# MingXiangL/SPE

Hardware: AMD Instinct MI355X
Metric: images/sec (whole node) at 3x800x1333 bs=2/GPU (higher is better)
Workload: dtype bf16/fp16 operands, fp32 accumulate; 1 GPU; TSCAM_cait_S24 (C=384, depth 24, 8 heads) + 0-layer encoder + 6-layer conditional-DETR decoder x2 stages, 100 queries, COCO heads (91), 2x3x800x1333 per GPU (N=4150 tokens), fwd + SetCriterion + SetCriterionRefine + bwd + grad all-reduce + clip + AdamW; global_batch=2, parallelism=dp1

## Files before the change

### include/spe_hip.h

```cpp
#ifndef SPE_HIP_H
#define SPE_HIP_H
#include <stddef.h>
#include <stdint.h>

#ifdef __cplusplus
extern "C" {
#endif

typedef struct ihipStream_t* spe_stream_t;

int spe_abi_version(void);

int spe_set_reduce_workspace(void* ws, size_t bytes, spe_stream_t stream);
int spe_reduce_defer_ranges(const void* const* ptrs, const size_t* bytes, int n);
int spe_reduce_defer_arena(void* arena, size_t bytes);
int spe_reduce_flush(spe_stream_t stream);
int spe_reduce_pending(void);

int spe_gemm_f32(const float* A, const float* B, float* C, const float* bias, float* C2,
                 int M, int N, int K, long lda, long ldb, long ldc, int transA, int transB,
                 int batch0, int batch1, long sA0, long sA1, long sB0, long sB1, long sC0, long sC1,
                 float alpha, int act, int splitk, int precision, spe_stream_t stream);

int spe_gemm_ex(const void* A, int a_bf16, const float* B, float* C, const float* bias, float* C2,
                int M, int N, int K, long lda, long ldb, long ldc, int transA, int transB,
                int batch0, int batch1, long sA0, long sA1, long sB0, long sB1, long sC0, long sC1,
                float alpha, int act, int splitk, int precision, spe_stream_t stream);

int spe_gemm_tile(int M, int N, int nbatch);
int spe_gemm_f32_plan(int M, int N, int K, long lda, long ldb, long ldc, int transA, int transB, int batch0, int batch1,
                      long sA0, long sA1, long sB0, long sB1, long sC0, long sC1, int splitk, int precision, int a_bf16,
                      int epilogue, int a_mod16, int b_mod16, long* v);

int spe_layernorm_fwd(const float* x, const float* gamma, const float* beta, float* y, float* mean,
                      float* rstd, long R, int C, float eps, void* y16, void* y16lo, spe_stream_t stream);
int spe_layernorm_fwd_h(const float* x, const float* gamma, const float* beta, float* y, float* mean,
                        float* rstd, long R, int C, float eps, void* y16, void* yh16, spe_stream_t stream);
int spe_layernorm_bwd(const float* dy, const float* x, const float* gamma, const float* mean,
                      const float* rstd, float* dx, float* dgamma, float* dbeta, long R, int C,
                      const float* add, spe_stream_t stream);
int spe_layernorm_bwd_ls(const float* dy, const float* x, const float* gamma, const float* mean, const float* rstd, float* dx,
                         float* dgamma, float* dbeta, long R, int C, const float* add, const float* ls_y, const float* ls_gamma,
                         void* ls_dy16, float* ls_db, float* ls_dg, spe_stream_t stream);

int spe_cvt_f16(const float* x, long ldx, int R, int C, void* out, long ldo, spe_stream_t stream);
int spe_gemm_bf16nt(const void* A16, const void* B16, const void* A16lo, const void* B16lo, float* C, const float* bias,
                    float* C2, int M, int N, int K, long lda, long ldb, long ldc, float alpha, int act, int splitk,
                    spe_stream_t stream);
int spe_linear_small_fwd(const float* x, long ldx, const void* W16, const void* W16lo, const float* bias, float* y, float* pre,
                         void* x16_out, int R, int N, int K, long ldc, int act, spe_stream_t stream);
int spe_linear_small_bwd(const float* dy, const float* aux, int act, const void* x16, const void* WT16, float* dx, float* dW,
                         float* db, int R, int N, int K, spe_stream_t stream);
int spe_linear_small_group_fwd(const float* x, long ldx, const void* const* W16, const void* const* W16lo, const float* const* bias,
                               const float* const* add, float* const* y, void* x16_out, int R, int nblk, int N, int K, spe_stream_t stream);
int spe_linear_small_group_bwd(const float* const* dy, const void* x16, const void* const* WT16, float* dx, float* const* dW,
                               float* const* db, int R, int nblk, int N, int K, spe_stream_t stream);
int spe_linear_small_plan(int entry, int R, int N, int K, int nblk, long ldx, int split, int want_dx, int want_dw, int want_db,
                          int any_dw, long* v);
int spe_gemm_bf16tn(const void* A16, const void* B16, float* C, int M, int N, int R, long lda, long ldb, long ldc,
                    float alpha, int splitk, spe_stream_t stream);
int spe_gemm_bf16tn_plan(int M, int N, int R, long lda, long ldb, int splitk, int* v);
int spe_gemm_bf16nt_ex(const void* A16, const void* B16, const void* A16lo, const void* B16lo, float* C, const float* bias,
                       float* C2, void* out16, void* out16lo, long ld16, void* out16T, long ld16t, float* colsum, const float* aux,
                       const float* res, const float* rgamma, int M, int N, int K, long lda, long ldb, long ldc, float alpha, int act,
                       int half_flags, spe_stream_t stream);
int spe_gemm_bf16nt_exd(const void* A16, const void* B16, const void* A16lo, const void* B16lo, float* C, const float* bias,
                        float* C2, void* out16, void* out16lo, long ld16, void* out16T, long ld16t, float* colsum, const float* aux,
                        const float* res, const float* rgamma, int M, int N, int K, long lda, long ldb, long ldc, float alpha, int act,
                        int half_flags, float p_drop, uint64_t seed, uint64_t offset, const float* sample_scale, long rows_per_sample,
                        spe_stream_t stream);
int spe_gemm_bf16nt_plan(int M, int N, int K, int split, int ex, int f16_operands, int f16_second, int splitk, int has_out16t,
                         long ld16t, int* plan);
int spe_cvt_bf16(const float* x, long ldx, int R, int C, void* out, void* out_lo, long ldo, void* outT, long ldt, float* colsum,
                 const float* aux, int act, spe_stream_t stream);
int spe_cvt_bf16_h(const float* x, long ldx, int R, int C, void* out, void* out_h, long ldo, void* outT, long ldt, spe_stream_t stream);
int spe_cvt_bf16_multi(const void* jobs_dev, int njobs, int total_tiles, spe_stream_t stream);

int spe_softmax_fwd(const float* S, const unsigned char* mask, float* P, float* Pd, int B, int H, int Nq,
                    int Nk, long ld, float p_drop, uint64_t seed, uint64_t offset, spe_stream_t stream);
int spe_softmax_bwd(const float* dPd, const float* P, float* dS, int B, int H, int Nq, int Nk, long ld,
                    float p_drop, uint64_t seed, uint64_t offset, spe_stream_t stream);

int spe_talking_softmax_fwd(const float* S, const float* Wl, const float* bl, const float* Ww, const float* bw,
                            float* P, float* Pd, int B, int H, int Nq, int Nk, long ld, float p_drop,
                            uint64_t seed, uint64_t offset, spe_stream_t stream);
int spe_talking_softmax_bwd(const float* dPd, const float* P, const float* S, const float* Wl, const float* Ww,
                            float* dS, float* ws, int nblocks, int B, int H, int Nq, int Nk, long ld,
                            float p_drop, uint64_t seed, uint64_t offset, spe_stream_t stream);

int spe_talking_fused_supported(int H, int dh);
int spe_attn_pack(const float* x, long sb, long sn, long sh, int B, int N, int H, int dh, float scale,
                  void* out, spe_stream_t stream);
int spe_talking_stats_plan(int B, int N, int nwg, int* steps_per_wg, int* nwg_used);
int spe_talking_stats(const void* Qf, const void* Kf, const float* Wl, const float* bl, float* ws_stats,
                      int B, int H, int N, int dh, int nwg, spe_stream_t stream);
int spe_attn_merge_rows(const float* ws, float* M, float* IL, const float* bl, float* rows, int Np, int B, int H, int N,
                        int steps_per_wg, spe_stream_t stream);
int spe_talking_wgrad_reduce(const float* ws_w, int nwg, int H, float* dWl, float* dbl, float* dWw, float* dbw,
                             spe_stream_t stream);

int spe_talking_flash_plan(int B, int N, int nwg, int* steps_per_wg, int* nwg_used, int* nmajor, int* rows_padded);
int spe_talking_flash_fwd(const void* Qf, const void* Kf, const void* V16, const float* Wl, const float* Ww, const float* bw,
                          const float* c0, int Np, float* ws, float* O, void* O16, void* O16lo, void* keepbits, int B, int H, int N, int dh,
                          int nwg, float p_drop, uint64_t seed, uint64_t offset, spe_stream_t stream);

int spe_talking_bwdk_pass1(const void* Qf, const void* dOf, const void* dO16, const void* Kf, const void* Vf, const float* Wl, const float* Ww,
                           const float* bw, const float* c0, int Np, float* ws_d, float* ws_v, float* ws_w, float* Drows, float* dv, void* dv16,
                           long ob, long on, long oh, const void* keepbits, int B, int H, int N, int dh, int nwg, float p_drop, spe_stream_t stream);
int spe_talking_bwdq_plan(int B, int N, int nwg, int* steps_per_wg, int* nwg_used, int* nmajor);
int spe_talking_bwdq_pass2(const void* Qf, const void* dOf, const void* Kf, const void* Vf, const void* K16, const float* Wl, const float* Ww,
                           const float* c0, const float* Drows, int Np, float* ws_q, float* ws_w, void* dS, float* dq, void* dq16,
                           long ob, long on, long oh, float scale, const void* keepbits, int B, int H, int N, int dh, int nwg, float p_drop,
                           spe_stream_t stream);

int spe_attn_pmean(const void* Qf, const void* Kf, const float* Wl, const float* c0, int Np, float* M, float alpha, int B, int H, int N, int dh,
                   spe_stream_t stream);
int spe_attn_pmean_dense(const float* P, float* M, float alpha, int B, int H, int N, long ld, spe_stream_t stream);

int spe_conv_head_fwd(const float* x, const float* W, const float* bias, float* map, float* logits, int B, int h, int w, int C, int K,
                      spe_stream_t stream);
int spe_conv_head_plan(int B, int h, int w, int C, int K, long* ws_floats);
int spe_conv_head_bwd(const float* x, const float* W, const float* dmap, const float* dlogits, float* dx, float* dW, float* db, float* ws,
                      long ws_floats, int B, int h, int w, int C, int K, spe_stream_t stream);

int spe_attn_pack16(const float* x, long sb, long sn, long sh, int B, int N, int H, int dh, void* out, spe_stream_t stream);
int spe_attn_pack_multi(int njobs, const float* const* xs, const long* strides, const float* scales, const int* kinds,
                        void* const* outs, const int* Ns, const int* dhs, int B, int H, spe_stream_t stream);
int spe_attn_contract(const void* T, const void* X16, float* out, long ob, long on, long oh, int B, int H, int N, int dh,
                      int trans, int fmt, float alpha, float* ws, unsigned int* counters, long ws_floats, void* out16,
                      void* out16lo, spe_stream_t stream);

int spe_colsum(const float* in, float* out, long R, int C, long ld, int accumulate, spe_stream_t stream);

int spe_layerscale_residual_fwd(const float* x, const float* y, const float* gamma, const float* sample_scale,
                                float* out, long R, int C, long rows_per_sample, spe_stream_t stream);
int spe_layerscale_residual_bwd(const float* dout, const float* y, const float* gamma, const float* sample_scale,
                                float* dy, float* dgamma, long R, int C, long rows_per_sample, spe_stream_t stream);
int spe_layerscale_residual_bwd16(const float* dout, const void* y, int y_f16, const float* gamma, void* dy16, void* dy16T, long ldt,
                                  float* db, float* dgamma, long R, int C, spe_stream_t stream);
int spe_layerscale_residual_bwd16d(const float* dout, const void* y, int y_f16, const float* gamma, void* dy16, void* dy16T, long ldt,
                                   float* db, float* dgamma, long R, int C, float p_drop, uint64_t seed, uint64_t offset,
                                   const float* sample_scale, long rows_per_sample, spe_stream_t stream);

int spe_act_bwd(const float* dy, const float* aux, float* dx, long n, int mode, spe_stream_t stream);

int spe_layernorm_res_fwd(const float* x, const float* z, const float* gamma, const float* beta, float* sum, float* y,
                          float* mean, float* rstd, long R, int C, float eps, float p, uint64_t seed, uint64_t offset,
                          spe_stream_t stream);
int spe_layernorm_res_bwd(const float* dy, const float* dy2, const float* sum, const float* gamma, const float* mean, const float* rstd,
                          float* ds, float* dz, float* dgamma, float* dbeta, long R, int C, float p, uint64_t seed,
                          uint64_t offset, spe_stream_t stream);

int spe_dropout(const float* x, float* y, long n, float p, uint64_t seed, uint64_t offset, spe_stream_t stream);

int spe_patchify(const float* img, float* cols, int B, int Cin, int Hi, int Wi, int P, spe_stream_t stream);

int spe_rowdot(const float* x, const float* y, float* D, int B, int L, int H, int dh, spe_stream_t stream);

int spe_add_rows(const float* a, const float* b, float* out, long n, long period, spe_stream_t stream);

int spe_bicubic(const float* src, float* dst, int gh, int gw, int h, int w, int C, int backward, spe_stream_t stream);

int spe_matcher_cost(const float* logits, const float* boxes, const int* tgt_ids, const float* tgt_boxes,
                     const int* toff, int total_targets, float* cost, int* err, int L, int B, int Q, int Kc,
                     float w_class, float w_bbox, float w_giou, spe_stream_t stream);

int spe_hungarian(const float* cost, const int* toff, long* srow, long* gidx, int* lidx, int* err, int L, int B, int Q,
                  spe_stream_t stream);
int spe_jitter_pick(const float* box, const float* scale, float* out, int M, int ncand, int ratio, spe_stream_t stream);

int spe_focal_loss(const float* logits, const int* tclass, const float* roww, float* grad, float* loss,
                   int* argmax, int L, long rows_per_l, int Kc, float alpha, float gamma, spe_stream_t stream);

int spe_box_loss(const float* pred_boxes, const long* srow, const float* tbox, const float* w, const int* lidx,
                 float* sums, float* g_l1, float* g_giou, long n, int L, spe_stream_t stream);
int spe_box_loss_bwd(const long* srow, const int* lidx, const float* g_l1, const float* g_giou, const float* c1,
                     const float* c2, float* dpred, long n, spe_stream_t stream);

int spe_kv_frags(const void* ym16, long ldm, const void* yp16, long ldp, void* Kf, void* V16, void* K16, void* Vf,
                 int L, int B, int S, int H, int dh, spe_stream_t stream);
int spe_kv_grad_scatter(const float* dk, const float* dv, void* dYm, long ldm, void* dYp, long ldp, int layer, int B, int S,
                        int H, int dh, spe_stream_t stream);
int spe_colsum_bf16_blocks(const void* x, long ld, long R, int nblk, int blkC, float* const* outs, int accumulate, spe_stream_t stream);

int spe_mha_plan(int B, int H, int Lq, int Lk, int* nch);
int spe_mha_fwd(const void* Qf, const void* Kf, const void* V16, const void* mask, float* Opart, float* ML, float* O,
                float* LSE, void* keepbits, int B, int H, int Lq, int Lk, int dk, int dv, int nch, float p_drop,
                uint64_t seed, uint64_t offset, spe_stream_t stream);
int spe_mha_bwd(const void* Qf, const void* Kf, const void* Vf, const void* dOf, const void* K16, const void* Q16,
                const void* dO16, const void* mask, const float* LSE, const float* D, const void* keepbits, float* dq,
                float* dq_ws, float* dk, float* dv, int B, int H, int Lq, int Lk, int dk_dim, int dv_dim, int nch, float scale,
                float p_drop, spe_stream_t stream);

int spe_pos_sine(const void* mask_u8, const float* dim_t, float* out, int B, int h, int w, int npf, float scale,
                 float eps, int normalize, spe_stream_t stream);

int spe_pos_learned_fwd(const float* col, const float* row, float* out, int B, int h, int w, int npf, spe_stream_t stream);
int spe_pos_learned_bwd(const float* g, float* d_col, float* d_row, int B, int h, int w, int npf, spe_stream_t stream);

int spe_nms_sorted(const float* boxes, const long* labels, const int* counts, unsigned char* keep, int nimg, int nmax,
                   float iou_threshold, spe_stream_t stream);

int spe_detect(const float* logits, const float* boxes, const float* sizes, int B, int Q, int Kc, int k, float iou_threshold,
               int do_nms, float* out_logit, long* out_label, float* out_box, int* out_query, int* out_count, spe_stream_t stream);

int spe_cam_prepare(const float* cams, int M, int h, int w, int rows, int cols, float cam_thr, float* minmax,
                    void* out, spe_stream_t stream);
int spe_cam_contour_boxes(const void* img, int rows, int cols, float area_ratio, int* boxes, int max_boxes, int* nboxes);
int spe_cam_boxes_device_workspace(int M, int rows, int cols, size_t* bytes);
int spe_cam_boxes_device(const void* img, int M, int rows, int cols, float area_ratio, void* workspace, size_t workspace_bytes,
                         int* boxes, int* nboxes, int max_boxes, spe_stream_t stream);

int spe_cam_targets(const int* packed, const int* cls0, int M, int max_boxes, int single, int W, int H, int cap, float* boxes,
                    long* labels, int* off, spe_stream_t stream);
int spe_refine_pick(const float* prob, const float* pred_boxes, const int* cls, const int* cls_off, const int* cls_host,
                    const int* cls_off_host, int B, int Q, int Kc, int U, float* scores, int* queries, float* boxes, spe_stream_t stream);

int spe_pseudo_quality(const float* boxes, const long* labels, const float* scores, const int* off, const float* gboxes,
                       const long* glabels, const int* goff, const int* off_host, const int* goff_host, int B, int T, int G, int C,
                       float iou_thresh, long* counters, spe_stream_t stream);

int spe_proposal_recall(const float* prob, const float* boxes, const float* gboxes, const long* glabels, const int* goff,
                        const int* goff_host, int B, int Q, int Kc, int G, int C, const float* thr, int T, const int* ks, int K,
                        long* counters, spe_stream_t stream);

int spe_voc_match(const float* det_boxes, const float* det_scores, const long* det_labels, const int* det_off,
                  const double* gt_boxes, const long* gt_labels, const unsigned char* gt_difficult, const int* gt_off,
                  int nimg, int num_classes, int max_det, int max_gt, double ovthresh, double score_scale, double coord_scale,
                  unsigned char* flags, double* scores_out, int* npos, int* nimgs, int* hits, spe_stream_t stream);
int spe_voc_ap(const unsigned char* flags, const int* seg_off, const int* npos, int num_classes, double* ap07, double* ap_area,
               double* rec, double* prec, spe_stream_t stream);

int spe_coco_match(const float* det_boxes, const long* det_cats, const int* det_off, const double* gt_boxes, const long* gt_cats,
                   const unsigned char* gt_iscrowd, const double* gt_area, const int* gt_off, const double* iou_thrs,
                   const double* area_rng, int nimg, int num_cats, int max_det, int max_gt, int top, int* rank, unsigned* words,
                   int* npig, spe_stream_t stream);
int spe_coco_accumulate(const unsigned* words, const int* rank, const float* det_scores, const int* seg_off, const int* npig,
                        const int* max_dets, const double* rec_thrs, int num_cats, int num_rec, int num_max_dets, double* precision,
                        double* recall, double* scores, spe_stream_t stream);

int spe_cls_ap_workspace(int n, int C, size_t* bytes);
int spe_cls_ap(const float* scores, const signed char* targets, int n, int C, long ld, int difficult, double* workspace, double* ap,
               int* npos, int* ncounted, spe_stream_t stream);

int spe_resample_plan(long* desc_host, int n, long* totals);
int spe_resample_tables(const long* desc_host, const long* desc_dev, int n, int* tables, spe_stream_t stream);
int spe_resample_h(const long* desc_host, const long* desc_dev, int n, const int* tables, unsigned char* tmp, spe_stream_t stream);
int spe_resample_v(const long* desc_host, const long* desc_dev, int n, const int* tables, const unsigned char* tmp, const float* lut,
                   float* out, unsigned char* mask, int Hmax, int Wmax, spe_stream_t stream);

#define SPE_JPEG_UNSUPPORTED (-7)
#define SPE_JPEG_CORRUPT (-8)
#define SPE_JPEG_INFO_INTS 224
int spe_jpeg_probe(const unsigned char* data, long n, int* info);
int spe_jpeg_entropy(const unsigned char* data, long n, short* coef, long coef_elems, int* reason);
int spe_jpeg_reconstruct(const long* desc_host, const long* desc_dev, int n, const short* coef, long coef_elems,
                         unsigned char* planes, long planes_bytes, spe_stream_t stream);

int spe_ledger_state_bytes(int K, int E, size_t* bytes);
int spe_ledger_record(const float* vals, const float* weights, const unsigned char* mask, const double* extras_host, int K, int E,
                      void* state, size_t state_bytes, float* total, spe_stream_t stream);
int spe_ledger_total_bwd(const float* g, const float* weights, const unsigned char* mask, int K, float* dvals, spe_stream_t stream);
int spe_ledger_summary(void* state, size_t state_bytes, int K, int E, const int* windows_host, const int* windows_dev,
                       const float* ring_override, const int* order, double* out, spe_stream_t stream);

int spe_sqnorm_partials(const float* g, long n, float* partials, int nblocks, spe_stream_t stream);
int spe_adamw_flat(float* p, float* g, float* m, float* v, long n, const long* seg_end, const float* seg_lr,
                   const float* seg_wd, int nseg, float beta1, float beta2, float eps, float bias_c1, float bias_c2,
                   const float* partials, int npartials, float max_norm, int write_grad, float grad_scale,
                   spe_stream_t stream);

#define SPE_ADAMW_GUARD_WORDS 16
int spe_adamw_gate(void* guard, const float* partials, int npartials, float max_norm, float grad_scale, double beta1,
                   double beta2, spe_stream_t stream);
int spe_adamw_flat_guarded(float* p, float* g, float* m, float* v, long n, const long* seg_end, const float* seg_lr,
                           const float* seg_wd, int nseg, float beta1, float beta2, float eps, const void* guard,
                           int write_grad, spe_stream_t stream);

int spe_accum_flat(float* dst, const float* a, const float* b, long n, spe_stream_t stream);

int spe_adamw_flat_ema(float* p, float* g, float* m, float* v, float* e, long n, const long* seg_end, const float* seg_lr,
                       const float* seg_wd, int nseg, float beta1, float beta2, float eps, float bias_c1, float bias_c2,
                       const float* partials, int npartials, float max_norm, int write_grad, float grad_scale,
                       const void* guard, double decay, int warmup, long t, spe_stream_t stream);
int spe_swap_flat(float* a, float* b, long n, spe_stream_t stream);

#define SPE_GRAD_REPORT_WORDS 8
int spe_grad_report(const float* g, const float* p, long n, const long* par_beg, const long* par_len, int npar,
                    float grad_scale, const void* guard, int when, void* out, spe_stream_t stream);

int spe_occupy(int nwg, long micros, float* buf, long buf_floats, spe_stream_t stream);

#ifdef __cplusplus
}
#endif
#endif
```

### spe_amd/csrc/attn_flash.hip

```cpp
#include "attn_flash_common.h"

struct FlashFwdArgs {
    const unsigned char* Qf; const unsigned char* Kf; const unsigned char* V16;
    const float* Wl; const float* Ww; const float* bw;
    const float* c0;
    int Np;
    float* ws_o;
    int B, N, nt, nmaj, spw; long total;
    float p_drop; uint64_t seed, offset;
    unsigned* keepbits;
};

#define FLF_NW 8
#define FLF_HB 4
#define FLF_QS (FLF_MAJ / FLF_NW)

template <int H, int DSTEPS, bool TAIL16, bool DROP>
__global__ __launch_bounds__(64 * FLF_NW, FLF_NW / 4) void talking_flash_fwd_kernel(FlashFwdArgs a) {
    constexpr int FULL = FragDims<DSTEPS, TAIL16>::FULL, DT = FragDims<DSTEPS, TAIL16>::DT, REC = FragDims<DSTEPS, TAIL16>::REC;
    constexpr int NW = FLF_NW, QS = FLF_QS;
    constexpr int TILEB = H * REC;
    extern __shared__ __attribute__((aligned(16))) unsigned char smem[];
    const int lane = threadIdx.x & 63, wave = __builtin_amdgcn_readfirstlane(threadIdx.x >> 6);
    const unsigned lds0 = __builtin_amdgcn_readfirstlane((unsigned)(uintptr_t)(__attribute__((address_space(3))) unsigned char*)smem);
    const unsigned char* sQ = smem + 5 * TILEB + wave * (QS * TILEB);
    const unsigned ldsQ = lds0 + 5 * TILEB + wave * (QS * TILEB);
    const int grp = wave >> 2;
    const int nt = a.nt, N = a.N;

    float Al4[H / 4][H];
    fl_mixA_f32<H, false>(a.Wl, lane, Al4);
    fls16x4_t Aw[H / 4][H / 4];
    fl_mixA_16<H, false, true>(a.Ww, lane, 1.0f, Aw);
    f32x4_t vbws[H / 4];
#pragma unroll
    for (int gh = 0; gh < H / 4; ++gh)
#pragma unroll
        for (int i = 0; i < 4; ++i) vbws[gh][i] = a.bw[4 * gh + i] * FL_PD_SCALE;
    constexpr int NP = TILEB / 1024, NPW = (NP + NW - 1) / NW;
    unsigned voff[NPW];
#pragma unroll
    for (int i = 0; i < NPW; ++i) {
        const int o = (i * NW + wave) * 1024 + lane * 16;
        voff[i] = (unsigned)((o / REC) * nt * REC + o % REC);
    }

    const long s_begin = (long)blockIdx.x * a.spw;
    long s_end = s_begin + a.spw; if (s_end > a.total) s_end = a.total;
    long s = s_begin;
    while (s < s_end) {
        const int bm = (int)(s / nt), kt0 = (int)(s % nt);
        int seg = nt - kt0; if (seg > s_end - s) seg = (int)(s_end - s);
        const int b = bm / a.nmaj, mj = bm % a.nmaj;
        const int qt0 = (mj * NW + wave) * QS;
        const bool wvalid = qt0 < nt;

#pragma unroll
        for (int u = 0; u < QS; ++u) {
            constexpr int NPQ = TILEB / 1024;
            const unsigned char* qbase = a.Qf + ((long)b * H * nt + min(qt0 + u, nt - 1)) * REC;
#pragma unroll
            for (int p = 0; p < NPQ; ++p) {
                const int o = p * 1024 + lane * 16;
                fl_glds16_s(qbase, (unsigned)((o / REC) * nt * REC + o % REC), ldsQ + u * TILEB + p * 1024);
            }
        }
        auto issue_tile = [&](const unsigned char* base, int kt, unsigned dst) {
            const unsigned char* tb = base + ((long)b * H * nt + kt) * REC;
            if constexpr (NP % NW == 0 && NPW <= 4) fl_glds16_run<NPW, NW * 1024>(tb, voff, dst + wave * 1024);
            else {
#pragma unroll
                for (int i = 0; i < NPW; ++i) {
                    const int p = i * NW + wave;
                    if (NP % NW != 0 && p >= NP) break;
                    fl_glds16_s(tb, voff[i], dst + p * 1024);
                }
            }
        };
        issue_tile(a.Kf, kt0, lds0);

        f32x4_t c0v[QS][H / 4];
        int qrow[QS];
#pragma unroll
        for (int u = 0; u < QS; ++u) {
            qrow[u] = (qt0 + u) * 16 + (lane & 15);
            const float* cp = a.c0 + ((long)b * a.Np + (wvalid ? min(qrow[u], N - 1) : 0)) * H;
#pragma unroll
            for (int gh = 0; gh < H / 4; ++gh) {
                c0v[u][gh] = *reinterpret_cast<const f32x4_t*>(cp + 4 * gh);
#pragma unroll
                for (int i = 0; i < 4; ++i) c0v[u][gh][i] += 8.0f;
            }
        }
        f32x4_t O[QS][H][DT];
#pragma unroll
        for (int u = 0; u < QS; ++u)
#pragma unroll
            for (int g = 0; g < H; ++g)
#pragma unroll
                for (int dt = 0; dt < DT; ++dt) O[u][g][dt] = (f32x4_t){0.f, 0.f, 0.f, 0.f};

        auto step_barrier = [&](int j) {
            asm volatile("s_waitcnt vmcnt(0)" ::: "memory");
            __builtin_amdgcn_s_barrier();
            asm volatile("" ::: "memory");
            if (j + 1 < seg) issue_tile(a.Kf, kt0 + j + 1, lds0 + ((j + 1) % 3) * TILEB);
            if (j < seg) issue_tile(a.V16, kt0 + j, lds0 + (3 + (j & 1)) * TILEB);
        };
        step_barrier(0);
        for (int i = 0; i < seg; ++i) {
            if (grp == 0) step_barrier(i + 1);
            if (!wvalid) { if (grp != 0) step_barrier(i + 1); continue; }
            const unsigned char* sK = smem + (i % 3) * TILEB;
            const unsigned char* sV = smem + (3 + (i & 1)) * TILEB;
            fls16x4_t bv[QS][4][H / 4];
#pragma unroll
            for (int u = 0; u < QS; ++u) {
                f32x4_t sp[4][H / 4];
#pragma unroll
                for (int r = 0; r < 4; ++r)
#pragma unroll
                    for (int gh = 0; gh < H / 4; ++gh) sp[r][gh] = c0v[u][gh];
#pragma unroll
                for (int h0 = 0; h0 < H; h0 += FLF_HB) {
                    flu32x4_t kf[FLF_HB][FULL ? FULL : 1], qf[FLF_HB][FULL ? FULL : 1];
                    fls16x4_t kt16[FLF_HB], qt16[FLF_HB];
#pragma unroll
                    for (int hb = 0; hb < FLF_HB; ++hb) {
                        const unsigned char* kr = sK + (h0 + hb) * REC;
                        const unsigned char* qr = sQ + (u * H + h0 + hb) * REC;
#pragma unroll
                        for (int st = 0; st < FULL; ++st) {
                            kf[hb][st] = *reinterpret_cast<const flu32x4_t*>(kr + st * 1024 + lane * 16);
                            qf[hb][st] = *reinterpret_cast<const flu32x4_t*>(qr + st * 1024 + lane * 16);
                        }
                        if constexpr (TAIL16) {
                            kt16[hb] = *reinterpret_cast<const fls16x4_t*>(kr + FULL * 1024 + lane * 8);
                            qt16[hb] = *reinterpret_cast<const fls16x4_t*>(qr + FULL * 1024 + lane * 8);
                        }
                    }
#pragma unroll
                    for (int hb = 0; hb < FLF_HB; ++hb) {
                        f32x4_t c = {0.f, 0.f, 0.f, 0.f};
#pragma unroll
                        for (int st = 0; st < FULL; ++st) c = fl_mfma32<true>(kf[hb][st], qf[hb][st], c);
                        if constexpr (TAIL16) {
                            const f32x4_t t = fl_mfma16<true>(kt16[hb], qt16[hb], (f32x4_t){0.f, 0.f, 0.f, 0.f});
                            c = (FULL > 0) ? c + t : t;
                        }
#pragma unroll
                        for (int r = 0; r < 4; ++r)
#pragma unroll
                            for (int gh = 0; gh < H / 4; ++gh) sp[r][gh] = __builtin_amdgcn_mfma_f32_4x4x1f32(Al4[gh][h0 + hb], c[r], sp[r][gh], 0, 0, 0);
                    }
                }
#pragma unroll
                for (int r = 0; r < 4; ++r)
#pragma unroll
                    for (int hh = 0; hh < H / 4; ++hh)
                        bv[u][r][hh] = fl_pack4_f16(fl_exp2(sp[r][hh][0]), fl_exp2(sp[r][hh][1]), fl_exp2(sp[r][hh][2]), fl_exp2(sp[r][hh][3]));
                __builtin_amdgcn_sched_barrier(0);
            }
            if (grp != 0) step_barrier(i + 1);
#pragma unroll
            for (int u = 0; u < QS; ++u) {
                f32x4_t pr[4][H / 4];
#pragma unroll
                for (int r = 0; r < 4; ++r)
#pragma unroll
                    for (int gh = 0; gh < H / 4; ++gh) {
                        f32x4_t d = vbws[gh];
#pragma unroll
                        for (int hh = 0; hh < H / 4; ++hh)
                            d = __builtin_amdgcn_mfma_f32_4x4x4f16(__builtin_bit_cast(flf16x4_t, Aw[gh][hh]), __builtin_bit_cast(flf16x4_t, bv[u][r][hh]), d, 0, 0, 0);
                        pr[r][gh] = d;
                    }
                if constexpr (DROP) {
                    const uint32_t thr = (uint32_t)(a.p_drop * 65536.0f);
                    const float inv = 1.0f / (1.0f - a.p_drop);
                    uint32_t kbw = 0u;
#pragma unroll
                    for (int hp = 0; hp < H / 2; ++hp) {
                        const int g0 = 2 * hp, g1 = 2 * hp + 1;
                        uint32_t o[4];
                        fl_keep_lots<H>(a.seed, a.offset, b, hp, qrow[u], (kt0 + i) * 16 + 4 * (lane >> 4), N, o);
#pragma unroll
                        for (int r = 0; r < 4; ++r) {
                            const bool e0 = fl_lot(o, 0, r) >= thr, e1 = fl_lot(o, 1, r) >= thr;
                            pr[r][g0 >> 2][g0 & 3] *= e0 ? inv : 0.f;
                            pr[r][g1 >> 2][g1 & 3] *= e1 ? inv : 0.f;
                            kbw |= ((e0 ? 1u : 0u) | (e1 ? 2u : 0u)) << (hp * 8 + 2 * r);
                        }
                    }
                    if (a.keepbits && wvalid && qt0 + u < nt) a.keepbits[(((long)b * nt + (qt0 + u)) * nt + (kt0 + i)) * 64 + lane] = kbw;
                }
#pragma unroll
                for (int g = 0; g < H; ++g) {
                    const fls16x4_t pk = fl_pack4<true>(pr[0][g >> 2][g & 3], pr[1][g >> 2][g & 3], pr[2][g >> 2][g & 3], pr[3][g >> 2][g & 3]);
#pragma unroll
                    for (int dt = 0; dt < DT; ++dt)
                        O[u][g][dt] = fl_mfma16<true>(*reinterpret_cast<const fls16x4_t*>(sV + g * REC + dt * 512 + lane * 8), pk, O[u][g][dt]);
                }
                __builtin_amdgcn_sched_barrier(0);
            }
        }
        __builtin_amdgcn_s_barrier();

        if (wvalid) {
            const int first_wg = (int)(((long)bm * nt) / a.spw);
            const int slot = (int)blockIdx.x - first_wg;
#pragma unroll
            for (int u = 0; u < QS; ++u) {
                if (qt0 + u >= nt) continue;
                float* dst = a.ws_o + ((((long)bm * FL_MAXSLOT + slot) * NW + wave) * QS + u) * (long)(H * DT * 256);
#pragma unroll
                for (int g = 0; g < H; ++g)
#pragma unroll
                    for (int dt = 0; dt < DT; ++dt) *reinterpret_cast<f32x4_t*>(dst + (g * DT + dt) * 256 + lane * 4) = O[u][g][dt];
            }
        }
        s += seg;
    }
}

__global__ __launch_bounds__(256) void flash_merge_kernel(const float* __restrict__ ws, float* __restrict__ O, long ob, long on, long oh,
                                                          unsigned short* __restrict__ O16, unsigned short* __restrict__ O16lo,
                                                          int B, int H, int N, int nt, int dh, int DT, int nmaj, int spw, long nvec) {
    const long i = (long)blockIdx.x * 256 + threadIdx.x;
    if (i >= nvec) return;
    constexpr int QS = FLF_QS;
    const int lane = (int)(i & 63);
    long r = i >> 6;
    const int dt = (int)(r % DT); r /= DT;
    const int g = (int)(r % H); r /= H;
    const int u = (int)(r % QS); r /= QS;
    const int wave = (int)(r % FLF_NW); r /= FLF_NW;
    const int bm = (int)r;
    const int b = bm / nmaj, mj = bm % nmaj;
    const int qt = (mj * FLF_NW + wave) * QS + u;
    const int q = qt * 16 + (lane & 15), d = dt * 16 + 4 * (lane >> 4);
    if (qt >= nt || q >= N || d >= dh) return;
    const int first_wg = (int)(((long)bm * nt) / spw), last_wg = (int)(((long)(bm + 1) * nt - 1) / spw);
    const long slot_stride = (long)FLF_MAJ * H * DT * 256;
    const float* src = ws + (long)bm * FL_MAXSLOT * slot_stride + (((long)wave * QS + u) * H + g) * (long)(DT * 256) + dt * 256 + lane * 4;
    f32x4_t acc = {0.f, 0.f, 0.f, 0.f};
    for (int sl = 0; sl <= last_wg - first_wg; ++sl) acc += *reinterpret_cast<const f32x4_t*>(src + sl * slot_stride);
    acc *= (1.0f / FL_PD_SCALE);
    const long oi = (long)b * ob + (long)q * on + (long)g * oh + d;
    if (d + 3 < dh && ((ob | on | oh) & 3) == 0) {
        if (O && ((reinterpret_cast<uintptr_t>(O) & 15) == 0)) *reinterpret_cast<f32x4_t*>(O + oi) = acc;
        else if (O) { O[oi] = acc[0]; O[oi + 1] = acc[1]; O[oi + 2] = acc[2]; O[oi + 3] = acc[3]; }
        if (O16) {
            unsigned short hi[4], lo[4];
#pragma unroll
            for (int k = 0; k < 4; ++k) { hi[k] = spe_f2bf(acc[k]); lo[k] = spe_f2bf(acc[k] - spe_bf2f(hi[k])); }
            const uint2 h2 = make_uint2((unsigned)hi[0] | ((unsigned)hi[1] << 16), (unsigned)hi[2] | ((unsigned)hi[3] << 16));
            if ((reinterpret_cast<uintptr_t>(O16) & 7) == 0) *reinterpret_cast<uint2*>(O16 + oi) = h2;
            else { O16[oi] = hi[0]; O16[oi + 1] = hi[1]; O16[oi + 2] = hi[2]; O16[oi + 3] = hi[3]; }
            if (O16lo) {
                const uint2 l2 = make_uint2((unsigned)lo[0] | ((unsigned)lo[1] << 16), (unsigned)lo[2] | ((unsigned)lo[3] << 16));
                if ((reinterpret_cast<uintptr_t>(O16lo) & 7) == 0) *reinterpret_cast<uint2*>(O16lo + oi) = l2;
                else { O16lo[oi] = lo[0]; O16lo[oi + 1] = lo[1]; O16lo[oi + 2] = lo[2]; O16lo[oi + 3] = lo[3]; }
            }
        }
        return;
    }
#pragma unroll
    for (int k = 0; k < 4; ++k) {
        if (d + k >= dh) break;
        if (O) O[oi + k] = acc[k];
        if (O16) {
            const unsigned short hi = spe_f2bf(acc[k]);
            O16[oi + k] = hi;
            if (O16lo) O16lo[oi + k] = spe_f2bf(acc[k] - spe_bf2f(hi));
        }
    }
}

template <int H, int DSTEPS, bool TAIL16>
static int launch_flash_fwd(const FlashFwdArgs& a, int nwg, bool drop, hipStream_t st) {
    constexpr int DT = FragDims<DSTEPS, TAIL16>::DT;
    if constexpr (flf_lds_bytes(H, DT, true) > FL_LDS_MAX) return -2;
    else return fl_launch<FlashFwdArgs, talking_flash_fwd_kernel<H, DSTEPS, TAIL16, true>, talking_flash_fwd_kernel<H, DSTEPS, TAIL16, false>>(
        a, nwg, 64 * FLF_NW, flf_lds_bytes(H, DT, false), flf_lds_bytes(H, DT, true), drop, st);
}

extern "C" int spe_talking_flash_plan(int B, int N, int nwg, int* steps_per_wg, int* nwg_used, int* nmajor, int* rows_padded) {
    const int nt = (N + 15) / 16;
    if ((long)B * nt <= 0 || nwg <= 0) { *steps_per_wg = 0; *nwg_used = 0; *nmajor = 0; *rows_padded = 0; return 0; }
    const FlashPlan p = fl_plan(B, nt, FLF_MAJ, nt, nwg);
    *steps_per_wg = p.spw; *nwg_used = p.nwg; *nmajor = p.nmaj; *rows_padded = nt * 16 + 64;
    return 0;
}

extern "C" int spe_talking_flash_fwd(const void* Qf, const void* Kf, const void* V16, const float* Wl, const float* Ww, const float* bw,
                                     const float* c0, int Np, float* ws, float* O, void* O16, void* O16lo, void* keepbits, int B, int H, int N,
                                     int dh, int nwg, float p_drop, uint64_t seed, uint64_t offset, hipStream_t st) {
    const int nt = (N + 15) / 16;
    if ((long)B * nt <= 0) return 0;
    if (dh < 1 || dh > 64 || nwg <= 0 || (O16lo && !O16) || Np < nt * 16 + 64) return -2;
    const FlashPlan p = fl_plan(B, nt, FLF_MAJ, nt, nwg);
    FlashFwdArgs a;
    a.Qf = (const unsigned char*)Qf; a.Kf = (const unsigned char*)Kf; a.V16 = (const unsigned char*)V16;
    a.Wl = Wl; a.Ww = Ww; a.bw = bw; a.c0 = c0; a.Np = Np; a.ws_o = ws;
    a.B = B; a.N = N; a.nt = nt; a.nmaj = p.nmaj; a.spw = p.spw; a.total = p.total;
    a.p_drop = p_drop; a.seed = seed; a.offset = offset; a.keepbits = reinterpret_cast<unsigned*>(p_drop > 0.f ? keepbits : nullptr);
    const bool drop = p_drop > 0.f;
    const int rc = attn_dispatch(H, dh, [&](auto h, auto ds, auto tl) {
        return launch_flash_fwd<decltype(h)::value, decltype(ds)::value, decltype(tl)::value>(a, p.nwg, drop, st); });
    if (rc != 0) return rc;
    const int DT = frag_geom(dh).dt;
    const long nvec = (long)B * p.nmaj * FLF_MAJ * H * DT * 64;
    hipLaunchKernelGGL(flash_merge_kernel, dim3((unsigned)((nvec + 255) / 256)), dim3(256), 0, st, ws, O, (long)N * H * dh, (long)H * dh, (long)dh,
                       reinterpret_cast<unsigned short*>(O16), reinterpret_cast<unsigned short*>(O16lo), B, H, N, nt, dh, DT, p.nmaj, p.spw, nvec);
    SPE_CHECK_LAUNCH();
    return 0;
}
```

### spe_amd/csrc/attn_flash_bwd.hip

```cpp
#include "attn_flash_common.h"

#define FLB_NW 4
#define FLB_HB 4
#define FLB_GWR 144
#define FLB_NK16 3
#define FLB_RSFUSE 1
#define FLB_DQAHEAD 2
#define FLB_SB_NOMEM 0x00F
#define FLB_PHASE() __builtin_amdgcn_sched_barrier(0)
#ifndef SPE_ABLATE
#undef FLB_DBG_SAMETILE
#undef FLB_DBG_NOST
#undef FLB_DBG_STAMP
#endif
#ifdef FLB_DBG_STAMP
#define FLB_STAMP(k) asm volatile("s_memtime %0\n\ts_waitcnt lgkmcnt(0)" : "=s"(stamp[k]))
#else
#define FLB_STAMP(k)
#endif
#ifndef FLB_STAGGER
#define FLB_STAGGER 1
#endif

struct FlashBwdArgs {
// ... 209 lines not shown
                    }
            }
            f32x4_t c[HB];
            static_assert(HB == 4, "chunk of 4 heads");
            flb_score_f16<FULL, TAIL16>(kfr.f, kfr.t, &qa[h0], &qta[h0], c);
            flb_fence4(c[0], c[1], c[2], c[3]);
#pragma unroll
            for (int hb = 0; hb < HB; ++hb) {
                const f32x4_t cs = c[hb];
                *reinterpret_cast<fls16x4_t*>(gwf + (h0 + hb) * GWR) = fl_pack4<false>(cs[0], cs[1], cs[2], cs[3]);
#pragma unroll
                for (int r = 0; r < 4; ++r)
#pragma unroll
                    for (int gh = 0; gh < H / 4; ++gh) sp[r][gh] = __builtin_amdgcn_mfma_f32_4x4x1f32(Al4[gh][h0 + hb], cs[r], sp[r][gh], 0, 0, 0);
            }
        };
        auto front_v = [&](int i, auto g0_c, const Frags& vfr, f32x4_t (&dp)[4][H / 4], uint32_t kb) {
            constexpr int g0 = decltype(g0_c)::value;
            if constexpr (g0 == 0) {
#pragma unroll
                for (int r = 0; r < 4; ++r)
#pragma unroll
                    for (int gh = 0; gh < H / 4; ++gh) dp[r][gh] = Dn[gh];
            }
            f32x4_t es[HB];
            flb_score_bf16<FULL, TAIL16>(vfr.f, vfr.t, &da[g0], &dta[g0], es);
            flb_fence4(es[0], es[1], es[2], es[3]);
#pragma unroll
            for (int hb = 0; hb < HB; ++hb) {
                if constexpr (DROP) {
                    const int g = g0 + hb;
#pragma unroll
                    for (int r = 0; r < 4; ++r) es[hb][r] *= ((kb >> ((g >> 1) * 8 + 2 * r + (g & 1))) & 1u) ? keep_inv : 0.f;
                }
            }
#pragma unroll
            for (int hq = 0; hq < HB / 4; ++hq)
#pragma unroll
                for (int r = 0; r < 4; ++r) {
                    const fls16x4_t bv = fl_pack4<false>(es[4 * hq][r], es[4 * hq + 1][r], es[4 * hq + 2][r], es[4 * hq + 3][r]);
#pragma unroll
                    for (int gh = 0; gh < H / 4; ++gh) dp[r][gh] = __builtin_amdgcn_mfma_f32_4x4x4bf16_1k(Awt[gh][g0 / 4 + hq], bv, dp[r][gh], 0, 0, 0);
                }
        };
        auto load_kb = [&](int i) -> uint32_t {
            if constexpr (DROP) return *reinterpret_cast<const uint32_t*>(smem + KBOFF + (i & 1) * 1024 + wave * 256 + lane * 4);
            else return 0u;
        };

        auto back_exp = [&](f32x4_t (&sp)[4][H / 4]) {
#pragma unroll
            for (int r = 0; r < 4; ++r)
#pragma unroll
                for (int gh = 0; gh < H / 4; ++gh)
#pragma unroll
                    for (int k = 0; k < 4; ++k) sp[r][gh][k] = fl_exp2(sp[r][gh][k]);
        };
        auto back_ds = [&](f32x4_t (&sp)[4][H / 4], f32x4_t (&dp)[4][H / 4]) {
            unsigned char* gwb = gw_wr + 2 * GWT;
#pragma unroll
            for (int r = 0; r < 4; ++r)
#pragma unroll
                for (int gh = 0; gh < H / 4; ++gh) sp[r][gh] = sp[r][gh] * dp[r][gh];
#pragma unroll
            for (int r = 0; r < 4; ++r)
#pragma unroll
                for (int g = 0; g < H; ++g) gb[g] += sp[r][g >> 2][g & 3];
#pragma unroll
            for (int g = 0; g < H; ++g)
                *reinterpret_cast<fls16x4_t*>(gwb + g * GWR) =
                    fl_pack4<false>(sp[0][g >> 2][g & 3], sp[1][g >> 2][g & 3], sp[2][g >> 2][g & 3], sp[3][g >> 2][g & 3]);
        };
        auto back_gw = [&](int i, f32x4_t (&sp)[4][H / 4], f32x4_t (&ds)[4][H / 4]) {
            {
                const unsigned rdf = gw_rd + (i & 1) * GWT, rdb = gw_rd + 2 * GWT;
                const unsigned char* gw_xrd = (gm < H) ? sgw + rdb : gw_zero;
                const unsigned char* gw_yrd = (gm < H) ? sgw + rdf : gw_zero;
                __builtin_amdgcn_fence(__ATOMIC_RELEASE, "wavefront");
                __builtin_amdgcn_fence(__ATOMIC_ACQUIRE, "wavefront");
#pragma unroll
                for (int c = 0; c < 8; ++c) {
                    const flu32x4_t xa = *reinterpret_cast<const flu32x4_t*>(gw_xrd + c * 16);
                    const flu32x4_t yb = *reinterpret_cast<const flu32x4_t*>(gw_yrd + c * 16);
                    gwacc[c & 3] = fl_mfma32<false>(xa, yb, gwacc[c & 3]);
                }
                __builtin_amdgcn_fence(__ATOMIC_RELEASE, "wavefront");
            }
#pragma unroll
            for (int r = 0; r < 4; ++r) {
                float x[H];
#pragma unroll
                for (int g = 0; g < H; ++g) x[g] = sp[r][g >> 2][g & 3];
                fl_mix_16<H, false>(x, Alt, nullptr, ds[r]);
            }
        };
        auto back_dq = [&](int i, f32x4_t (&ds)[4][H / 4]) {
            {
                const int kt = kt0 + i;
                const unsigned char* sK16 = smem + 2 * KVB + (i % NK16) * TILEB;
                fls16x4_t ka[H][DT];
#pragma unroll
                for (int h = 0; h < ((FLB_DQAHEAD < H) ? FLB_DQAHEAD : H); ++h)
#pragma unroll
                    for (int dt = 0; dt < DT; ++dt) ka[h][dt] = *reinterpret_cast<const fls16x4_t*>(sK16 + h * REC + dt * 512 + lane * 8);
#pragma unroll
                for (int h = 0; h < H; ++h) {
                    if (h + FLB_DQAHEAD < H) {
#pragma unroll
                        for (int dt = 0; dt < DT; ++dt) ka[h + FLB_DQAHEAD][dt] = *reinterpret_cast<const fls16x4_t*>(sK16 + (h + FLB_DQAHEAD) * REC + dt * 512 + lane * 8);
                        __builtin_amdgcn_sched_barrier(FLB_SB_NOMEM);
                    }
                    const fls16x4_t pk = fl_pack4<false>(ds[0][h >> 2][h & 3], ds[1][h >> 2][h & 3], ds[2][h >> 2][h & 3], ds[3][h >> 2][h & 3]);
#ifndef FLB_DBG_NOST
                    __builtin_nontemporal_store(__builtin_bit_cast(flu32x2_t, pk),
                                                reinterpret_cast<flu32x2_t*>(a.dS + (((((long)b * H + h) * nt + qt) * nt + kt) * 64 + lane) * 4));
#endif
                    flb_dq_mfma<DT>(dQ[h], ka[h], pk);
                }
            }
        };
        auto front = [&](int i, f32x4_t (&sp)[4][H / 4], f32x4_t (&dp)[4][H / 4], auto mask_c) {
            const uint32_t kb = load_kb(i);
            Frags fa, fb;
            load_k(i, 0, fa);
            if constexpr (H > HB) load_k(i, HB, fb);
            front_k(i, std::integral_constant<int, 0>{}, fa, sp, mask_c);
            load_v(i, 0, fa);
            if constexpr (H > HB) front_k(i, std::integral_constant<int, HB>{}, fb, sp, mask_c);
            if constexpr (H > HB) load_v(i, HB, fb);
            front_v(i, std::integral_constant<int, 0>{}, fa, dp, kb);
            if constexpr (H > HB) front_v(i, std::integral_constant<int, HB>{}, fb, dp, kb);
        };
        auto back = [&](int i, f32x4_t (&sp)[4][H / 4], f32x4_t (&dp)[4][H / 4]) {
            f32x4_t ds[4][H / 4];
            back_exp(sp);
            back_ds(sp, dp);
            back_gw(i, sp, ds);
            back_dq(i, ds);
        };
        auto step = [&](int i, f32x4_t (&sp)[4][H / 4], f32x4_t (&dp)[4][H / 4], f32x4_t (&spn)[4][H / 4], f32x4_t (&dpn)[4][H / 4], Frags& fr0, Frags& fr1,
                        bool more) {
            f32x4_t ds[4][H / 4];
            const uint32_t kb = load_kb(i + 1);
            if constexpr (H > HB) load_k(i + 1, HB, fr1); else load_v(i + 1, 0, fr1);
            __builtin_amdgcn_sched_barrier(FLB_SB_NOMEM);
            front_k(i + 1, std::integral_constant<int, 0>{}, fr0, spn, std::false_type{});
            back_exp(sp);
            FLB_PHASE();
            FLB_STAMP(2);
            if (FLB_STAGGER && more && wave >= NW / 2) issue_tiles(i + 2);
            if constexpr (H > HB) {
                load_v(i + 1, 0, fr0);
                __builtin_amdgcn_sched_barrier(FLB_SB_NOMEM);
                front_k(i + 1, std::integral_constant<int, HB>{}, fr1, spn, std::false_type{});
            }
            back_ds(sp, dp);
            FLB_PHASE();
            FLB_STAMP(3);
            if constexpr (H > HB) {
                load_v(i + 1, HB, fr1);
                __builtin_amdgcn_sched_barrier(FLB_SB_NOMEM);
                front_v(i + 1, std::integral_constant<int, 0>{}, fr0, dpn, kb);
            } else front_v(i + 1, std::integral_constant<int, 0>{}, fr1, dpn, kb);
            back_gw(i, sp, ds);
            FLB_PHASE();
            FLB_STAMP(4);
            if constexpr (H > HB) front_v(i + 1, std::integral_constant<int, HB>{}, fr1, dpn, kb);
            back_dq(i, ds);
        };

        auto admit = [&](int nxt, bool late) {
            asm volatile("s_waitcnt vmcnt(0)" ::: "memory");
            __builtin_amdgcn_s_barrier();
            asm volatile("" ::: "memory");
            if (nxt + 1 < seg && !(late && wave >= NW / 2)) issue_tiles(nxt + 1);
        };

        const int nfull = ((N & 15) != 0 && kt0 + seg == nt) ? seg - 1 : seg;
        f32x4_t spA[4][H / 4], dpA[4][H / 4], spB[4][H / 4], dpB[4][H / 4];
        Frags frA, frB;
        issue_tiles(0);
        admit(0, false);
        if (nfull > 0) {
            if (wvalid) front(0, spA, dpA, std::false_type{});
            for (int i = 0; i + 1 < nfull; ++i) {
                FLB_STAMP(0);
                admit(i + 1, FLB_STAGGER && wvalid);
                FLB_STAMP(1);
                if (wvalid) {
                    load_k(i + 1, 0, frA);
                    step(i, spA, dpA, spB, dpB, frA, frB, i + 2 < seg);
#pragma unroll
                    for (int r = 0; r < 4; ++r)
#pragma unroll
                        for (int gh = 0; gh < H / 4; ++gh) { spA[r][gh] = spB[r][gh]; dpA[r][gh] = dpB[r][gh]; }
                }
#ifdef FLB_DBG_STAMP
                FLB_STAMP(5);
                asm volatile("s_waitcnt lgkmcnt(0)" : "+s"(stamp[0]), "+s"(stamp[1]), "+s"(stamp[2]), "+s"(stamp[3]), "+s"(stamp[4]), "+s"(stamp[5]));
                for (int k = 0; k < 5; ++k) stacc[k] += stamp[k + 1] - stamp[k];
                ++stn;
#endif
            }
            if (nfull < seg) admit(nfull, false);
            if (wvalid) back(nfull - 1, spA, dpA);
        }
        if (nfull < seg) {
            if (wvalid) { front(nfull, spA, dpA, std::true_type{}); back(nfull, spA, dpA); }
        }
        __builtin_amdgcn_s_barrier();

        const int first_wg = (int)(((long)bm * nt) / a.spw);
        const int slot = (int)blockIdx.x - first_wg;
        {
#pragma unroll
            for (int g = 0; g < H; ++g)
#pragma unroll
                for (int dt = 0; dt < DT; ++dt) flb_acc_fence(dQ[g][dt]);
            if (wvalid) {
                float* dst = a.ws_q + (((long)bm * FL_MAXSLOT + slot) * NW + wave) * (long)(H * DT * 256);
#pragma unroll
                for (int g = 0; g < H; ++g)
#pragma unroll
                    for (int dt = 0; dt < DT; ++dt) *reinterpret_cast<f32x4_t*>(dst + (g * DT + dt) * 256 + lane * 4) = dQ[g][dt];
            }
        }
        s += seg;
    }

#ifdef FLB_DBG_STAMP
    if (blockIdx.x == 0 && threadIdx.x == 0) {
        unsigned long long* o = reinterpret_cast<unsigned long long*>(a.dS);
        for (int k = 0; k < 5; ++k) o[k] = stacc[k];
        o[5] = stn;
    }
#endif
    {
        constexpr int NWG = 2 * (H * H + H);
        float* row = a.ws_w + ((long)blockIdx.x * NW + wave) * NWG;
        const f32x4_t dsum = (gwacc[0] + gwacc[1]) + (gwacc[2] + gwacc[3]);
        const int nn = lane & 15;
#pragma unroll
        for (int r = 0; r < 4; ++r) {
            const int g = 4 * (lane >> 4) + r;
            if (g < H && nn < H) row[g * H + nn] = FL_LN2 * dsum[r];
        }
#pragma unroll
        for (int g = 0; g < H; ++g) {
            const float v = spe_wave_sum(gb[g]);
            if (lane == 0) row[H * H + g] = v;
        }
    }
}

__global__ __launch_bounds__(256) void bwdq_dq_merge_kernel(const float* __restrict__ ws, float* __restrict__ O, unsigned short* __restrict__ O16,
                                                            long ob, long on, long oh, int B, int H, int N, int nt, int dh, int DT, int nmaj, int spw,
                                                            float scale, long nvec) {
    const long i = (long)blockIdx.x * 256 + threadIdx.x;
    if (i >= nvec) return;
    const int lane = (int)(i & 63);
    long r = i >> 6;
    const int dt = (int)(r % DT); r /= DT;
    const int g = (int)(r % H); r /= H;
    const int wave = (int)(r % FLB_NW); r /= FLB_NW;
    const long bm = r;
    const int b = (int)(bm / nmaj), mj = (int)(bm % nmaj);
    const int qt = mj * FLB_NW + wave;
    const int q = qt * 16 + (lane & 15), d = dt * 16 + 4 * (lane >> 4);
    if (qt >= nt || q >= N || d >= dh) return;
    const int first_wg = (int)((bm * nt) / spw), last_wg = (int)(((bm + 1) * nt - 1) / spw);
    const long slot_stride = (long)FLB_NW * H * DT * 256;
    const float* src = ws + bm * FL_MAXSLOT * slot_stride + ((long)wave * H + g) * (long)(DT * 256) + dt * 256 + lane * 4;
    f32x4_t acc = {0.f, 0.f, 0.f, 0.f};
    for (int sl = 0; sl <= last_wg - first_wg; ++sl) acc += *reinterpret_cast<const f32x4_t*>(src + sl * slot_stride);
    acc *= scale;
    const long oi = (long)b * ob + (long)q * on + (long)g * oh + d;
#pragma unroll
    for (int k = 0; k < 4; ++k) {
        if (d + k >= dh) break;
        if (O) O[oi + k] = acc[k];
    }
    if (O16) {
        if (d + 3 < dh && ((ob | on | oh) & 3) == 0 && ((reinterpret_cast<uintptr_t>(O16) & 7) == 0)) {
            const unsigned short h0 = spe_f2bf(acc[0]), h1 = spe_f2bf(acc[1]), h2 = spe_f2bf(acc[2]), h3 = spe_f2bf(acc[3]);
            *reinterpret_cast<uint2*>(O16 + oi) = make_uint2((unsigned)h0 | ((unsigned)h1 << 16), (unsigned)h2 | ((unsigned)h3 << 16));
        } else {
#pragma unroll
            for (int k = 0; k < 4; ++k) { if (d + k >= dh) break; O16[oi + k] = spe_f2bf(acc[k]); }
        }
    }
}

struct FlashBwdKArgs {
    const unsigned char* Qf; const unsigned char* dOf; const unsigned char* dO16;
    const unsigned char* Kf; const unsigned char* Vf;
    const float* Wl; const float* Ww; const float* bw;
    const float* c0; int Np;
    float* ws_d;
    float* ws_v;
    float* ws_w;
    const unsigned* keepbits;
    int B, N, nt, nmaj, spw; long total;
    float p_drop;
};

__device__ __forceinline__ void flb_rowsum4(const f32x4_t (&t)[4], f32x4_t& o) {
    float a0, a1, a2, a3, b0, b1, b2, b3;
    asm("s_nop 1\n\t"
        "v_add_f32_dpp %0, %12, %12 row_ror:8 row_mask:0xf bank_mask:0x3\n\t"
        "v_add_f32_dpp %1, %13, %13 row_ror:8 row_mask:0xf bank_mask:0x3\n\t"
        "v_add_f32_dpp %2, %14, %14 row_ror:8 row_mask:0xf bank_mask:0x3\n\t"
        "v_add_f32_dpp %3, %15, %15 row_ror:8 row_mask:0xf bank_mask:0x3\n\t"
        "v_add_f32_dpp %0, %20, %20 row_ror:8 row_mask:0xf bank_mask:0xc\n\t"
        "v_add_f32_dpp %1, %21, %21 row_ror:8 row_mask:0xf bank_mask:0xc\n\t"
        "v_add_f32_dpp %2, %22, %22 row_ror:8 row_mask:0xf bank_mask:0xc\n\t"
        "v_add_f32_dpp %3, %23, %23 row_ror:8 row_mask:0xf bank_mask:0xc\n\t"
        "v_add_f32_dpp %4, %16, %16 row_ror:8 row_mask:0xf bank_mask:0x3\n\t"
        "v_add_f32_dpp %5, %17, %17 row_ror:8 row_mask:0xf bank_mask:0x3\n\t"
        "v_add_f32_dpp %6, %18, %18 row_ror:8 row_mask:0xf bank_mask:0x3\n\t"
        "v_add_f32_dpp %7, %19, %19 row_ror:8 row_mask:0xf bank_mask:0x3\n\t"
        "v_add_f32_dpp %4, %24, %24 row_ror:8 row_mask:0xf bank_mask:0xc\n\t"
        "v_add_f32_dpp %5, %25, %25 row_ror:8 row_mask:0xf bank_mask:0xc\n\t"
        "v_add_f32_dpp %6, %26, %26 row_ror:8 row_mask:0xf bank_mask:0xc\n\t"
        "v_add_f32_dpp %7, %27, %27 row_ror:8 row_mask:0xf bank_mask:0xc\n\t"
        "v_add_f32_dpp %8, %0, %0 row_half_mirror row_mask:0xf bank_mask:0x5\n\t"
        "v_add_f32_dpp %9, %1, %1 row_half_mirror row_mask:0xf bank_mask:0x5\n\t"
        "v_add_f32_dpp %10, %2, %2 row_half_mirror row_mask:0xf bank_mask:0x5\n\t"
        "v_add_f32_dpp %11, %3, %3 row_half_mirror row_mask:0xf bank_mask:0x5\n\t"
        "v_add_f32_dpp %8, %4, %4 row_half_mirror row_mask:0xf bank_mask:0xa\n\t"
        "v_add_f32_dpp %9, %5, %5 row_half_mirror row_mask:0xf bank_mask:0xa\n\t"
        "v_add_f32_dpp %10, %6, %6 row_half_mirror row_mask:0xf bank_mask:0xa\n\t"
        "v_add_f32_dpp %11, %7, %7 row_half_mirror row_mask:0xf bank_mask:0xa\n\t"
        "v_add_f32_dpp %8, %8, %8 quad_perm:[1,0,3,2] row_mask:0xf bank_mask:0xf\n\t"
        "v_add_f32_dpp %9, %9, %9 quad_perm:[1,0,3,2] row_mask:0xf bank_mask:0xf\n\t"
        "v_add_f32_dpp %10, %10, %10 quad_perm:[1,0,3,2] row_mask:0xf bank_mask:0xf\n\t"
        "v_add_f32_dpp %11, %11, %11 quad_perm:[1,0,3,2] row_mask:0xf bank_mask:0xf\n\t"
        "v_add_f32_dpp %8, %8, %8 quad_perm:[2,3,0,1] row_mask:0xf bank_mask:0xf\n\t"
        "v_add_f32_dpp %9, %9, %9 quad_perm:[2,3,0,1] row_mask:0xf bank_mask:0xf\n\t"
        "v_add_f32_dpp %10, %10, %10 quad_perm:[2,3,0,1] row_mask:0xf bank_mask:0xf\n\t"
        "v_add_f32_dpp %11, %11, %11 quad_perm:[2,3,0,1] row_mask:0xf bank_mask:0xf"
        : "=&v"(a0), "=&v"(a1), "=&v"(a2), "=&v"(a3), "=&v"(b0), "=&v"(b1), "=&v"(b2), "=&v"(b3),
          "=&v"(o[0]), "=&v"(o[1]), "=&v"(o[2]), "=&v"(o[3])
        : "v"(t[0][0]), "v"(t[0][1]), "v"(t[0][2]), "v"(t[0][3]), "v"(t[1][0]), "v"(t[1][1]), "v"(t[1][2]), "v"(t[1][3]),
          "v"(t[2][0]), "v"(t[2][1]), "v"(t[2][2]), "v"(t[2][3]), "v"(t[3][0]), "v"(t[3][1]), "v"(t[3][2]), "v"(t[3][3]));
}

#define FLB_SCORE_RS_ASM(NAME, M32, M16)                                                                                                   \
    __device__ __forceinline__ void NAME(const flu32x4_t (*k32)[1], const flu32x2_t* k16, const flu32x4_t (*q32)[1], const flu32x2_t* q16, \
                                         f32x4_t* c, const f32x4_t (&t)[4], f32x4_t& o) {                                                  \
        float a0, a1, a2, a3, b0, b1, b2, b3;                                                                                              \
            asm("s_nop 1\n\t"   \
                M32 " %0, %16, %24, 0\n\t"   \
                "v_add_f32_dpp %4, %32, %32 row_ror:8 row_mask:0xf bank_mask:0x3\n\t"   \
                "v_add_f32_dpp %5, %33, %33 row_ror:8 row_mask:0xf bank_mask:0x3\n\t"   \
                "v_add_f32_dpp %6, %34, %34 row_ror:8 row_mask:0xf bank_mask:0x3\n\t"   \
                "v_add_f32_dpp %7, %35, %35 row_ror:8 row_mask:0xf bank_mask:0x3\n\t"   \
                M32 " %1, %17, %25, 0\n\t"   \
                "v_add_f32_dpp %4, %40, %40 row_ror:8 row_mask:0xf bank_mask:0xc\n\t"   \
                "v_add_f32_dpp %5, %41, %41 row_ror:8 row_mask:0xf bank_mask:0xc\n\t"   \
                "v_add_f32_dpp %6, %42, %42 row_ror:8 row_mask:0xf bank_mask:0xc\n\t"   \
                "v_add_f32_dpp %7, %43, %43 row_ror:8 row_mask:0xf bank_mask:0xc\n\t"   \
                M32 " %2, %18, %26, 0\n\t"   \
                "v_add_f32_dpp %8, %36, %36 row_ror:8 row_mask:0xf bank_mask:0x3\n\t"   \
                "v_add_f32_dpp %9, %37, %37 row_ror:8 row_mask:0xf bank_mask:0x3\n\t"   \
                "v_add_f32_dpp %10, %38, %38 row_ror:8 row_mask:0xf bank_mask:0x3\n\t"   \
                "v_add_f32_dpp %11, %39, %39 row_ror:8 row_mask:0xf bank_mask:0x3\n\t"   \
                M32 " %3, %19, %27, 0\n\t"   \
                "v_add_f32_dpp %8, %44, %44 row_ror:8 row_mask:0xf bank_mask:0xc\n\t"   \
                "v_add_f32_dpp %9, %45, %45 row_ror:8 row_mask:0xf bank_mask:0xc\n\t"   \
                "v_add_f32_dpp %10, %46, %46 row_ror:8 row_mask:0xf bank_mask:0xc\n\t"   \
                "v_add_f32_dpp %11, %47, %47 row_ror:8 row_mask:0xf bank_mask:0xc\n\t"   \
                M16 " %0, %20, %28, %0\n\t"   \
                "v_add_f32_dpp %12, %4, %4 row_half_mirror row_mask:0xf bank_mask:0x5\n\t"   \
                "v_add_f32_dpp %13, %5, %5 row_half_mirror row_mask:0xf bank_mask:0x5\n\t"   \
                "v_add_f32_dpp %14, %6, %6 row_half_mirror row_mask:0xf bank_mask:0x5\n\t"   \
                "v_add_f32_dpp %15, %7, %7 row_half_mirror row_mask:0xf bank_mask:0x5\n\t"   \
                M16 " %1, %21, %29, %1\n\t"   \
                "v_add_f32_dpp %12, %8, %8 row_half_mirror row_mask:0xf bank_mask:0xa\n\t"   \
                "v_add_f32_dpp %13, %9, %9 row_half_mirror row_mask:0xf bank_mask:0xa\n\t"   \
                "v_add_f32_dpp %14, %10, %10 row_half_mirror row_mask:0xf bank_mask:0xa\n\t"   \
                "v_add_f32_dpp %15, %11, %11 row_half_mirror row_mask:0xf bank_mask:0xa\n\t"   \
                M16 " %2, %22, %30, %2\n\t"   \
                "v_add_f32_dpp %12, %12, %12 quad_perm:[1,0,3,2] row_mask:0xf bank_mask:0xf\n\t"   \
                "v_add_f32_dpp %13, %13, %13 quad_perm:[1,0,3,2] row_mask:0xf bank_mask:0xf\n\t"   \
                "v_add_f32_dpp %14, %14, %14 quad_perm:[1,0,3,2] row_mask:0xf bank_mask:0xf\n\t"   \
                "v_add_f32_dpp %15, %15, %15 quad_perm:[1,0,3,2] row_mask:0xf bank_mask:0xf\n\t"   \
                M16 " %3, %23, %31, %3\n\t"   \
                "v_add_f32_dpp %12, %12, %12 quad_perm:[2,3,0,1] row_mask:0xf bank_mask:0xf\n\t"   \
                "v_add_f32_dpp %13, %13, %13 quad_perm:[2,3,0,1] row_mask:0xf bank_mask:0xf\n\t"   \
                "v_add_f32_dpp %14, %14, %14 quad_perm:[2,3,0,1] row_mask:0xf bank_mask:0xf\n\t"   \
                "v_add_f32_dpp %15, %15, %15 quad_perm:[2,3,0,1] row_mask:0xf bank_mask:0xf"   \
            : "=&v"(c[0]), "=&v"(c[1]), "=&v"(c[2]), "=&v"(c[3]), "=&v"(a0), "=&v"(a1), "=&v"(a2), "=&v"(a3), "=&v"(b0), "=&v"(b1), "=&v"(b2),  \
              "=&v"(b3), "=&v"(o[0]), "=&v"(o[1]), "=&v"(o[2]), "=&v"(o[3])                                                                 \
            : "v"(k32[0][0]), "v"(k32[1][0]), "v"(k32[2][0]), "v"(k32[3][0]), "v"(k16[0]), "v"(k16[1]), "v"(k16[2]), "v"(k16[3]),          \
              "a"(q32[0][0]), "a"(q32[1][0]), "a"(q32[2][0]), "a"(q32[3][0]), "a"(q16[0]), "a"(q16[1]), "a"(q16[2]), "a"(q16[3]),          \
              "v"(t[0][0]), "v"(t[0][1]), "v"(t[0][2]), "v"(t[0][3]), "v"(t[1][0]), "v"(t[1][1]), "v"(t[1][2]), "v"(t[1][3]),              \
              "v"(t[2][0]), "v"(t[2][1]), "v"(t[2][2]), "v"(t[2][3]), "v"(t[3][0]), "v"(t[3][1]), "v"(t[3][2]), "v"(t[3][3]));             \
    }
FLB_SCORE_RS_ASM(flb_score_rs_f16, "v_mfma_f32_16x16x32_f16", "v_mfma_f32_16x16x16_f16")
FLB_SCORE_RS_ASM(flb_score_rs_bf16, "v_mfma_f32_16x16x32_bf16", "v_mfma_f32_16x16x16_bf16")



template <int H, int DSTEPS, bool TAIL16, bool DROP>
__global__ __launch_bounds__(64 * FLB_NW, 1) void talking_bwdk_kernel(FlashBwdKArgs a) {
    constexpr int FULL = FragDims<DSTEPS, TAIL16>::FULL, DT = FragDims<DSTEPS, TAIL16>::DT, REC = FragDims<DSTEPS, TAIL16>::REC;
    constexpr int NW = FLB_NW, HB = (H >= FLB_HB) ? FLB_HB : H;
    constexpr int TILEB = H * REC;
    constexpr int STG = 2 * TILEB;
    constexpr int NK16 = FLB_NK16;
    constexpr int F1 = FULL ? FULL : 1;
    extern __shared__ __attribute__((aligned(16))) unsigned char smem[];
    const int lane = threadIdx.x & 63, wave = __builtin_amdgcn_readfirstlane(threadIdx.x >> 6);
    const unsigned lds0 = __builtin_amdgcn_readfirstlane((unsigned)(uintptr_t)(__attribute__((address_space(3))) unsigned char*)smem);
    const int nt = a.nt;
    constexpr int C0OFF = 2 * STG + NK16 * TILEB, DXB = 16 * H * 4, DXOFF = C0OFF + 2048, GCOFF = DXOFF + 2 * NW * DXB;
    constexpr int KBOFF = GCOFF + 512 + NW * 3 * (4 * H * FLB_GWR);

    float Al4[H / 4][H];
    fl_mixA_f32<H, false>(a.Wl, lane, Al4);
    fls16x4_t Awt[H / 4][H / 4];
    fl_mixA_16<H, true, false>(a.Ww, lane, 1.0f, Awt);
    fls16x4_t Awp[H / 4][H / 4];
    fl_mixA_16<H, false, true>(a.Ww, lane, 1.0f, Awp);
    f32x4_t vbw[H / 4];
#pragma unroll
    for (int gh = 0; gh < H / 4; ++gh)
#pragma unroll
        for (int i = 0; i < 4; ++i) vbw[gh][i] = a.bw[4 * gh + i] * FL_PD_SCALE;

    constexpr int GWR = FLB_GWR, GWT = 4 * H * GWR;
    unsigned char* gconst = smem + GCOFF;
    unsigned char* sgw = gconst + 512 + wave * (3 * GWT);
    if (threadIdx.x < 64) reinterpret_cast<uint2*>(gconst)[threadIdx.x] = (threadIdx.x >= 26 && threadIdx.x < 42) ? make_uint2(0x3F803F80u, 0x3F803F80u) : make_uint2(0u, 0u);
    const int gm = lane & 15, gk = lane >> 4;
    unsigned char* gw_wr = sgw + (gk * H) * GWR + gm * 8;
    const unsigned gw_rd = (unsigned)((gk * H + gm) * GWR);
    const unsigned char* gw_zero = gconst + 48;
    const unsigned char* gw_ones = gconst + 208;
    f32x4_t gwacc[4];
#pragma unroll
    for (int i = 0; i < 4; ++i) gwacc[i] = (f32x4_t){0.f, 0.f, 0.f, 0.f};

    constexpr int NP = TILEB / 1024, NPW = (NP + NW - 1) / NW;
    unsigned voff[NPW];
#pragma unroll
    for (int i = 0; i < NPW; ++i) {
        const int o = (i * NW + wave) * 1024 + lane * 16;
        voff[i] = (unsigned)((o / REC) * nt * REC + o % REC);
    }
    const float keep_inv = DROP ? 1.0f / (1.0f - a.p_drop) : 1.0f;
    const int kbsh = 2 * (gm & 3);
#ifdef FLB_DBG_STAMP
    unsigned long long stamp[7] = {0, 0, 0, 0, 0, 0, 0}, stacc[6] = {0, 0, 0, 0, 0, 0}, stn = 0;
#endif
    const int kbln = (gm >> 2) << 4;

    const long s_begin = (long)blockIdx.x * a.spw;
    long s_end = s_begin + a.spw; if (s_end > a.total) s_end = a.total;
    long s = s_begin;
    while (s < s_end) {
        const int bm = (int)(s / nt), qt0 = (int)(s % nt);
        int seg = nt - qt0; if (seg > s_end - s) seg = (int)(s_end - s);
        const int b = bm / a.nmaj, mj = bm % a.nmaj;
        const int kt = mj * NW + wave;
        const bool wvalid = kt < nt;
        const int ktc = wvalid ? kt : nt - 1;
        const int nvw = (nt - mj * NW < NW) ? nt - mj * NW : NW;
        unsigned kb_voff = 0u;
        if constexpr (DROP) {
            const int w = lane >> 4, kw = (mj * NW + w < nt) ? w : 0;
            kb_voff = (unsigned)(kw * 256 + (lane & 15) * 16);
        }

        flu32x4_t ka[H][F1], va[H][F1];
        flu32x2_t kta[H], vta[H];
#pragma unroll
        for (int h = 0; h < H; ++h) {
            const unsigned char* kb_ = a.Kf + (((long)b * H + h) * nt + ktc) * REC;
            const unsigned char* vb_ = a.Vf + (((long)b * H + h) * nt + ktc) * REC;
#pragma unroll
            for (int st = 0; st < FULL; ++st) {
                ka[h][st] = *reinterpret_cast<const flu32x4_t*>(kb_ + st * 1024 + lane * 16);
                va[h][st] = *reinterpret_cast<const flu32x4_t*>(vb_ + st * 1024 + lane * 16);
            }
            if constexpr (TAIL16) {
                kta[h] = *reinterpret_cast<const flu32x2_t*>(kb_ + FULL * 1024 + lane * 8);
                vta[h] = *reinterpret_cast<const flu32x2_t*>(vb_ + FULL * 1024 + lane * 8);
            } else { kta[h] = (flu32x2_t){0u, 0u}; vta[h] = (flu32x2_t){0u, 0u}; }
        }
        f32x4_t dV[H][DT];
#pragma unroll
        for (int g = 0; g < H; ++g)
#pragma unroll
            for (int dt = 0; dt < DT; ++dt) dV[g][dt] = (f32x4_t){0.f, 0.f, 0.f, 0.f};

        auto issue_tiles = [&](int i) {
#ifdef FLB_DBG_SAMETILE
            const int qt = 0;
#else
            const int qt = qt0 + i;
#endif
#pragma unroll
            for (int op = 0; op < 3; ++op) {
                const unsigned char* base = (op == 0) ? a.Qf : ((op == 1) ? a.dOf : a.dO16);
                const unsigned char* tb = base + ((long)b * H * nt + qt) * REC;
                const unsigned dst = (op < 2) ? lds0 + (i & 1) * STG + op * TILEB : lds0 + 2 * STG + (i % NK16) * TILEB;
                if constexpr (NP % NW == 0 && NPW <= 4) fl_glds16_run<NPW, NW * 1024>(tb, voff, dst + wave * 1024);
                else {
#pragma unroll
                    for (int ii = 0; ii < NPW; ++ii) {
                        const int p = ii * NW + wave;
                        if (NP % NW != 0 && p >= NP) break;
                        fl_glds16_s(tb, voff[ii], dst + p * 1024);
                    }
                }
            }
            if (wave == NW - 1) fl_glds16_s(a.c0 + ((long)b * a.Np + qt * 16) * H, (unsigned)(lane * 16), lds0 + C0OFF + (i & 1) * 1024);
            if constexpr (DROP)
                if (wave == 1) fl_glds16_s(a.keepbits + (((long)b * nt + qt) * nt + mj * NW) * 64, kb_voff, lds0 + KBOFF + (i & 1) * 1024);
        };

        struct Frags { flu32x4_t f[HB][F1]; flu32x2_t t[HB]; };
        auto load_frags = [&](const unsigned char* tile, int h0, Frags& o) {
#pragma unroll
            for (int hb = 0; hb < HB; ++hb) {
                const unsigned char* r = tile + (h0 + hb) * REC;
#pragma unroll
                for (int st = 0; st < FULL; ++st) o.f[hb][st] = *reinterpret_cast<const flu32x4_t*>(r + st * 1024 + lane * 16);
                if constexpr (TAIL16) o.t[hb] = *reinterpret_cast<const flu32x2_t*>(r + FULL * 1024 + lane * 8);
                else o.t[hb] = (flu32x2_t){0u, 0u};
            }
        };
        auto load_q = [&](int i, int h0, Frags& o) { load_frags(smem + (i & 1) * STG, h0, o); };
        auto load_d = [&](int i, int g0, Frags& o) { load_frags(smem + (i & 1) * STG + TILEB, g0, o); };
        auto front_q = [&](int i, auto h0_c, const Frags& qfr, f32x4_t (&sp)[4][H / 4], const f32x4_t (*rs_t)[4] = nullptr, f32x4_t* rs_o = nullptr) {
            constexpr int h0 = decltype(h0_c)::value;
            if constexpr (h0 == 0) {
                const unsigned char* cr = smem + C0OFF + (i & 1) * 1024 + (4 * gk) * H * 4;
#pragma unroll
                for (int r = 0; r < 4; ++r)
#pragma unroll
                    for (int gh = 0; gh < H / 4; ++gh) sp[r][gh] = *reinterpret_cast<const f32x4_t*>(cr + (r * H + 4 * gh) * 4) + 8.0f;
            }
            f32x4_t c[HB];
            static_assert(HB == 4, "chunk of 4 heads");
            if constexpr (FULL == 1 && TAIL16) {
                if (rs_t) flb_score_rs_f16(qfr.f, qfr.t, &ka[h0], &kta[h0], c, *rs_t, *rs_o);
                else flb_score_f16<FULL, TAIL16>(qfr.f, qfr.t, &ka[h0], &kta[h0], c);
            } else flb_score_f16<FULL, TAIL16>(qfr.f, qfr.t, &ka[h0], &kta[h0], c);
            flb_fence4(c[0], c[1], c[2], c[3]);

#pragma unroll
            for (int hb = 0; hb < HB; ++hb) {
                const f32x4_t cs = c[hb];
#pragma unroll
                for (int r = 0; r < 4; ++r)
#pragma unroll
                    for (int gh = 0; gh < H / 4; ++gh) sp[r][gh] = __builtin_amdgcn_mfma_f32_4x4x1f32(Al4[gh][h0 + hb], cs[r], sp[r][gh], 0, 0, 0);
            }
        };
        auto front_d = [&](int i, auto g0_c, const Frags& dfr, f32x4_t (&dp)[4][H / 4], const uint32_t (&kb)[4], const f32x4_t (*rs_t)[4] = nullptr,
                           f32x4_t* rs_o = nullptr) {
            constexpr int g0 = decltype(g0_c)::value;
            unsigned char* gwf = gw_wr + (i & 1) * GWT;
            if constexpr (g0 == 0) {
#pragma unroll
                for (int r = 0; r < 4; ++r)
#pragma unroll
                    for (int gh = 0; gh < H / 4; ++gh) dp[r][gh] = (f32x4_t){0.f, 0.f, 0.f, 0.f};
            }
            f32x4_t es[HB];
            if constexpr (FULL == 1 && TAIL16) {
                if (rs_t) flb_score_rs_bf16(dfr.f, dfr.t, &va[g0], &vta[g0], es, *rs_t, *rs_o);
                else flb_score_bf16<FULL, TAIL16>(dfr.f, dfr.t, &va[g0], &vta[g0], es);
            } else flb_score_bf16<FULL, TAIL16>(dfr.f, dfr.t, &va[g0], &vta[g0], es);
            flb_fence4(es[0], es[1], es[2], es[3]);
#pragma unroll
            for (int hb = 0; hb < HB; ++hb) {
                if constexpr (DROP) {
                    const int g = g0 + hb;
#pragma unroll
                    for (int r = 0; r < 4; ++r) es[hb][r] *= ((kb[r] >> ((g >> 1) * 8 + kbsh + (g & 1))) & 1u) ? keep_inv : 0.f;
                }
                *reinterpret_cast<fls16x4_t*>(gwf + (g0 + hb) * GWR) = fl_pack4<false>(es[hb][0], es[hb][1], es[hb][2], es[hb][3]);
            }
#pragma unroll
            for (int hq = 0; hq < HB / 4; ++hq)
#pragma unroll
                for (int r = 0; r < 4; ++r) {
                    const fls16x4_t bv = fl_pack4<false>(es[4 * hq][r], es[4 * hq + 1][r], es[4 * hq + 2][r], es[4 * hq + 3][r]);
#pragma unroll
                    for (int gh = 0; gh < H / 4; ++gh) dp[r][gh] = __builtin_amdgcn_mfma_f32_4x4x4bf16_1k(Awt[gh][g0 / 4 + hq], bv, dp[r][gh], 0, 0, 0);
                }
        };
        auto load_kb = [&](int i, uint32_t (&kb)[4]) {
            if constexpr (DROP) {
                const flu32x4_t w4 = *reinterpret_cast<const flu32x4_t*>(smem + KBOFF + (i & 1) * 1024 + (wvalid ? wave : 0) * 256 + (kbln + 4 * gk) * 4);
#pragma unroll
                for (int r = 0; r < 4; ++r) kb[r] = w4[r];
            } else {
#pragma unroll
                for (int r = 0; r < 4; ++r) kb[r] = 0u;
            }
        };

        auto back_exp = [&](f32x4_t (&sp)[4][H / 4]) {
#pragma unroll
            for (int r = 0; r < 4; ++r)
#pragma unroll
                for (int gh = 0; gh < H / 4; ++gh)
#pragma unroll
                    for (int k = 0; k < 4; ++k) sp[r][gh][k] = fl_exp2(sp[r][gh][k]);
        };
        auto d_terms = [&](int gh, f32x4_t (&sp)[4][H / 4], f32x4_t (&dp)[4][H / 4], f32x4_t (&t)[4]) {
#pragma unroll
            for (int r = 0; r < 4; ++r) t[r] = dp[r][gh] * sp[r][gh];
        };
        auto d_store = [&](int i, int gh, const f32x4_t& o) {
            float* dx = reinterpret_cast<float*>(smem + DXOFF + ((i & 1) * NW + wave) * DXB) + (4 * gk + (gm >> 2)) * H;
            if ((gm & 3) == 0) *reinterpret_cast<f32x4_t*>(dx + 4 * gh) = o;
        };
        auto back_ds = [&](int i, f32x4_t (&sp)[4][H / 4], f32x4_t (&dp)[4][H / 4], bool with_d = true) {
            unsigned char* gwb = gw_wr + 2 * GWT;
            float* dx = reinterpret_cast<float*>(smem + DXOFF + ((i & 1) * NW + wave) * DXB) + (4 * gk + (gm >> 2)) * H;
#pragma unroll
            for (int gh = 0; gh < (with_d ? H / 4 : 0); ++gh) {
                f32x4_t t[4], o;
#pragma unroll
                for (int r = 0; r < 4; ++r) t[r] = dp[r][gh] * sp[r][gh];
                flb_rowsum4(t, o);
                if ((gm & 3) == 0) *reinterpret_cast<f32x4_t*>(dx + 4 * gh) = o;
            }
#pragma unroll
            for (int g = 0; g < H; ++g)
                *reinterpret_cast<fls16x4_t*>(gwb + g * GWR) =
                    fl_pack4<false>(sp[0][g >> 2][g & 3], sp[1][g >> 2][g & 3], sp[2][g >> 2][g & 3], sp[3][g >> 2][g & 3]);
        };
        auto back_gw = [&](int i, f32x4_t (&sp)[4][H / 4], f32x4_t (&pp)[4][H / 4]) {
            {
                const unsigned rdf = gw_rd + (i & 1) * GWT, rdb = gw_rd + 2 * GWT;
                const unsigned char* gw_xrd = (gm < H) ? sgw + rdf : gw_zero;
                const unsigned char* gw_yrd = (gm < H) ? sgw + rdb : ((gm == H) ? gw_ones : gw_zero);
                __builtin_amdgcn_fence(__ATOMIC_RELEASE, "wavefront");
                __builtin_amdgcn_fence(__ATOMIC_ACQUIRE, "wavefront");
#pragma unroll
                for (int c = 0; c < 8; ++c) {
                    const flu32x4_t xa = *reinterpret_cast<const flu32x4_t*>(gw_xrd + c * 16);
                    const flu32x4_t yb = *reinterpret_cast<const flu32x4_t*>(gw_yrd + c * 16);
                    gwacc[c & 3] = fl_mfma32<false>(xa, yb, gwacc[c & 3]);
                }
                __builtin_amdgcn_fence(__ATOMIC_RELEASE, "wavefront");
            }
#pragma unroll
            for (int r = 0; r < 4; ++r) {
                fls16x4_t bv[H / 4];
#pragma unroll
                for (int hh = 0; hh < H / 4; ++hh) bv[hh] = fl_pack4_f16(sp[r][hh][0], sp[r][hh][1], sp[r][hh][2], sp[r][hh][3]);
#pragma unroll
                for (int gh = 0; gh < H / 4; ++gh) {
                    f32x4_t d = vbw[gh];
#pragma unroll
                    for (int hh = 0; hh < H / 4; ++hh)
                        d = __builtin_amdgcn_mfma_f32_4x4x4f16(__builtin_bit_cast(flf16x4_t, Awp[gh][hh]), __builtin_bit_cast(flf16x4_t, bv[hh]), d, 0, 0, 0);
                    pp[r][gh] = d;
                }
            }
        };
        auto back_dv = [&](int i, f32x4_t (&pp)[4][H / 4], const uint32_t (&kb)[4]) {
            const unsigned char* sD16 = smem + 2 * STG + (i % NK16) * TILEB;
            fls16x4_t da[H][DT];
#pragma unroll
            for (int h = 0; h < ((FLB_DQAHEAD < H) ? FLB_DQAHEAD : H); ++h)
#pragma unroll
                for (int dt = 0; dt < DT; ++dt) da[h][dt] = *reinterpret_cast<const fls16x4_t*>(sD16 + h * REC + dt * 512 + lane * 8);
#pragma unroll
            for (int h = 0; h < H; ++h) {
                if (h + FLB_DQAHEAD < H) {
#pragma unroll
                    for (int dt = 0; dt < DT; ++dt) da[h + FLB_DQAHEAD][dt] = *reinterpret_cast<const fls16x4_t*>(sD16 + (h + FLB_DQAHEAD) * REC + dt * 512 + lane * 8);
                    __builtin_amdgcn_sched_barrier(FLB_SB_NOMEM);
                }
                float p4[4];
#pragma unroll
                for (int r = 0; r < 4; ++r) {
                    p4[r] = pp[r][h >> 2][h & 3];
                    if constexpr (DROP) p4[r] *= ((kb[r] >> ((h >> 1) * 8 + kbsh + (h & 1))) & 1u) ? keep_inv : 0.f;
                }
                const fls16x4_t pk = fl_pack4<false>(p4[0], p4[1], p4[2], p4[3]);
                flb_dq_mfma<DT>(dV[h], da[h], pk);
            }
        };
        auto d_flush = [&](int i) {
            constexpr int PER = 16 * H / NW;
            if (lane < PER) {
                const float* src = reinterpret_cast<const float*>(smem + DXOFF + (i & 1) * NW * DXB) + wave * PER + lane;
                float acc = src[0];
#pragma unroll
                for (int w = 1; w < NW; ++w) acc += (w < nvw) ? src[w * (DXB / 4)] : 0.f;
                a.ws_d[((long)bm * a.Np + (qt0 + i) * 16) * H + wave * PER + lane] = acc * (1.0f / FL_PD_SCALE);
            }
        };
        auto front = [&](int i, f32x4_t (&sp)[4][H / 4], f32x4_t (&dp)[4][H / 4], uint32_t (&kb)[4]) {
            load_kb(i, kb);
            Frags fa, fb;
            load_q(i, 0, fa);
            if constexpr (H > HB) load_q(i, HB, fb);
            front_q(i, std::integral_constant<int, 0>{}, fa, sp);
            load_d(i, 0, fa);
            if constexpr (H > HB) front_q(i, std::integral_constant<int, HB>{}, fb, sp);
            if constexpr (H > HB) load_d(i, HB, fb);
            front_d(i, std::integral_constant<int, 0>{}, fa, dp, kb);
            if constexpr (H > HB) front_d(i, std::integral_constant<int, HB>{}, fb, dp, kb);
        };
        auto back = [&](int i, f32x4_t (&sp)[4][H / 4], f32x4_t (&dp)[4][H / 4], const uint32_t (&kb)[4]) {
            f32x4_t pp[4][H / 4];
            back_exp(sp);
            back_ds(i, sp, dp);
            back_gw(i, sp, pp);
            back_dv(i, pp, kb);
        };
        auto step = [&](int i, f32x4_t (&sp)[4][H / 4], f32x4_t (&dp)[4][H / 4], f32x4_t (&spn)[4][H / 4], f32x4_t (&dpn)[4][H / 4], Frags& fr0, Frags& fr1,
                        const uint32_t (&kb)[4], uint32_t (&kbn)[4], bool more) {
            f32x4_t pp[4][H / 4];
            load_kb(i + 1, kbn);
            if constexpr (H > HB) load_q(i + 1, HB, fr1); else load_d(i + 1, 0, fr1);
            __builtin_amdgcn_sched_barrier(FLB_SB_NOMEM);
            front_q(i + 1, std::integral_constant<int, 0>{}, fr0, spn);
            back_exp(sp);
            FLB_PHASE();
            FLB_STAMP(3);
            if (FLB_STAGGER && more && wave >= NW / 2) issue_tiles(i + 2);
            constexpr bool RSF = FLB_RSFUSE && H == 2 * HB && FULL == 1 && TAIL16;
            f32x4_t rt[4], ro0, ro1;
            if constexpr (H > HB) {
                load_d(i + 1, 0, fr0);
                if constexpr (RSF) d_terms(0, sp, dp, rt);
                __builtin_amdgcn_sched_barrier(FLB_SB_NOMEM);
                if constexpr (RSF) front_q(i + 1, std::integral_constant<int, HB>{}, fr1, spn, &rt, &ro0);
                else front_q(i + 1, std::integral_constant<int, HB>{}, fr1, spn);
            }
            if constexpr (RSF) { d_store(i, 0, ro0); back_ds(i, sp, dp, false); d_terms(1, sp, dp, rt); }
            else back_ds(i, sp, dp);

            FLB_PHASE();
            FLB_STAMP(4);
            if constexpr (H > HB) {
                load_d(i + 1, HB, fr1);
                __builtin_amdgcn_sched_barrier(FLB_SB_NOMEM);
                if constexpr (RSF) { front_d(i + 1, std::integral_constant<int, 0>{}, fr0, dpn, kbn, &rt, &ro1); d_store(i, 1, ro1); }
                else front_d(i + 1, std::integral_constant<int, 0>{}, fr0, dpn, kbn);
            } else front_d(i + 1, std::integral_constant<int, 0>{}, fr1, dpn, kbn);
            back_gw(i, sp, pp);
            FLB_PHASE();
            FLB_STAMP(5);
            if constexpr (H > HB) front_d(i + 1, std::integral_constant<int, HB>{}, fr1, dpn, kbn);
            back_dv(i, pp, kb);
        };
        auto admit = [&](int nxt, bool late) {
            asm volatile("s_waitcnt vmcnt(0)" ::: "memory");
            __builtin_amdgcn_s_barrier();
            asm volatile("" ::: "memory");
            if (nxt + 1 < seg && !(late && wave >= NW / 2)) issue_tiles(nxt + 1);
        };

        f32x4_t spA[4][H / 4], dpA[4][H / 4], spB[4][H / 4], dpB[4][H / 4];
        uint32_t kbA[4], kbB[4];
        Frags frA, frB;
        issue_tiles(0);
        admit(0, false);
        if (wvalid) front(0, spA, dpA, kbA);
        for (int i = 0; i + 1 < seg; ++i) {
            FLB_STAMP(0);
            admit(i + 1, FLB_STAGGER && wvalid);
            FLB_STAMP(1);
            if (i > 0) d_flush(i - 1);
            FLB_STAMP(2);
            if (wvalid) {
                load_q(i + 1, 0, frA);
                step(i, spA, dpA, spB, dpB, frA, frB, kbA, kbB, i + 2 < seg);
#pragma unroll
                for (int r = 0; r < 4; ++r) {
                    kbA[r] = kbB[r];
#pragma unroll
                    for (int gh = 0; gh < H / 4; ++gh) { spA[r][gh] = spB[r][gh]; dpA[r][gh] = dpB[r][gh]; }
                }
            }
#ifdef FLB_DBG_STAMP
            FLB_STAMP(6);
            asm volatile("s_waitcnt lgkmcnt(0)" : "+s"(stamp[0]), "+s"(stamp[1]), "+s"(stamp[2]), "+s"(stamp[3]), "+s"(stamp[4]), "+s"(stamp[5]), "+s"(stamp[6]));
            for (int k = 0; k < 6; ++k) stacc[k] += stamp[k + 1] - stamp[k];
            ++stn;
#endif
        }
        if (wvalid) back(seg - 1, spA, dpA, kbA);
        __builtin_amdgcn_s_barrier();
        if (seg > 1) d_flush(seg - 2);
        d_flush(seg - 1);

        const int first_wg = (int)(((long)bm * nt) / a.spw);
        const int slot = (int)blockIdx.x - first_wg;
#pragma unroll
        for (int g = 0; g < H; ++g)
#pragma unroll
            for (int dt = 0; dt < DT; ++dt) flb_acc_fence(dV[g][dt]);
        if (wvalid) {
            float* dst = a.ws_v + (((long)bm * FL_MAXSLOT + slot) * NW + wave) * (long)(H * DT * 256);
#pragma unroll
            for (int g = 0; g < H; ++g)
#pragma unroll
                for (int dt = 0; dt < DT; ++dt) *reinterpret_cast<f32x4_t*>(dst + (g * DT + dt) * 256 + lane * 4) = dV[g][dt];
        }
        s += seg;
    }

#ifdef FLB_DBG_STAMP
    if (blockIdx.x == 0 && threadIdx.x == 0) {
        unsigned long long* o = reinterpret_cast<unsigned long long*>(a.ws_w);
        for (int k = 0; k < 6; ++k) o[k] = stacc[k];
        o[6] = stn;
    }
#endif
    {
        constexpr int NWG = 2 * (H * H + H);
        float* row = a.ws_w + ((long)blockIdx.x * NW + wave) * NWG + (H * H + H);
        const f32x4_t dsum = (gwacc[0] + gwacc[1]) + (gwacc[2] + gwacc[3]);
        const int nn = lane & 15;
#pragma unroll
        for (int r = 0; r < 4; ++r) {
            const int g = 4 * (lane >> 4) + r;
            if (g < H && nn < H) row[g * H + nn] = dsum[r] * (1.0f / FL_PD_SCALE);
            if (g < H && nn == H) row[H * H + g] = dsum[r];
        }
    }
}

__global__ __launch_bounds__(256) void bwdk_rows_merge_kernel(const float* __restrict__ ws, float* __restrict__ out, int B, int H, int N, int Np, int nmaj) {
    const long i = (long)blockIdx.x * 256 + threadIdx.x;
    const long per = (long)Np * H;
    if (i >= (long)B * per) return;
    const long bq = i / H; const int q = (int)(bq % Np), b = (int)(bq / Np);
    if (q >= N) { out[i] = 0.f; return; }
    const float* src = ws + (long)b * nmaj * per + (i - (long)b * per);
    float acc = 0.f;
    int m = 0;
    for (; m + 8 <= nmaj; m += 8) {
        float v[8];
#pragma unroll
        for (int k = 0; k < 8; ++k) v[k] = src[(long)(m + k) * per];
#pragma unroll
        for (int k = 0; k < 8; ++k) acc += v[k];
    }
    for (; m < nmaj; ++m) acc += src[(long)m * per];
    out[i] = acc;
}

constexpr int flbq_lds_bytes(int H, int DT, bool drop) {
    return (4 + FLB_NK16) * H * DT * 512 + 512 + FLB_NW * 3 * 4 * H * FLB_GWR + (drop ? 2048 : 0);
}
constexpr int flbk_lds_bytes(int H, int DT, bool drop) {
    return (4 + FLB_NK16) * H * DT * 512 + 2048 + 2 * FLB_NW * 16 * H * 4 + 512 + FLB_NW * 3 * 4 * H * FLB_GWR + (drop ? 2048 : 0);
}

static int dispatch_bwdq(const FlashBwdArgs& a, int H, int dh, int nwg, hipStream_t st) {
    return attn_dispatch(H, dh, [&](auto h, auto ds, auto tl) {
        constexpr int HH = decltype(h)::value, DS = decltype(ds)::value, DT = FragDims<DS, decltype(tl)::value>::DT;
        constexpr bool TL = decltype(tl)::value;
        if constexpr (flbq_lds_bytes(HH, DT, true) > FL_LDS_MAX) return -2;
        else return fl_launch<FlashBwdArgs, talking_bwdq_kernel<HH, DS, TL, true>, talking_bwdq_kernel<HH, DS, TL, false>>(
            a, nwg, 64 * FLB_NW, flbq_lds_bytes(HH, DT, false), flbq_lds_bytes(HH, DT, true), a.p_drop > 0.f, st);
    });
}

extern "C" int spe_talking_bwdq_plan(int B, int N, int nwg, int* steps_per_wg, int* nwg_used, int* nmajor) {
    const int nt = (N + 15) / 16;
    if ((long)B * nt <= 0 || nwg <= 0) { *steps_per_wg = 0; *nwg_used = 0; *nmajor = 0; return 0; }
    const FlashPlan p = fl_plan(B, nt, FLB_NW, nt, nwg);
    *steps_per_wg = p.spw; *nwg_used = p.nwg; *nmajor = p.nmaj;
    return 0;
}

static int bwdq_fill(FlashBwdArgs& a, FlashPlan& p, const void* Qf, const void* dOf, const void* Kf, const void* Vf, const void* K16, const float* Wl,
                     const float* Ww, const float* c0, int Np, const void* keepbits, int B, int H, int N, int dh, int nwg, float p_drop) {
    const int nt = (N + 15) / 16;
    if (dh < 1 || dh > 64 || nwg <= 0 || Np < nt * 16 || (p_drop > 0.f && !keepbits)) return -2;
    p = fl_plan(B, nt, FLB_NW, nt, nwg);
    a.Qf = (const unsigned char*)Qf; a.dOf = (const unsigned char*)dOf; a.Kf = (const unsigned char*)Kf; a.Vf = (const unsigned char*)Vf;
    a.K16 = (const unsigned char*)K16; a.Wl = Wl; a.Ww = Ww; a.c0 = c0; a.Np = Np; a.Drows = nullptr;
    a.ws_q = nullptr; a.ws_w = nullptr; a.dS = nullptr;
    a.keepbits = (p_drop > 0.f) ? reinterpret_cast<const unsigned*>(keepbits) : nullptr;
    a.B = B; a.N = N; a.nt = nt; a.nmaj = p.nmaj; a.spw = p.spw; a.total = p.total; a.p_drop = p_drop;
    return 0;
}


extern "C" int spe_talking_bwdq_pass2(const void* Qf, const void* dOf, const void* Kf, const void* Vf, const void* K16, const float* Wl, const float* Ww,
                                      const float* c0, const float* Drows, int Np, float* ws_q, float* ws_w, void* dS, float* dq, void* dq16,
                                      long ob, long on, long oh, float scale, const void* keepbits, int B, int H, int N, int dh, int nwg, float p_drop,
                                      hipStream_t st) {
    if ((long)B * ((N + 15) / 16) <= 0) return 0;
    FlashBwdArgs a; FlashPlan p;
    int rc = bwdq_fill(a, p, Qf, dOf, Kf, Vf, K16, Wl, Ww, c0, Np, keepbits, B, H, N, dh, nwg, p_drop);
    if (rc != 0) return rc;
    if (!ws_q || !ws_w || !dS || !Drows || !K16 || (!dq && !dq16)) return -2;
    a.ws_q = ws_q; a.ws_w = ws_w; a.dS = reinterpret_cast<unsigned short*>(dS); a.Drows = Drows;
    rc = dispatch_bwdq(a, H, dh, p.nwg, st);
    if (rc != 0) return rc;
    const int DT = frag_geom(dh).dt;
    const long nvec = (long)B * p.nmaj * FLB_NW * H * DT * 64;
    hipLaunchKernelGGL(bwdq_dq_merge_kernel, dim3((unsigned)((nvec + 255) / 256)), dim3(256), 0, st, ws_q, dq, reinterpret_cast<unsigned short*>(dq16),
                       ob, on, oh, B, H, N, a.nt, dh, DT, p.nmaj, p.spw, scale, nvec);
    SPE_CHECK_LAUNCH();
    return 0;
}

static int dispatch_bwdk(const FlashBwdKArgs& a, int H, int dh, int nwg, hipStream_t st) {
    return attn_dispatch(H, dh, [&](auto h, auto ds, auto tl) {
        constexpr int HH = decltype(h)::value, DS = decltype(ds)::value, DT = FragDims<DS, decltype(tl)::value>::DT;
        constexpr bool TL = decltype(tl)::value;
        if constexpr (flbk_lds_bytes(HH, DT, true) > FL_LDS_MAX) return -2;
        else return fl_launch<FlashBwdKArgs, talking_bwdk_kernel<HH, DS, TL, true>, talking_bwdk_kernel<HH, DS, TL, false>>(
            a, nwg, 64 * FLB_NW, flbk_lds_bytes(HH, DT, false), flbk_lds_bytes(HH, DT, true), a.p_drop > 0.f, st);
    });
}

extern "C" int spe_talking_fused_supported(int H, int dh) {
    return attn_dispatch(H, dh, [](auto h, auto ds, auto tl) {
        constexpr int HH = decltype(h)::value, DT = FragDims<decltype(ds)::value, decltype(tl)::value>::DT;
        return (flf_lds_bytes(HH, DT, true) <= FL_LDS_MAX && flbq_lds_bytes(HH, DT, true) <= FL_LDS_MAX && flbk_lds_bytes(HH, DT, true) <= FL_LDS_MAX) ? 0 : -2;
    }) == 0;
}

extern "C" int spe_talking_bwdk_pass1(const void* Qf, const void* dOf, const void* dO16, const void* Kf, const void* Vf, const float* Wl, const float* Ww,
                                      const float* bw, const float* c0, int Np, float* ws_d, float* ws_v, float* ws_w, float* Drows, float* dv, void* dv16,
                                      long ob, long on, long oh, const void* keepbits, int B, int H, int N, int dh, int nwg, float p_drop, hipStream_t st) {
    const int nt = (N + 15) / 16;
    if ((long)B * nt <= 0) return 0;
    if (dh < 1 || dh > 64 || nwg <= 0 || Np < nt * 16 + 64 || (p_drop > 0.f && !keepbits)) return -2;
    if (!Qf || !dOf || !dO16 || !Kf || !Vf || !Wl || !Ww || !bw || !c0 || !ws_d || !ws_v || !ws_w || !Drows || (!dv && !dv16)) return -2;
    const FlashPlan p = fl_plan(B, nt, FLB_NW, nt, nwg);
    FlashBwdKArgs a;
    a.Qf = (const unsigned char*)Qf; a.dOf = (const unsigned char*)dOf; a.dO16 = (const unsigned char*)dO16;
    a.Kf = (const unsigned char*)Kf; a.Vf = (const unsigned char*)Vf; a.Wl = Wl; a.Ww = Ww; a.bw = bw; a.c0 = c0; a.Np = Np;
    a.ws_d = ws_d; a.ws_v = ws_v; a.ws_w = ws_w;
    a.keepbits = (p_drop > 0.f) ? reinterpret_cast<const unsigned*>(keepbits) : nullptr;
    a.B = B; a.N = N; a.nt = nt; a.nmaj = p.nmaj; a.spw = p.spw; a.total = p.total; a.p_drop = p_drop;
    int rc = dispatch_bwdk(a, H, dh, p.nwg, st);
    if (rc != 0) return rc;
    const long n = (long)B * Np * H;
    hipLaunchKernelGGL(bwdk_rows_merge_kernel, dim3((unsigned)((n + 255) / 256)), dim3(256), 0, st, ws_d, Drows, B, H, N, Np, p.nmaj);
    SPE_CHECK_LAUNCH();
    const int DT = frag_geom(dh).dt;
    const long nvec = (long)B * p.nmaj * FLB_NW * H * DT * 64;
    hipLaunchKernelGGL(bwdq_dq_merge_kernel, dim3((unsigned)((nvec + 255) / 256)), dim3(256), 0, st, ws_v, dv, reinterpret_cast<unsigned short*>(dv16),
                       ob, on, oh, B, H, N, nt, dh, DT, p.nmaj, p.spw, 1.0f / FL_PD_SCALE, nvec);
    SPE_CHECK_LAUNCH();
    return 0;
}
```

### spe_amd/csrc/attn_flash_common.h

```cpp
#pragma once
#include <type_traits>
#include "attn_pack.h"

typedef unsigned int flu32x4_t __attribute__((ext_vector_type(4)));
typedef unsigned int flu32x2_t __attribute__((ext_vector_type(2)));
typedef short fls16x4_t __attribute__((ext_vector_type(4)));
typedef _Float16 flf16x4_t __attribute__((ext_vector_type(4)));
typedef _Float16 flf16x8_t __attribute__((ext_vector_type(8)));
typedef __bf16 flbf16x4_t __attribute__((ext_vector_type(4)));

#define FL_PD_SCALE 256.0f
#define FL_LOG2E 1.4426950408889634f
#define FL_LN2 0.6931471805599453f
#define FL_MAXSLOT 8

__device__ __forceinline__ float fl_exp2(float x) { return __builtin_amdgcn_exp2f(x); }

__device__ __forceinline__ _Float16 fl_f2h_sat(float f) { return (_Float16)((f != f) ? f : __builtin_amdgcn_fmed3f(f, -65504.f, 65504.f)); }

template <bool F16>
__device__ __forceinline__ fls16x4_t fl_pack4(float a, float b, float c, float d) {
    if constexpr (F16) {
        flf16x4_t v;
        v[0] = fl_f2h_sat(a); v[1] = fl_f2h_sat(b); v[2] = fl_f2h_sat(c); v[3] = fl_f2h_sat(d);
        return __builtin_bit_cast(fls16x4_t, v);
    } else {
        flbf16x4_t v; v[0] = (__bf16)a; v[1] = (__bf16)b; v[2] = (__bf16)c; v[3] = (__bf16)d;
        return __builtin_bit_cast(fls16x4_t, v);
    }
}

__device__ __forceinline__ fls16x4_t fl_pack4_f16(float a, float b, float c, float d) {
    flf16x4_t v; v[0] = (_Float16)a; v[1] = (_Float16)b; v[2] = (_Float16)c; v[3] = (_Float16)d;
    return __builtin_bit_cast(fls16x4_t, v);
}

template <int H, bool TRANSPOSE>
__device__ __forceinline__ void fl_mixA_f32(const float* __restrict__ W, int lane, float (&A)[H / 4][H]) {
#pragma unroll
    for (int gh = 0; gh < H / 4; ++gh)
#pragma unroll
        for (int h = 0; h < H; ++h) {
            const int go = 4 * gh + (lane & 3);
            A[gh][h] = TRANSPOSE ? W[h * H + go] : W[go * H + h];
        }
}
template <int H>
__device__ __forceinline__ void fl_mix_f32(const f32x4_t (&s)[H], const float (&A)[H / 4][H], const f32x4_t (&c)[4][H / 4], f32x4_t (&out)[4][H / 4]) {
#pragma unroll
    for (int r = 0; r < 4; ++r)
#pragma unroll
        for (int gh = 0; gh < H / 4; ++gh) {
            f32x4_t d = c[r][gh];
#pragma unroll
            for (int h = 0; h < H; ++h) d = __builtin_amdgcn_mfma_f32_4x4x1f32(A[gh][h], s[h][r], d, 0, 0, 0);
            out[r][gh] = d;
        }
}

template <int H, bool TRANSPOSE, bool F16>
__device__ __forceinline__ void fl_mixA_16(const float* __restrict__ W, int lane, float wscale, fls16x4_t (&A)[H / 4][H / 4]) {
#pragma unroll
    for (int gh = 0; gh < H / 4; ++gh)
#pragma unroll
        for (int hh = 0; hh < H / 4; ++hh) {
            float v[4];
#pragma unroll
            for (int k = 0; k < 4; ++k) {
                const int go = 4 * gh + (lane & 3), hi = 4 * hh + k;
                v[k] = wscale * (TRANSPOSE ? W[hi * H + go] : W[go * H + hi]);
            }
            A[gh][hh] = fl_pack4<F16>(v[0], v[1], v[2], v[3]);
        }
}
template <int H, bool F16>
__device__ __forceinline__ void fl_mix_16(const float (&x)[H], const fls16x4_t (&A)[H / 4][H / 4], const f32x4_t* init, f32x4_t (&out)[H / 4]) {
    fls16x4_t bv[H / 4];
#pragma unroll
    for (int hh = 0; hh < H / 4; ++hh) bv[hh] = fl_pack4<F16>(x[4 * hh], x[4 * hh + 1], x[4 * hh + 2], x[4 * hh + 3]);
#pragma unroll
    for (int gh = 0; gh < H / 4; ++gh) {
        f32x4_t d = init ? init[gh] : (f32x4_t){0.f, 0.f, 0.f, 0.f};
#pragma unroll
        for (int hh = 0; hh < H / 4; ++hh) {
            if constexpr (F16) d = __builtin_amdgcn_mfma_f32_4x4x4f16(__builtin_bit_cast(flf16x4_t, A[gh][hh]), __builtin_bit_cast(flf16x4_t, bv[hh]), d, 0, 0, 0);
            else d = __builtin_amdgcn_mfma_f32_4x4x4bf16_1k(A[gh][hh], bv[hh], d, 0, 0, 0);
        }
        out[gh] = d;
    }
}

__device__ __forceinline__ void fl_glds16(const void* gsrc, unsigned lds_dst) {
    unsigned keep;
    asm volatile("s_mov_b32 %0, m0\n\ts_mov_b32 m0, %2\n\ts_nop 0\n\tglobal_load_lds_dwordx4 %1, off\n\ts_mov_b32 m0, %0"
                 : "=&s"(keep) : "v"(gsrc), "s"(lds_dst) : "memory");
}

__device__ __forceinline__ void fl_glds16_s(const void* sbase, unsigned voff, unsigned lds_dst) {
    unsigned keep;
    asm volatile("s_mov_b32 %0, m0\n\ts_mov_b32 m0, %3\n\ts_nop 0\n\tglobal_load_lds_dwordx4 %1, %2\n\ts_mov_b32 m0, %0"
                 : "=&s"(keep) : "v"(voff), "s"(sbase), "s"(lds_dst) : "memory");
}
template <int CNT, int STRIDE>
__device__ __forceinline__ void fl_glds16_run(const void* sbase, const unsigned* voff, unsigned lds_dst) {
    static_assert(CNT >= 1 && CNT <= 4, "pieces per wave and tile");
    if constexpr (CNT == 1)
        asm volatile("s_mov_b32 m0, %1\n\ts_nop 0\n\tglobal_load_lds_dwordx4 %2, %0"
                     :: "s"(sbase), "s"(lds_dst), "v"(voff[0]) : "memory");
    else if constexpr (CNT == 2)
        asm volatile("s_mov_b32 m0, %1\n\ts_nop 0\n\tglobal_load_lds_dwordx4 %2, %0\n\ts_add_u32 m0, m0, %4\n\ts_nop 0\n\tglobal_load_lds_dwordx4 %3, %0"
                     :: "s"(sbase), "s"(lds_dst), "v"(voff[0]), "v"(voff[1]), "n"(STRIDE) : "memory", "scc");
    else if constexpr (CNT == 3)
        asm volatile("s_mov_b32 m0, %1\n\ts_nop 0\n\tglobal_load_lds_dwordx4 %2, %0\n\ts_add_u32 m0, m0, %5\n\ts_nop 0\n\tglobal_load_lds_dwordx4 %3, %0\n\t"
                     "s_add_u32 m0, m0, %5\n\ts_nop 0\n\tglobal_load_lds_dwordx4 %4, %0"
                     :: "s"(sbase), "s"(lds_dst), "v"(voff[0]), "v"(voff[1]), "v"(voff[2]), "n"(STRIDE) : "memory", "scc");
    else
        asm volatile("s_mov_b32 m0, %1\n\ts_nop 0\n\tglobal_load_lds_dwordx4 %2, %0\n\ts_add_u32 m0, m0, %6\n\ts_nop 0\n\tglobal_load_lds_dwordx4 %3, %0\n\t"
                     "s_add_u32 m0, m0, %6\n\ts_nop 0\n\tglobal_load_lds_dwordx4 %4, %0\n\ts_add_u32 m0, m0, %6\n\ts_nop 0\n\tglobal_load_lds_dwordx4 %5, %0"
                     :: "s"(sbase), "s"(lds_dst), "v"(voff[0]), "v"(voff[1]), "v"(voff[2]), "v"(voff[3]), "n"(STRIDE) : "memory", "scc");
}

template <int DSTEPS, bool TAIL16>
__device__ __forceinline__ flu32x4_t fl_frag_global(const flu32x4_t* __restrict__ base, long rec, int st, int lane) {
    constexpr int FULL = FragDims<DSTEPS, TAIL16>::FULL, REC8 = FragDims<DSTEPS, TAIL16>::REC / 8;
    const uint2* p = reinterpret_cast<const uint2*>(base) + rec * REC8;
    if (TAIL16 && st == FULL) {
        const uint2 v = p[FULL * 128 + lane];
        return (flu32x4_t){v.x, v.y, 0u, 0u};
    }
    return *reinterpret_cast<const flu32x4_t*>(p + st * 128 + lane * 2);
}
template <int DSTEPS, bool TAIL16>
__device__ __forceinline__ flu32x4_t fl_frag_lds(const unsigned char* rec, int st, int lane) {
    constexpr int FULL = FragDims<DSTEPS, TAIL16>::FULL;
    if (TAIL16 && st == FULL) {
        const flu32x2_t v = *reinterpret_cast<const flu32x2_t*>(rec + FULL * 1024 + lane * 8);
        return (flu32x4_t){v[0], v[1], 0u, 0u};
    }
    return *reinterpret_cast<const flu32x4_t*>(rec + st * 1024 + lane * 16);
}
template <bool F16>
__device__ __forceinline__ f32x4_t fl_mfma32(flu32x4_t a, flu32x4_t b, f32x4_t c) {
    if constexpr (F16) return __builtin_amdgcn_mfma_f32_16x16x32_f16(__builtin_bit_cast(flf16x8_t, a), __builtin_bit_cast(flf16x8_t, b), c, 0, 0, 0);
    else return __builtin_amdgcn_mfma_f32_16x16x32_bf16(__builtin_bit_cast(bf16x8_t, a), __builtin_bit_cast(bf16x8_t, b), c, 0, 0, 0);
}
template <bool F16>
__device__ __forceinline__ f32x4_t fl_mfma16(fls16x4_t a, fls16x4_t b, f32x4_t c) {
    if constexpr (F16) return __builtin_amdgcn_mfma_f32_16x16x16f16(__builtin_bit_cast(flf16x4_t, a), __builtin_bit_cast(flf16x4_t, b), c, 0, 0, 0);
    else return __builtin_amdgcn_mfma_f32_16x16x16bf16_1k(a, b, c, 0, 0, 0);
}

struct FlashPlan { int nmaj, nstream, spw, nwg; long total; };
__host__ __device__ static inline FlashPlan fl_plan(int B, int nt_major, int per_major, int nstream, int nwg_max) {
    FlashPlan p;
    p.nmaj = (nt_major + per_major - 1) / per_major;
    p.nstream = nstream;
    p.total = (long)B * p.nmaj * nstream;
    long spw = (p.total + nwg_max - 1) / nwg_max;
    const long min_spw = (nstream + (FL_MAXSLOT - 2)) / (FL_MAXSLOT - 1);
    if (spw < min_spw) spw = min_spw;
    if (spw < 1) spw = 1;
    p.spw = (int)spw;
    p.nwg = (int)((p.total + spw - 1) / spw);
    return p;
}

template <int H>
__device__ __forceinline__ void fl_keep_lots(uint64_t seed, uint64_t offset, int b, int hp, int q, int key0, int N, uint32_t (&o)[4]) {
    const uint64_t ctr = (((uint64_t)b * (H / 2) + hp) * (uint64_t)N + (uint64_t)q) * (uint64_t)((N + 3) >> 2) + (uint64_t)(key0 >> 2);
    spe_philox4((uint32_t)ctr, (uint32_t)(ctr >> 32), (uint32_t)offset, (uint32_t)(offset >> 32), (uint32_t)seed, (uint32_t)(seed >> 32), o);
}
__device__ __forceinline__ uint32_t fl_lot(const uint32_t (&o)[4], int head, int i) {
    const uint32_t w = o[2 * head + (i >> 1)];
    return (i & 1) ? (w >> 16) : (w & 0xffffu);
}

__device__ __forceinline__ uint32_t fl_quad_bcast(uint32_t v, int t) {
    switch (t) {
        case 0: return (uint32_t)__builtin_amdgcn_update_dpp(0, (int)v, 0x00, 0xf, 0xf, false);
        case 1: return (uint32_t)__builtin_amdgcn_update_dpp(0, (int)v, 0x55, 0xf, 0xf, false);
        case 2: return (uint32_t)__builtin_amdgcn_update_dpp(0, (int)v, 0xaa, 0xf, 0xf, false);
        default: return (uint32_t)__builtin_amdgcn_update_dpp(0, (int)v, 0xff, 0xf, 0xf, false);
    }
}

template <int H, typename F>
static int attn_dispatch_h(int dh, F&& f) {
    const FragGeom g = frag_geom(dh);
    using HC = std::integral_constant<int, H>;
    using D1 = std::integral_constant<int, 1>;
    using D2 = std::integral_constant<int, 2>;
    if (g.dsteps == 2) return g.tail ? f(HC{}, D2{}, std::true_type{}) : f(HC{}, D2{}, std::false_type{});
    return g.tail ? f(HC{}, D1{}, std::true_type{}) : f(HC{}, D1{}, std::false_type{});
}
template <typename F>
static int attn_dispatch(int H, int dh, F&& f) {
    if (dh < 1 || dh > 64) return -2;
    if (H == 8) return attn_dispatch_h<8>(dh, f);
    if (H == 4) return attn_dispatch_h<4>(dh, f);
    return -2;
}

#define FL_LDS_MAX (160 * 1024)
template <typename Args, void (*KDROP)(Args), void (*KPLAIN)(Args)>
static int fl_launch(const Args& a, int nwg, int threads, int lds_plain, int lds_drop, bool drop, hipStream_t st) {
    static bool attr_set[2] = {false, false};
    void (*const fn)(Args) = drop ? KDROP : KPLAIN;
    const int smem = drop ? lds_drop : lds_plain;
    if (!attr_set[drop]) {
        hipError_t e = hipFuncSetAttribute(reinterpret_cast<const void*>(fn), hipFuncAttributeMaxDynamicSharedMemorySize, smem);
        if (e != hipSuccess) return (int)e;
        attr_set[drop] = true;
    }
    hipLaunchKernelGGL(fn, dim3(nwg), dim3(threads), smem, st, a);
    SPE_CHECK_LAUNCH();
    return 0;
}
#define FLF_MAJ 8
constexpr int flf_lds_bytes(int H, int DT, bool ) { return (5 + FLF_MAJ) * H * DT * 512; }
```

### spe_amd/kernels.py

```python
import collections
import ctypes
import os
import weakref

import torch

from . import lib

_PRECISION = 2
import functools as _functools
import threading as _threading

_TLS = _threading.local()


def _in_bwd():
    return getattr(_TLS, "in_bwd", False)


def backward_scope(fn):
    @_functools.wraps(fn)
    def wrapped(ctx, *grads):
        prev, _TLS.in_bwd = _in_bwd(), True
        if _DEFER_FLATS is not None and not _FLUSH_QUEUED[0]:
# ... 911 lines not shown
    R, C = dout2.shape
    dy = torch.empty_like(dout2)
    dg = _zeros_or(dg_out, C, dout2.device)
    _call("spe_layerscale_residual_bwd", _p(dout2), _p(y2), _p(gamma), _p(sample_scale), _p(dy), _p(dg), R, C,
             rows_per_sample, _st())
    return dy, dg


def dropout(x, p, seed, offset):
    _chk(x)
    y = torch.empty_like(x)
    _call("spe_dropout", _p(x), _p(y), x.numel(), float(p), seed, offset, _st())
    return y


def pad4(n):
    return (n + 3) // 4 * 4


def softmax_fwd(S, mask_u8, B, H, Nq, Nk, ld, p_drop, seed, offset):
    Pd = torch.empty_like(S) if p_drop > 0 else None
    _call("spe_softmax_fwd", _p(S), _p(mask_u8), _p(S), _p(Pd), B, H, Nq, Nk, ld, float(p_drop), seed, offset, _st())
    return S, Pd


def softmax_bwd(dPd, P, B, H, Nq, Nk, ld, p_drop, seed, offset):
    _call("spe_softmax_bwd", _p(dPd), _p(P), _p(dPd), B, H, Nq, Nk, ld, float(p_drop), seed, offset, _st())
    return dPd


def talking_fwd(S, Wl, bl, Ww, bw, B, H, Nq, Nk, ld, p_drop, seed, offset):
    Pd = torch.empty_like(S)
    _call("spe_talking_softmax_fwd", _p(S), _p(Wl), _p(bl), _p(Ww), _p(bw), _p(S), _p(Pd), B, H, Nq, Nk, ld,
             float(p_drop), seed, offset, _st())
    return S, Pd


def talking_bwd(dPd, P, S, Wl, Ww, B, H, Nq, Nk, ld, p_drop, seed, offset):
    nblocks = min(B * Nq, 1024)
    nw = 2 * (H * H + H)
    ws = torch.empty((nblocks, nw), device=dPd.device, dtype=torch.float32)
    _call("spe_talking_softmax_bwd", _p(dPd), _p(P), _p(S), _p(Wl), _p(Ww), _p(dPd), _p(ws), nblocks, B, H, Nq, Nk, ld,
             float(p_drop), seed, offset, _st())
    g = colsum(ws)
    hh = H * H
    return dPd, g[:hh].view(H, H), g[hh:hh + H], g[hh + H:2 * hh + H].view(H, H), g[2 * hh + H:]


def patchify(img, P):
    _chk(img)
    B, Cin, Hi, Wi = img.shape
    h, w = Hi // P, Wi // P
    cols = torch.empty((B * h * w, Cin * P * P), device=img.device, dtype=torch.float32)
    _call("spe_patchify", _p(img), _p(cols), B, Cin, Hi, Wi, P, _st())
    return cols


def add_rows(a, table):
    _chk(a, table)
    out = torch.empty_like(a)
    _call("spe_add_rows", _p(a), _p(table), _p(out), a.numel(), table.numel(), _st())
    return out


def matcher_cost(logits, boxes, tgt_ids_i32, tgt_boxes, toff_i32, total_targets, w_class, w_bbox, w_giou):
    _chk(logits, boxes, tgt_boxes)
    L, B, Q, Kc = logits.shape
    cost = torch.empty((L, Q * total_targets), device=logits.device, dtype=torch.float32)
    err = torch.zeros((1,), device=logits.device, dtype=torch.int32)
    _call("spe_matcher_cost", _p(logits), _p(boxes), _p(tgt_ids_i32), _p(tgt_boxes), _p(toff_i32), total_targets,
             _p(cost), _p(err), L, B, Q, Kc, float(w_class), float(w_bbox), float(w_giou), _st())
    return cost, err


def hungarian(cost, toff_i32, L, B, Q, total_targets, err=None):
    dev = cost.device
    srow = torch.empty((L * total_targets,), device=dev, dtype=torch.int64)
    gidx = torch.empty_like(srow)
    lidx = torch.empty((L * total_targets,), device=dev, dtype=torch.int32)
    _call("spe_hungarian", _p(cost), _p(toff_i32), _p(srow), _p(gidx), _p(lidx), _p(err), L, B, Q, _st())
    return srow, gidx, lidx


def focal_loss(logits, tclass_i32, roww, alpha, gamma):
    _chk(logits, roww)
    L, R, Kc = logits.shape
    grad = torch.empty_like(logits)
    loss = torch.zeros((L,), device=logits.device, dtype=torch.float32)
    amax = torch.empty((L, R), device=logits.device, dtype=torch.int32)
    _call("spe_focal_loss", _p(logits), _p(tclass_i32), _p(roww), _p(grad), _p(loss), _p(amax), L, R, Kc,
             float(alpha), float(gamma), _st())
    return loss, grad, amax


def box_loss(pred_boxes, srow_i64, tbox, w, lidx_i32, L):
    _chk(pred_boxes, tbox, w)
    n = srow_i64.numel()
    sums = torch.zeros((L, 2), device=pred_boxes.device, dtype=torch.float32)
    g1 = torch.empty((n, 4), device=pred_boxes.device, dtype=torch.float32)
    g2 = torch.empty_like(g1)
    _call("spe_box_loss", _p(pred_boxes), _p(srow_i64), _p(tbox), _p(w), _p(lidx_i32), _p(sums), _p(g1), _p(g2), n, int(L), _st())
    return sums, g1, g2


def box_loss_bwd(srow_i64, lidx_i32, g1, g2, c1, c2, shape):
    dpred = torch.zeros(shape, device=g1.device, dtype=torch.float32)
    _call("spe_box_loss_bwd", _p(srow_i64), _p(lidx_i32), _p(g1), _p(g2), _p(c1), _p(c2), _p(dpred), srow_i64.numel(), _st())
    return dpred


STATS_NWG = 512
_STATS_NWG_SOLO = STATS_NWG


def set_cu_reserve(n):
    global _CU_RESERVE, STATS_NWG
    _CU_RESERVE = int(n)
    STATS_NWG = max(8, (_STATS_NWG_SOLO - int(n)) & ~7) if n > 0 else _STATS_NWG_SOLO


_CU_RESERVE = 0


def get_cu_reserve():
    return _CU_RESERVE


@_functools.lru_cache(maxsize=None)
def fused_supported(H, dh):
    return bool(lib.load().spe_talking_fused_supported(H, dh))


LOG2E = 1.4426950408889634


def attn_pack(x4, scale=1.0):
    _chk(x4)
    B, N, H, dh = x4.shape
    nt = (N + 15) // 16
    out = torch.empty((B, H, nt, frag_record_elems(dh)), device=x4.device, dtype=torch.bfloat16)
    _call("spe_attn_pack", _p(x4), x4.stride(0), x4.stride(1), x4.stride(2), B, N, H, dh, float(scale), _p(out), _st())
    return out


_PLANS = {}


def fused_plan(B, N):
    key = ("stats", B, N, STATS_NWG)
    r = _PLANS.get(key)
    if r is None:
        spw, nwg = ctypes.c_int(0), ctypes.c_int(0)
        lib.call("spe_talking_stats_plan", B, N, STATS_NWG, ctypes.byref(spw), ctypes.byref(nwg))
        r = _PLANS[key] = (spw.value, nwg.value)
    return r


STATS_SLOTS = 8


def talking_stats(Qf, Kf, Wl, bl, ws_stats, B, H, N, dh):
    _call("spe_talking_stats", _p(Qf), _p(Kf), _p(Wl), _p(bl), _p(ws_stats), B, H, N, dh, STATS_NWG, _st())


def score_blocks(B, H, N, device, dtype=torch.bfloat16):
    nt = (N + 15) // 16
    return torch.empty((B, H, nt, nt, 64, 4), device=device, dtype=dtype)


def attn_pack16(x4):
    B, N, H, dh = x4.shape
    assert x4.stride(3) == 1
    nt, DT = (N + 15) // 16, (dh + 15) // 16
    out = torch.empty((B, H, nt, DT, 64, 4), device=x4.device, dtype=torch.bfloat16)
    _call("spe_attn_pack16", _p(x4), x4.stride(0), x4.stride(1), x4.stride(2), B, N, H, dh, _p(out), _st())
    return out


def frag_record_elems(dh):
    rem = dh % 32
    full = dh // 32 + (1 if rem > 16 else 0)
    return full * 512 + (256 if 0 < rem <= 16 else 0)


F16 = 1000


def attn_pack_multi(jobs):
    B, _, H, _ = jobs[0][0].shape
    n = len(jobs)
    outs = []
    for x4, scale, kind in jobs:
        Bn, N, Hn, dh = x4.shape
        assert Bn == B and Hn == H and x4.stride(3) == 1 and x4.dtype == torch.float32
        nt = (N + 15) // 16
        if kind % F16 == 32:
            shape = (B, H, nt, frag_record_elems(dh))
        elif kind % F16 == 322:
            shape = (B, H, nt, (dh + 31) // 32, 64, 8)
        else:
            shape = (B, H, nt, (dh + 15) // 16, 64, 4)
        outs.append(torch.empty(shape, device=x4.device, dtype=torch.float16 if kind >= F16 else torch.bfloat16))
    xs = (ctypes.c_void_p * n)(*[j[0].data_ptr() for j in jobs])
    strides = (ctypes.c_long * (3 * n))(*[s for j in jobs for s in (j[0].stride(0), j[0].stride(1), j[0].stride(2))])
    scales = (ctypes.c_float * n)(*[float(j[1]) for j in jobs])
    kinds = (ctypes.c_int * n)(*[{32: 0, 16: 1, 322: 2}[j[2] % F16] + (16 if j[2] >= F16 else 0) for j in jobs])
    optr = (ctypes.c_void_p * n)(*[o.data_ptr() for o in outs])
    Ns = (ctypes.c_int * n)(*[j[0].shape[1] for j in jobs])
    dhs = (ctypes.c_int * n)(*[j[0].shape[3] for j in jobs])
    _call("spe_attn_pack_multi", n, xs, strides, scales, kinds, optr, Ns, dhs, B, H, _st())
    return outs


def mha_plan(B, H, Lq, Lk):
    nch = ctypes.c_int(0)
    lib.call("spe_mha_plan", B, H, Lq, Lk, ctypes.byref(nch))
    return nch.value


def mha_fwd(Qf, Kf, V16, mask_u8, B, H, Lq, Lk, dk, dv, nch, p_drop, seed, offset):
    dev = Qf.device
    ntq, ntk, dvt = (Lq + 15) // 16, (Lk + 15) // 16, (dv + 15) // 16
    items = B * H * ntq * nch
    opart = torch.empty((items, dvt, 64, 4), device=dev, dtype=torch.float32)
    ml = torch.empty((items, 16, 2), device=dev, dtype=torch.float32)
    O = torch.empty((B, Lq, H * dv), device=dev, dtype=torch.float32)
    lse = torch.empty((B, H, Lq), device=dev, dtype=torch.float32)
    keep = torch.empty((B * H * ntq * ntk * 4,), device=dev, dtype=torch.int64) if p_drop > 0 else None
    _call("spe_mha_fwd", _p(Qf), _p(Kf), _p(V16), _p(mask_u8), _p(opart), _p(ml), _p(O), _p(lse), _p(keep), B, H, Lq, Lk, dk, dv,
          nch, float(p_drop), seed, offset, _st())
    return O, lse, keep


def mha_bwd(Qf, Kf, Vf, dOf, K16, Q16, dO16, mask_u8, lse, D, keep, B, H, Lq, Lk, dk, dv, nch, scale, p_drop):
    dev = Qf.device
    dq = torch.empty((B, Lq, H, dk), device=dev, dtype=torch.float32)
    ws = torch.empty((nch, dq.numel()), device=dev, dtype=torch.float32) if nch > 1 else None
    dk_ = torch.empty((B, Lk, H, dk), device=dev, dtype=torch.float32)
    dv_ = torch.empty((B, Lk, H, dv), device=dev, dtype=torch.float32)
    _call("spe_mha_bwd", _p(Qf), _p(Kf), _p(Vf), _p(dOf), _p(K16), _p(Q16), _p(dO16), _p(mask_u8), _p(lse), _p(D), _p(keep), _p(dq),
          _p(ws), _p(dk_), _p(dv_), B, H, Lq, Lk, dk, dv, nch, float(scale), float(p_drop), _st())
    if ws is not None:
        colsum(ws, out=dq.view(-1), accumulate=False)
    return dq, dk_, dv_


def rowdot(x4, y4):
    _chk(x4, y4)
    B, L, H, dh = x4.shape
    D = torch.empty((B, H, L), device=x4.device, dtype=torch.float32)
    _call("spe_rowdot", _p(x4), _p(y4), _p(D), B, L, H, dh, _st())
    return D


_CONTRACT_WS = {}


def _contract_ws(device):
    ent = _CONTRACT_WS.get(device)
    if ent is None:
        ent = (torch.empty(256 * 4 * 4 * 256, device=device, dtype=torch.float32),
               torch.zeros(1024, device=device, dtype=torch.int32))
        _CONTRACT_WS[device] = ent
    return ent


def attn_contract(T, X16, out4, trans, alpha=1.0, out16=None, out16lo=None):
    ref = out4 if out4 is not None else out16
    B, N, H, dh = ref.shape
    assert ref.stride(3) == 1
    tf, xf = T.dtype == torch.float16, X16.dtype == torch.float16
    fmt = {(False, False): 0, (True, True): 1, (True, False): 2}[(tf, xf)]
    ws, cnt = _contract_ws(ref.device)
    _call("spe_attn_contract", _p(T), _p(X16), _p(out4), ref.stride(0), ref.stride(1), ref.stride(2), B, H, N, dh,
          int(trans), fmt, float(alpha), _p(ws), _p(cnt), ws.numel(), _p(out16), _p(out16lo), _st())
    return ref


FLASH_NWG = 256
FLASH_SLOTS = 8


def flash_plan(B, N):
    key = ("flash", B, N, FLASH_NWG)
    r = _PLANS.get(key)
    if r is None:
        spw, nwg, nmaj, npad = ctypes.c_int(0), ctypes.c_int(0), ctypes.c_int(0), ctypes.c_int(0)
        lib.call("spe_talking_flash_plan", B, N, FLASH_NWG, ctypes.byref(spw), ctypes.byref(nwg), ctypes.byref(nmaj), ctypes.byref(npad))
        r = _PLANS[key] = (spw.value, nwg.value, nmaj.value, npad.value)
    return r


_FLASH_WS = {}


def _flash_ws(device, floats):
    ent = _FLASH_WS.get(device)
    if ent is None or ent.numel() < floats:
        ent = torch.empty((floats,), device=device, dtype=torch.float32)
        _FLASH_WS[device] = ent
    return ent


def talking_flash_fwd(Qf, Kf, V16, Wl, Ww, bw, c0, B, H, N, dh, p_drop, seed, offset, want16=False, want16lo=False, want_bits=False):
    dev = Qf.device
    nmaj = flash_plan(B, N)[2]
    ws = _flash_ws(dev, B * nmaj * FLASH_SLOTS * 128 * H * 16 * ((dh + 15) // 16))
    C = H * dh
    O = torch.empty((B, N, C), device=dev, dtype=torch.float32)
    O16 = torch.empty((B * N, C), device=dev, dtype=torch.bfloat16) if want16 else None
    O16lo = torch.empty((B * N, C), device=dev, dtype=torch.bfloat16) if (want16 and want16lo) else None
    nt = (N + 15) // 16
    bits = torch.empty((B, nt, nt, 64), device=dev, dtype=torch.int32) if (want_bits and p_drop > 0) else None
    _call("spe_talking_flash_fwd", _p(Qf), _p(Kf), _p(V16), _p(Wl), _p(Ww), _p(bw), _p(c0), c0.shape[1], _p(ws), _p(O), _p(O16), _p(O16lo),
          _p(bits), B, H, N, dh, FLASH_NWG, float(p_drop), seed, offset, _st())
    if want_bits:
        return O, O16, O16lo, bits
    return O, O16, O16lo


def bwdq_plan(B, N):
    budget = max(8, FLASH_NWG - _CU_RESERVE)
    key = ("bwdq", B, N, budget)
    r = _PLANS.get(key)
    if r is None:
        spw, nwg, nmaj = ctypes.c_int(0), ctypes.c_int(0), ctypes.c_int(0)
        lib.call("spe_talking_bwdq_plan", B, N, budget, ctypes.byref(spw), ctypes.byref(nwg), ctypes.byref(nmaj))
        if len(_PLANS) > 256:
            _PLANS.clear()
        r = _PLANS[key] = (spw.value, nwg.value, nmaj.value)
    return r


def talking_bwdk_pass1(Qf, dOf, dO16, Kf, Vf, Wl, Ww, bw, c0, keepbits, dv4, dv16, B, H, N, dh, p_drop):
    ref = dv4 if dv4 is not None else dv16
    assert ref.stride(3) == 1 and (dv4 is None or dv16 is None or dv4.stride() == dv16.stride())
    dev = Qf.device
    _, nwg, nmaj = bwdq_plan(B, N)
    Np = c0.shape[1]
    ws_d = torch.empty((B * nmaj, Np, H), device=dev, dtype=torch.float32)
    ws_v = _flash_ws(dev, B * nmaj * FLASH_SLOTS * 4 * H * 256 * ((dh + 15) // 16))
    ws_w = torch.empty((4 * nwg, 2 * (H * H + H)), device=dev, dtype=torch.float32)
    Drows = torch.empty((B, Np, H), device=dev, dtype=torch.float32)
    _call("spe_talking_bwdk_pass1", _p(Qf), _p(dOf), _p(dO16), _p(Kf), _p(Vf), _p(Wl), _p(Ww), _p(bw), _p(c0), Np, _p(ws_d), _p(ws_v), _p(ws_w),
          _p(Drows), _p(dv4), _p(dv16), ref.stride(0), ref.stride(1), ref.stride(2), _p(keepbits), B, H, N, dh, max(8, FLASH_NWG - _CU_RESERVE),
          float(p_drop), _st())
    return Drows, ws_w


def talking_bwdq_pass2(Qf, dOf, Kf, Vf, K16, Wl, Ww, c0, Drows, ws_w, dS, dq4, dq16, scale, keepbits, B, H, N, dh, p_drop):
    ref = dq4 if dq4 is not None else dq16
    assert ref.stride(3) == 1 and (dq4 is None or dq16 is None or dq4.stride() == dq16.stride())
    nmaj = bwdq_plan(B, N)[2]
    ws_q = _flash_ws(ref.device, B * nmaj * FLASH_SLOTS * 4 * H * 256 * ((dh + 15) // 16))
    _call("spe_talking_bwdq_pass2", _p(Qf), _p(dOf), _p(Kf), _p(Vf), _p(K16), _p(Wl), _p(Ww), _p(c0), _p(Drows), c0.shape[1], _p(ws_q), _p(ws_w),
          _p(dS), _p(dq4), _p(dq16), ref.stride(0), ref.stride(1), ref.stride(2), float(scale), _p(keepbits), B, H, N, dh,
          max(8, FLASH_NWG - _CU_RESERVE), float(p_drop), _st())


def attn_merge_rows(ws_stats, bl, B, H, N, spw):
    Np = flash_plan(B, N)[3]
    M = torch.empty((B, H, N), device=ws_stats.device, dtype=torch.float32)
    IL = torch.empty_like(M)
    c0 = torch.empty((B, Np, H), device=ws_stats.device, dtype=torch.float32)
    _call("spe_attn_merge_rows", _p(ws_stats), _p(M), _p(IL), _p(bl), _p(c0), Np, B, H, N, spw, _st())
    return M, IL, c0


def talking_row_constants(Qf, Kf, Wl, bl, B, H, N, dh):
    ws_stats = torch.empty((B * ((N + 15) // 16) * STATS_SLOTS * H * 16 * 2,), device=Qf.device, dtype=torch.float32)
    talking_stats(Qf, Kf, Wl, bl, ws_stats, B, H, N, dh)
    return attn_merge_rows(ws_stats, bl, B, H, N, fused_plan(B, N)[0])


def attn_pmean(Qf, Kf, Wl, c0, M, alpha, B, H, N, dh):
    _call("spe_attn_pmean", _p(Qf), _p(Kf), _p(Wl), _p(c0), c0.shape[1], _p(M), float(alpha), B, H, N, dh, _st())


def attn_pmean_dense(P, M, alpha, B, H, N, ld):
    _call("spe_attn_pmean_dense", _p(P), _p(M), float(alpha), B, H, N, ld, _st())


def bmm_f32(A, B):
    _chk(A, B)
    Bt, M, Kd = A.shape
    N = B.shape[2]
    C = torch.empty((Bt, M, N), device=A.device, dtype=torch.float32)
    _call("spe_gemm_f32", _p(A), _p(B), _p(C), None, None, M, N, Kd, Kd, N, N, 0, 0, Bt, 1, M * Kd, 0, Kd * N, 0, M * N, 0,
          1.0, 0, 1, 1, _st())
    return C


def conv_head_fwd(x3, W, b, h, w):
    _chk(x3, W, b)
    B, hw, C = x3.shape
    Kc = W.shape[0]
    assert hw == h * w and x3.is_contiguous() and W.is_contiguous() and b.is_contiguous()
    m = torch.empty((B, Kc, h, w), device=x3.device, dtype=torch.float32)
    lg = torch.empty((B, Kc), device=x3.device, dtype=torch.float32)
    _call("spe_conv_head_fwd", _p(x3), _p(W), _p(b), _p(m), _p(lg), B, h, w, C, Kc, _st())
    return m, lg


def conv_head_bwd(x3, W, dmap, dlogits, h, w, need_dx=True, dW_out=None, db_out=None):
    _chk(x3, W, dmap, dlogits)
    B, hw, C = x3.shape
    Kc = W.shape[0]
    n = ctypes.c_long(0)
    lib.call("spe_conv_head_plan", B, h, w, C, Kc, ctypes.byref(n))
    ws = torch.empty((n.value,), device=x3.device, dtype=torch.float32)
    dx = torch.empty_like(x3) if need_dx else None
    dW = dW_out.view(W.shape) if dW_out is not None else torch.empty_like(W)
    db = db_out.view(-1) if db_out is not None else torch.empty((Kc,), device=x3.device, dtype=torch.float32)
    _call("spe_conv_head_bwd", _p(x3), _p(W), _p(dmap), _p(dlogits), _p(dx), _p(dW), _p(db), _p(ws), n.value, B, h, w, C, Kc, _st())
    return dx, dW, db


def jitter_pick(box, scale, ratio):
    _chk(box, scale)
    M, ncand = scale.shape[0], scale.shape[1]
    out = torch.empty((M, ratio, 4), device=box.device, dtype=torch.float32)
    _call("spe_jitter_pick", _p(box), _p(scale), _p(out), M, ncand, int(ratio), _st())
    return out


def talking_wgrad_reduce(ws_w, H, params):
    shapes = ((H, H), (H,), (H, H), (H,))
    outs = []
    for prm, shp in zip(params, shapes):
        buf = grad_buffer(prm) if prm is not None else None
        outs.append(buf.view(shp) if buf is not None else torch.empty(shp, device=ws_w.device, dtype=torch.float32))
    _call("spe_talking_wgrad_reduce", _p(ws_w), ws_w.shape[0], H, _p(outs[0]), _p(outs[1]), _p(outs[2]), _p(outs[3]), _st())
    return outs


def gemm_bf16a(A16, B, C, M, N, K, lda, ldb, ldc, transA, transB, batch0, batch1, sA, sB, sC, alpha=1.0):
    _call("spe_gemm_ex", _p(A16), 1, _p(B), _p(C), None, None, M, N, K, lda, ldb, ldc, int(transA), int(transB), batch0, batch1,
          sA[0], sA[1], sB[0], sB[1], sC[0], sC[1], float(alpha), 0, 1, 0, _st())
    return C


def bicubic(src, gh, gw, h, w, backward=False):
    _chk(src)
    C = src.shape[-1]
    if backward:
        out = torch.zeros((gh * gw, C), device=src.device, dtype=torch.float32)
    else:
        out = torch.empty((h * w, C), device=src.device, dtype=torch.float32)
    _call("spe_bicubic", _p(src), _p(out), gh, gw, h, w, C, int(backward), _st())
    return out


def sqnorm_partials(g_flat, partials):
    _call("spe_sqnorm_partials", _p(g_flat), g_flat.numel(), _p(partials), partials.numel(), _st())


def adamw_flat(p, g, m, v, seg_end_i64, seg_lr, seg_wd, beta1, beta2, eps, bias_c1, bias_c2, partials, max_norm, write_grad,
               grad_scale=1.0):
    _call("spe_adamw_flat", _p(p), _p(g), _p(m), _p(v), p.numel(), _p(seg_end_i64), _p(seg_lr), _p(seg_wd), seg_end_i64.numel(),
          float(beta1), float(beta2), float(eps), float(bias_c1), float(bias_c2), _p(partials), partials.numel(),
          float(max_norm), int(bool(write_grad)), float(grad_scale), _st())


ADAMW_GUARD_WORDS = 16
GUARD_APPLIED, GUARD_SKIPPED, GUARD_FIRST, GUARD_APPLY, GUARD_CLIP, GUARD_BC1, GUARD_BC2SQRT, GUARD_NORM, GUARD_STEP_F = range(9)


def adamw_gate(guard_i32, partials, max_norm, grad_scale, beta1, beta2):
    _call("spe_adamw_gate", _p(guard_i32), _p(partials), partials.numel(), float(max_norm), float(grad_scale), float(beta1),
          float(beta2), _st())


def adamw_flat_guarded(p, g, m, v, seg_end_i64, seg_lr, seg_wd, beta1, beta2, eps, guard_i32, write_grad):
    _call("spe_adamw_flat_guarded", _p(p), _p(g), _p(m), _p(v), p.numel(), _p(seg_end_i64), _p(seg_lr), _p(seg_wd), seg_end_i64.numel(),
          float(beta1), float(beta2), float(eps), _p(guard_i32), int(bool(write_grad)), _st())


def adamw_flat_ema(p, g, m, v, e, seg_end_i64, seg_lr, seg_wd, beta1, beta2, eps, write_grad, decay, warmup, guard_i32=None, bias_c1=1.0,
                   bias_c2=1.0, partials=None, max_norm=0.0, grad_scale=1.0, t=0):
    _call("spe_adamw_flat_ema", _p(p), _p(g), _p(m), _p(v), _p(e), p.numel(), _p(seg_end_i64), _p(seg_lr), _p(seg_wd), seg_end_i64.numel(),
          float(beta1), float(beta2), float(eps), float(bias_c1), float(bias_c2), _p(partials), 0 if partials is None else partials.numel(),
          float(max_norm), int(bool(write_grad)), float(grad_scale), _p(guard_i32), float(decay), int(bool(warmup)), int(t), _st())


GRAD_REPORT_WORDS = 8
REPORT_GRAD_SQ, REPORT_GRAD_ABSMAX, REPORT_WEIGHT_SQ, REPORT_WEIGHT_ABSMAX, REPORT_NAN, REPORT_INF, REPORT_FIRST_BAD, REPORT_ATTEMPT = range(8)


def grad_report(g, p, par_beg, par_len, grad_scale, out, guard_i32=None, when=0):
    _chk(g, p)
    npar = par_beg.numel()
    if par_beg.dtype != torch.int64 or par_len.dtype != torch.int64 or par_len.numel() != npar:
        raise ValueError("grad_report: par_beg and par_len are int64 tables of equal length")
    if out.dtype != torch.int32 or out.numel() != npar * GRAD_REPORT_WORDS or not out.is_contiguous():
        raise ValueError("grad_report: out is a contiguous int32 tensor of GRAD_REPORT_WORDS words per parameter")
    if p is not None and p.numel() != g.numel():
        raise ValueError("grad_report: g and p must have the same number of elements")
    _call("spe_grad_report", _p(g), _p(p), g.numel(), _p(par_beg), _p(par_len), npar, float(grad_scale), _p(guard_i32), int(when),
          _p(out), _st())
    return out


def swap_flat(a, b):
    _chk(a, b)
    if a.numel() != b.numel() or not (a.is_contiguous() and b.is_contiguous()):
        raise ValueError("swap_flat: two contiguous buffers with the same number of elements")
    _call("spe_swap_flat", _p(a), _p(b), a.numel(), _st())


def accum_flat(dst, a, b=None):
    _chk(dst, a, b)
    n = dst.numel()
    if a.numel() != n or (b is not None and b.numel() != n):
        raise ValueError("accum_flat: dst, a and b must have the same number of elements")
    if not (dst.is_contiguous() and a.is_contiguous() and (b is None or b.is_contiguous())):
        raise ValueError("accum_flat: contiguous buffers only")
    _call("spe_accum_flat", _p(dst), _p(a), _p(b), n, _st())
    return dst


def nms_sorted(boxes, labels, iou_threshold, counts=None):
    _chk(boxes)
    I, n, _ = boxes.shape
    assert labels.dtype == torch.int64 and labels.is_contiguous()
    keep = torch.empty((I, n), device=boxes.device, dtype=torch.uint8)
    _call("spe_nms_sorted", _p(boxes), _p(labels), _p(counts), _p(keep), I, n, float(iou_threshold), _st())
    return keep.bool()


DETECT_MAX_K, DETECT_MAX_N = 1024, 1 << 20


def detect(logits, boxes, sizes, k, iou_threshold, nms=True, out=None):
    _chk(logits, boxes, sizes)
    B, Q, Kc = logits.shape
    N, k = Q * Kc, int(k)
    if k < 1 or k > N:
        raise ValueError(f"detect: k = {k} out of range for {N} = {Q} x {Kc} scores per image")
    if k > DETECT_MAX_K or N > DETECT_MAX_N:
        raise ValueError(f"detect: at most k = {DETECT_MAX_K} of at most {DETECT_MAX_N} scores per image (k = {k}, Q * Kc = {N})")
    if boxes.shape != (B, Q, 4) or sizes.shape != (B, 2):
        raise ValueError(f"detect: boxes {tuple(boxes.shape)} / sizes {tuple(sizes.shape)} do not fit logits {tuple(logits.shape)}")
    if not (logits.is_contiguous() and boxes.is_contiguous() and sizes.is_contiguous()):
        raise ValueError("detect: contiguous tensors only")
    dev = logits.device
    if out is None:
        out = (torch.empty((B, k), device=dev, dtype=torch.float32), torch.empty((B, k), device=dev, dtype=torch.int64),
               torch.empty((B, k, 4), device=dev, dtype=torch.float32), torch.empty((B, k), device=dev, dtype=torch.int32),
               torch.empty((B,), device=dev, dtype=torch.int32))
    logit, label, box, query, count = out
    want = (((B, k), torch.float32), ((B, k), torch.int64), ((B, k, 4), torch.float32), ((B, k), torch.int32), ((B,), torch.int32))
    for t, (shape, dt) in zip(out, want):
        if tuple(t.shape) != shape or t.dtype != dt or t.device != dev or not t.is_contiguous():
            raise ValueError("detect: `out` must be the five contiguous buffers of an earlier call with the same B and k")
    _call("spe_detect", _p(logits), _p(boxes), _p(sizes), B, Q, Kc, k, float(iou_threshold), 1 if nms else 0, _p(logit), _p(label),
          _p(box), _p(query), _p(count), _st())
    return logit, label, box, query, count


def cam_prepare(maps, rows, cols, cam_thr):
    _chk(maps)
    M, h, w = maps.shape
    out = torch.empty((M, rows, cols), device=maps.device, dtype=torch.uint8)
    mm = torch.empty((2 * M,), device=maps.device, dtype=torch.float32)
    _call("spe_cam_prepare", _p(maps), M, h, w, rows, cols, float(cam_thr), _p(mm), _p(out), _st())
    return out


def cam_contour_boxes(img_u8_host, area_ratio, max_boxes=256):
    assert img_u8_host.device.type == "cpu" and img_u8_host.dtype == torch.uint8 and img_u8_host.is_contiguous()
    rows, cols = img_u8_host.shape
    boxes = torch.empty((max_boxes, 4), dtype=torch.int32)
    n = ctypes.c_int(0)
    lib.call("spe_cam_contour_boxes", ctypes.c_void_p(img_u8_host.data_ptr()), rows, cols, float(area_ratio),
             ctypes.c_void_p(boxes.data_ptr()), max_boxes, ctypes.byref(n))
    return boxes[:n.value].clone()


CAM_MAX_BOXES = 2048


def cam_boxes_workspace_bytes(M, rows, cols):
    n = ctypes.c_size_t(0)
    lib.call("spe_cam_boxes_device_workspace", M, rows, cols, ctypes.byref(n))
    return n.value


def cam_boxes_device_packed(imgs_u8_device, area_ratio, max_boxes=256):
    t = imgs_u8_device
    if not t.is_cuda:
        raise lib.SpeLibraryError("spe_amd kernels run on the GPU only (got a CPU tensor); there is no CPU fallback")
    assert t.dtype == torch.uint8 and t.dim() == 3 and t.is_contiguous()
    M, rows, cols = t.shape
    out = torch.empty((M * (1 + 4 * max_boxes),), device=t.device, dtype=torch.int32)
    if M:
        nbytes = cam_boxes_workspace_bytes(M, rows, cols)
        ws = torch.empty((nbytes // 4,), device=t.device, dtype=torch.int32)
        _call("spe_cam_boxes_device", _p(t), M, rows, cols, float(area_ratio), _p(ws), nbytes, _p(out[M:]), _p(out), max_boxes, _st())
    return out


def cam_boxes_device(imgs_u8_device, area_ratio, max_boxes=256):
    M = imgs_u8_device.shape[0]
    out = cam_boxes_device_packed(imgs_u8_device, area_ratio, max_boxes)
    return out[M:].view(M, max_boxes, 4), out[:M]


CAM_TARGETS_MAX_M = 65535


def cam_targets(packed, cls0, max_boxes, single, W, H, cap=None, out=None):
    if not (packed.is_cuda and cls0.is_cuda):
        raise lib.SpeLibraryError("spe_amd kernels run on the GPU only (got a CPU tensor); there is no CPU fallback")
    M = cls0.numel()
    if packed.dtype != torch.int32 or cls0.dtype != torch.int32 or not (packed.is_contiguous() and cls0.is_contiguous()):
        raise TypeError("cam_targets: contiguous int32 tables only")
    if packed.numel() != M * (1 + 4 * max_boxes):
        raise ValueError(f"cam_targets: {packed.numel()} packed words do not hold {M} maps of {max_boxes} boxes")
    if cap is None:
        cap = M * (1 if single else max_boxes)
    if out is None:
        out = (torch.empty((cap, 4), device=packed.device, dtype=torch.float32), torch.empty((cap,), device=packed.device, dtype=torch.int64),
               torch.empty((M + 1,), device=packed.device, dtype=torch.int32))
    boxes, labels, off = out
    _check_typed("cam_targets", ((boxes, torch.float32), (labels, torch.int64), (off, torch.int32)))
    if boxes.numel() < 4 * cap or labels.numel() < cap or off.numel() < M + 1:
        raise ValueError("cam_targets: `out` is smaller than cap rows / M + 1 offsets")
    _call("spe_cam_targets", _p(packed), _p(cls0), M, int(max_boxes), 1 if single else 0, int(W), int(H), int(cap), _p(boxes), _p(labels),
          _p(off), _st())
    return boxes, labels, off


def refine_pick(prob, pred_boxes, cls, cls_off, host=None, out=None):
    _chk(prob, pred_boxes)
    B, Q, Kc = prob.shape
    U = cls.numel()
    if pred_boxes.shape != (B, Q, 4) or cls_off.numel() != B + 1:
        raise ValueError(f"refine_pick: boxes {tuple(pred_boxes.shape)} / {cls_off.numel()} offsets do not fit prob {tuple(prob.shape)}")
    _check_typed("refine_pick", ((cls, torch.int32), (cls_off, torch.int32)))
    if not (prob.is_contiguous() and pred_boxes.is_contiguous()):
        raise ValueError("refine_pick: contiguous tensors only")
    dev = prob.device
    if out is None:
        out = (torch.empty((U,), device=dev, dtype=torch.float32), torch.empty((U,), device=dev, dtype=torch.int32),
               torch.empty((U, 4), device=dev, dtype=torch.float32))
    scores, queries, boxes = out
# ... 332 lines not shown
```

Baseline: 42.47 images/sec.

## Save fp16 attention probabilities in flash forward and reuse them in bwdk pass

Adds an optional forward path that writes the post-mix attention probabilities as fp16 blocks to global memory, plus a backward dK/dV pass variant that streams those saved blocks into LDS in place of recomputing QK^T, the talking-head logit mix and the softmax from Q, K and row stats. This swaps recomputation in backward for a large extra write in forward and a read in backward (B*nt*nt*256*H halves, about 275 MB at N=4150, H=8). The Python wrappers expose want_p and P16 arguments. The visible changes do not show any caller setting them, so the default path may be unchanged. The inline-asm clobber lists also gain m0.

New measurement: 41.98 images/sec. -1.2%, worse.

```diff
diff --git a/include/spe_hip.h b/include/spe_hip.h
--- a/include/spe_hip.h
+++ b/include/spe_hip.h
@@ -103,10 +103,16 @@
 int spe_talking_flash_fwd(const void* Qf, const void* Kf, const void* V16, const float* Wl, const float* Ww, const float* bw,
                           const float* c0, int Np, float* ws, float* O, void* O16, void* O16lo, void* keepbits, int B, int H, int N, int dh,
                           int nwg, float p_drop, uint64_t seed, uint64_t offset, spe_stream_t stream);
+int spe_talking_flash_fwd_p(const void* Qf, const void* Kf, const void* V16, const float* Wl, const float* Ww, const float* bw,
+                            const float* c0, int Np, float* ws, float* O, void* O16, void* O16lo, void* keepbits, void* P16, int B, int H, int N,
+                            int dh, int nwg, float p_drop, uint64_t seed, uint64_t offset, spe_stream_t stream);
 
 int spe_talking_bwdk_pass1(const void* Qf, const void* dOf, const void* dO16, const void* Kf, const void* Vf, const float* Wl, const float* Ww,
                            const float* bw, const float* c0, int Np, float* ws_d, float* ws_v, float* ws_w, float* Drows, float* dv, void* dv16,
                            long ob, long on, long oh, const void* keepbits, int B, int H, int N, int dh, int nwg, float p_drop, spe_stream_t stream);
+int spe_talking_bwdk_pass1_p(const void* P16, const void* dOf, const void* dO16, const void* Vf, const float* Ww, const float* bw, int Np,
+                             float* ws_d, float* ws_v, float* ws_w, float* Drows, float* dv, void* dv16, long ob, long on, long oh,
+                             const void* keepbits, int B, int H, int N, int dh, int nwg, float p_drop, spe_stream_t stream);
 int spe_talking_bwdq_plan(int B, int N, int nwg, int* steps_per_wg, int* nwg_used, int* nmajor);
 int spe_talking_bwdq_pass2(const void* Qf, const void* dOf, const void* Kf, const void* Vf, const void* K16, const float* Wl, const float* Ww,
                            const float* c0, const float* Drows, int Np, float* ws_q, float* ws_w, void* dS, float* dq, void* dq16,
diff --git a/spe_amd/csrc/attn_flash.hip b/spe_amd/csrc/attn_flash.hip
--- a/spe_amd/csrc/attn_flash.hip
+++ b/spe_amd/csrc/attn_flash.hip
@@ -9,13 +9,14 @@
     int B, N, nt, nmaj, spw; long total;
     float p_drop; uint64_t seed, offset;
     unsigned* keepbits;
+    unsigned char* p16;
 };
 
 #define FLF_NW 8
 #define FLF_HB 4
 #define FLF_QS (FLF_MAJ / FLF_NW)
 
-template <int H, int DSTEPS, bool TAIL16, bool DROP>
+template <int H, int DSTEPS, bool TAIL16, bool DROP, bool SAVEP>
 __global__ __launch_bounds__(64 * FLF_NW, FLF_NW / 4) void talking_flash_fwd_kernel(FlashFwdArgs a) {
     constexpr int FULL = FragDims<DSTEPS, TAIL16>::FULL, DT = FragDims<DSTEPS, TAIL16>::DT, REC = FragDims<DSTEPS, TAIL16>::REC;
     constexpr int NW = FLF_NW, QS = FLF_QS;
@@ -44,6 +45,7 @@
         const int o = (i * NW + wave) * 1024 + lane * 16;
         voff[i] = (unsigned)((o / REC) * nt * REC + o % REC);
     }
+    const unsigned p_off0 = (unsigned)((lane >> 4) * 32 * H + (((lane & 15) ^ (4 * (lane >> 4))) * 2 * H));
 
     const long s_begin = (long)blockIdx.x * a.spw;
     long s_end = s_begin + a.spw; if (s_end > a.total) s_end = a.total;
@@ -162,6 +164,29 @@
                 __builtin_amdgcn_sched_barrier(0);
             }
             if (grp != 0) step_barrier(i + 1);
+            if constexpr (SAVEP) {
+#pragma unroll
+                for (int u = 0; u < QS; ++u) {
+                    if (qt0 + u >= nt) continue;
+                    unsigned char* pb = a.p16 + (((long)b * nt + (qt0 + u)) * nt + (kt0 + i)) * (long)(512 * H);
+                    const bool qok = qrow[u] < N;
+                    const int key0 = (kt0 + i) * 16 + 4 * (lane >> 4);
+#pragma unroll
+                    for (int r = 0; r < 4; ++r) {
+                        const bool ok = qok && key0 + r < N;
+                        unsigned char* dst = pb + ((p_off0 ^ (unsigned)(r * 2 * H)) + (unsigned)(r * 128 * H));
+                        if constexpr (H == 8) {
+                            const flu32x2_t lo = __builtin_bit_cast(flu32x2_t, bv[u][r][0]), hi = __builtin_bit_cast(flu32x2_t, bv[u][r][1]);
+                            const flu32x4_t w = ok ? (flu32x4_t){lo[0], lo[1], hi[0], hi[1]} : (flu32x4_t){0u, 0u, 0u, 0u};
+                            __builtin_nontemporal_store(w, reinterpret_cast<flu32x4_t*>(dst));
+                        } else {
+                            static_assert(H == 4 || H == 8, "one 2 H byte chunk per (query, key)");
+                            const flu32x2_t lo = __builtin_bit_cast(flu32x2_t, bv[u][r][0]);
+                            __builtin_nontemporal_store(ok ? lo : (flu32x2_t){0u, 0u}, reinterpret_cast<flu32x2_t*>(dst));
+                        }
+                    }
+                }
+            }
 #pragma unroll
             for (int u = 0; u < QS; ++u) {
                 f32x4_t pr[4][H / 4];
@@ -277,11 +302,11 @@
     }
 }
 
-template <int H, int DSTEPS, bool TAIL16>
+template <int H, int DSTEPS, bool TAIL16, bool SAVEP>
 static int launch_flash_fwd(const FlashFwdArgs& a, int nwg, bool drop, hipStream_t st) {
     constexpr int DT = FragDims<DSTEPS, TAIL16>::DT;
     if constexpr (flf_lds_bytes(H, DT, true) > FL_LDS_MAX) return -2;
-    else return fl_launch<FlashFwdArgs, talking_flash_fwd_kernel<H, DSTEPS, TAIL16, true>, talking_flash_fwd_kernel<H, DSTEPS, TAIL16, false>>(
+    else return fl_launch<FlashFwdArgs, talking_flash_fwd_kernel<H, DSTEPS, TAIL16, true, SAVEP>, talking_flash_fwd_kernel<H, DSTEPS, TAIL16, false, SAVEP>>(
         a, nwg, 64 * FLF_NW, flf_lds_bytes(H, DT, false), flf_lds_bytes(H, DT, true), drop, st);
 }
 
@@ -293,9 +318,9 @@
     return 0;
 }
 
-extern "C" int spe_talking_flash_fwd(const void* Qf, const void* Kf, const void* V16, const float* Wl, const float* Ww, const float* bw,
-                                     const float* c0, int Np, float* ws, float* O, void* O16, void* O16lo, void* keepbits, int B, int H, int N,
-                                     int dh, int nwg, float p_drop, uint64_t seed, uint64_t offset, hipStream_t st) {
+static int flash_fwd_run(const void* Qf, const void* Kf, const void* V16, const float* Wl, const float* Ww, const float* bw,
+                         const float* c0, int Np, float* ws, float* O, void* O16, void* O16lo, void* keepbits, void* P16, int B, int H, int N,
+                         int dh, int nwg, float p_drop, uint64_t seed, uint64_t offset, hipStream_t st) {
     const int nt = (N + 15) / 16;
     if ((long)B * nt <= 0) return 0;
     if (dh < 1 || dh > 64 || nwg <= 0 || (O16lo && !O16) || Np < nt * 16 + 64) return -2;
@@ -305,9 +330,11 @@
     a.Wl = Wl; a.Ww = Ww; a.bw = bw; a.c0 = c0; a.Np = Np; a.ws_o = ws;
     a.B = B; a.N = N; a.nt = nt; a.nmaj = p.nmaj; a.spw = p.spw; a.total = p.total;
     a.p_drop = p_drop; a.seed = seed; a.offset = offset; a.keepbits = reinterpret_cast<unsigned*>(p_drop > 0.f ? keepbits : nullptr);
+    a.p16 = reinterpret_cast<unsigned char*>(P16);
     const bool drop = p_drop > 0.f;
     const int rc = attn_dispatch(H, dh, [&](auto h, auto ds, auto tl) {
-        return launch_flash_fwd<decltype(h)::value, decltype(ds)::value, decltype(tl)::value>(a, p.nwg, drop, st); });
+        if (P16) return launch_flash_fwd<decltype(h)::value, decltype(ds)::value, decltype(tl)::value, true>(a, p.nwg, drop, st);
+        return launch_flash_fwd<decltype(h)::value, decltype(ds)::value, decltype(tl)::value, false>(a, p.nwg, drop, st); });
     if (rc != 0) return rc;
     const int DT = frag_geom(dh).dt;
     const long nvec = (long)B * p.nmaj * FLF_MAJ * H * DT * 64;
@@ -316,3 +343,16 @@
     SPE_CHECK_LAUNCH();
     return 0;
 }
+
+extern "C" int spe_talking_flash_fwd(const void* Qf, const void* Kf, const void* V16, const float* Wl, const float* Ww, const float* bw,
+                                     const float* c0, int Np, float* ws, float* O, void* O16, void* O16lo, void* keepbits, int B, int H, int N,
+                                     int dh, int nwg, float p_drop, uint64_t seed, uint64_t offset, hipStream_t st) {
+    return flash_fwd_run(Qf, Kf, V16, Wl, Ww, bw, c0, Np, ws, O, O16, O16lo, keepbits, nullptr, B, H, N, dh, nwg, p_drop, seed, offset, st);
+}
+
+extern "C" int spe_talking_flash_fwd_p(const void* Qf, const void* Kf, const void* V16, const float* Wl, const float* Ww, const float* bw,
+                                       const float* c0, int Np, float* ws, float* O, void* O16, void* O16lo, void* keepbits, void* P16, int B, int H,
+                                       int N, int dh, int nwg, float p_drop, uint64_t seed, uint64_t offset, hipStream_t st) {
+    if (!P16) return -2;
+    return flash_fwd_run(Qf, Kf, V16, Wl, Ww, bw, c0, Np, ws, O, O16, O16lo, keepbits, P16, B, H, N, dh, nwg, p_drop, seed, offset, st);
+}
diff --git a/spe_amd/csrc/attn_flash_bwd.hip b/spe_amd/csrc/attn_flash_bwd.hip
--- a/spe_amd/csrc/attn_flash_bwd.hip
+++ b/spe_amd/csrc/attn_flash_bwd.hip
@@ -535,6 +535,7 @@
     const unsigned* keepbits;
     int B, N, nt, nmaj, spw; long total;
     float p_drop;
+    const unsigned char* P16;
 };
 
 __device__ __forceinline__ void flb_rowsum4(const f32x4_t (&t)[4], f32x4_t& o) {
@@ -635,23 +636,25 @@
 
 
 
-template <int H, int DSTEPS, bool TAIL16, bool DROP>
+template <int H, int DSTEPS, bool TAIL16, bool DROP, bool SAVEDP>
 __global__ __launch_bounds__(64 * FLB_NW, 1) void talking_bwdk_kernel(FlashBwdKArgs a) {
     constexpr int FULL = FragDims<DSTEPS, TAIL16>::FULL, DT = FragDims<DSTEPS, TAIL16>::DT, REC = FragDims<DSTEPS, TAIL16>::REC;
     constexpr int NW = FLB_NW, HB = (H >= FLB_HB) ? FLB_HB : H;
     constexpr int TILEB = H * REC;
-    constexpr int STG = 2 * TILEB;
+    constexpr int PB = 512 * H;
+    constexpr int S0 = SAVEDP ? NW * PB : TILEB;
+    constexpr int STG = S0 + TILEB;
     constexpr int NK16 = FLB_NK16;
     constexpr int F1 = FULL ? FULL : 1;
     extern __shared__ __attribute__((aligned(16))) unsigned char smem[];
     const int lane = threadIdx.x & 63, wave = __builtin_amdgcn_readfirstlane(threadIdx.x >> 6);
     const unsigned lds0 = __builtin_amdgcn_readfirstlane((unsigned)(uintptr_t)(__attribute__((address_space(3))) unsigned char*)smem);
     const int nt = a.nt;
-    constexpr int C0OFF = 2 * STG + NK16 * TILEB, DXB = 16 * H * 4, DXOFF = C0OFF + 2048, GCOFF = DXOFF + 2 * NW * DXB;
+    constexpr int C0OFF = 2 * STG + NK16 * TILEB, DXB = 16 * H * 4, DXOFF = C0OFF + (SAVEDP ? 0 : 2048), GCOFF = DXOFF + 2 * NW * DXB;
     constexpr int KBOFF = GCOFF + 512 + NW * 3 * (4 * H * FLB_GWR);
 
     float Al4[H / 4][H];
-    fl_mixA_f32<H, false>(a.Wl, lane, Al4);
+    if constexpr (!SAVEDP) fl_mixA_f32<H, false>(a.Wl, lane, Al4);
     fls16x4_t Awt[H / 4][H / 4];
     fl_mixA_16<H, true, false>(a.Ww, lane, 1.0f, Awt);
     fls16x4_t Awp[H / 4][H / 4];
@@ -682,6 +685,10 @@
         const int o = (i * NW + wave) * 1024 + lane * 16;
         voff[i] = (unsigned)((o / REC) * nt * REC + o % REC);
     }
+    unsigned pvoff[PB / 1024];
+#pragma unroll
+    for (int i = 0; i < PB / 1024; ++i) pvoff[i] = (unsigned)(i * 1024 + lane * 16);
+    const unsigned p_rd0 = (unsigned)((gm & 3) * 128 * H + (gm >> 2) * 32 * H + ((4 * gk) ^ gm) * 2 * H);
     const float keep_inv = DROP ? 1.0f / (1.0f - a.p_drop) : 1.0f;
     const int kbsh = 2 * (gm & 3);
 #ifdef FLB_DBG_STAMP
@@ -714,11 +721,11 @@
             const unsigned char* vb_ = a.Vf + (((long)b * H + h) * nt + ktc) * REC;
 #pragma unroll
             for (int st = 0; st < FULL; ++st) {
-                ka[h][st] = *reinterpret_cast<const flu32x4_t*>(kb_ + st * 1024 + lane * 16);
+                if constexpr (!SAVEDP) ka[h][st] = *reinterpret_cast<const flu32x4_t*>(kb_ + st * 1024 + lane * 16);
                 va[h][st] = *reinterpret_cast<const flu32x4_t*>(vb_ + st * 1024 + lane * 16);
             }
             if constexpr (TAIL16) {
-                kta[h] = *reinterpret_cast<const flu32x2_t*>(kb_ + FULL * 1024 + lane * 8);
+                if constexpr (!SAVEDP) kta[h] = *reinterpret_cast<const flu32x2_t*>(kb_ + FULL * 1024 + lane * 8);
                 vta[h] = *reinterpret_cast<const flu32x2_t*>(vb_ + FULL * 1024 + lane * 8);
             } else { kta[h] = (flu32x2_t){0u, 0u}; vta[h] = (flu32x2_t){0u, 0u}; }
         }
@@ -734,11 +741,13 @@
 #else
             const int qt = qt0 + i;
 #endif
-#pragma unroll
-            for (int op = 0; op < 3; ++op) {
+            if constexpr (SAVEDP)
+                fl_glds16_run<PB / 1024, 1024>(a.P16 + (((long)b * nt + qt) * nt + ktc) * (long)PB, pvoff, lds0 + (i & 1) * STG + wave * PB);
+#pragma unroll
+            for (int op = SAVEDP ? 1 : 0; op < 3; ++op) {
                 const unsigned char* base = (op == 0) ? a.Qf : ((op == 1) ? a.dOf : a.dO16);
                 const unsigned char* tb = base + ((long)b * H * nt + qt) * REC;
-                const unsigned dst = (op < 2) ? lds0 + (i & 1) * STG + op * TILEB : lds0 + 2 * STG + (i % NK16) * TILEB;
+                const unsigned dst = (op < 2) ? lds0 + (i & 1) * STG + op * S0 : lds0 + 2 * STG + (i % NK16) * TILEB;
                 if constexpr (NP % NW == 0 && NPW <= 4) fl_glds16_run<NPW, NW * 1024>(tb, voff, dst + wave * 1024);
                 else {
 #pragma unroll
@@ -749,7 +758,8 @@
                     }
                 }
             }
-            if (wave == NW - 1) fl_glds16_s(a.c0 + ((long)b * a.Np + qt * 16) * H, (unsigned)(lane * 16), lds0 + C0OFF + (i & 1) * 1024);
+            if constexpr (!SAVEDP)
+                if (wave == NW - 1) fl_glds16_s(a.c0 + ((long)b * a.Np + qt * 16) * H, (unsigned)(lane * 16), lds0 + C0OFF + (i & 1) * 1024);
             if constexpr (DROP)
                 if (wave == 1) fl_glds16_s(a.keepbits + (((long)b * nt + qt) * nt + mj * NW) * 64, kb_voff, lds0 + KBOFF + (i & 1) * 1024);
         };
@@ -766,7 +776,32 @@
             }
         };
         auto load_q = [&](int i, int h0, Frags& o) { load_frags(smem + (i & 1) * STG, h0, o); };
-        auto load_d = [&](int i, int g0, Frags& o) { load_frags(smem + (i & 1) * STG + TILEB, g0, o); };
+        auto load_d = [&](int i, int g0, Frags& o) { load_frags(smem + (i & 1) * STG + S0, g0, o); };
+        auto load_p = [&](int i, fls16x4_t (&ph)[4][H / 4]) {
+            const unsigned char* pb = smem + (i & 1) * STG + wave * PB;
+#pragma unroll
+            for (int r = 0; r < 4; ++r) {
+                const unsigned char* src = pb + (p_rd0 ^ (unsigned)(r * 2 * H));
+                if constexpr (H == 8) {
+                    const flu32x4_t w = *reinterpret_cast<const flu32x4_t*>(src);
+                    ph[r][0] = __builtin_bit_cast(fls16x4_t, (flu32x2_t){w[0], w[1]});
+                    ph[r][1] = __builtin_bit_cast(fls16x4_t, (flu32x2_t){w[2], w[3]});
+                } else {
+                    static_assert(H == 4 || H == 8, "one 2 H byte chunk per (query, key)");
+                    ph[r][0] = *reinterpret_cast<const fls16x4_t*>(src);
+                }
+            }
+        };
+        auto cvt_p = [&](const fls16x4_t (&ph)[4][H / 4], f32x4_t (&sp)[4][H / 4]) {
+#pragma unroll
+            for (int r = 0; r < 4; ++r)
+#pragma unroll
+                for (int gh = 0; gh < H / 4; ++gh) {
+                    const flf16x4_t h4 = __builtin_bit_cast(flf16x4_t, ph[r][gh]);
+#pragma unroll
+                    for (int k = 0; k < 4; ++k) sp[r][gh][k] = (float)h4[k];
+                }
+        };
         auto front_q = [&](int i, auto h0_c, const Frags& qfr, f32x4_t (&sp)[4][H / 4], const f32x4_t (*rs_t)[4] = nullptr, f32x4_t* rs_o = nullptr) {
             constexpr int h0 = decltype(h0_c)::value;
             if constexpr (h0 == 0) {
@@ -870,7 +905,7 @@
                 *reinterpret_cast<fls16x4_t*>(gwb + g * GWR) =
                     fl_pack4<false>(sp[0][g >> 2][g & 3], sp[1][g >> 2][g & 3], sp[2][g >> 2][g & 3], sp[3][g >> 2][g & 3]);
         };
-        auto back_gw = [&](int i, f32x4_t (&sp)[4][H / 4], f32x4_t (&pp)[4][H / 4]) {
+        auto back_gw = [&](int i, f32x4_t (&sp)[4][H / 4], f32x4_t (&pp)[4][H / 4], const fls16x4_t (*ph)[H / 4] = nullptr) {
             {
                 const unsigned rdf = gw_rd + (i & 1) * GWT, rdb = gw_rd + 2 * GWT;
                 const unsigned char* gw_xrd = (gm < H) ? sgw + rdf : gw_zero;
@@ -889,7 +924,10 @@
             for (int r = 0; r < 4; ++r) {
                 fls16x4_t bv[H / 4];
 #pragma unroll
-                for (int hh = 0; hh < H / 4; ++hh) bv[hh] = fl_pack4_f16(sp[r][hh][0], sp[r][hh][1], sp[r][hh][2], sp[r][hh][3]);
+                for (int hh = 0; hh < H / 4; ++hh) {
+                    if constexpr (SAVEDP) bv[hh] = ph[r][hh];
+                    else bv[hh] = fl_pack4_f16(sp[r][hh][0], sp[r][hh][1], sp[r][hh][2], sp[r][hh][3]);
+                }
 #pragma unroll
                 for (int gh = 0; gh < H / 4; ++gh) {
                     f32x4_t d = vbw[gh];
@@ -990,6 +1028,52 @@
             if constexpr (H > HB) front_d(i + 1, std::integral_constant<int, HB>{}, fr1, dpn, kbn);
             back_dv(i, pp, kb);
         };
+        auto front_p = [&](int i, f32x4_t (&sp)[4][H / 4], f32x4_t (&dp)[4][H / 4], fls16x4_t (&ph)[4][H / 4], uint32_t (&kb)[4]) {
+            load_kb(i, kb);
+            load_p(i, ph);
+            Frags fa, fb;
+            load_d(i, 0, fa);
+            if constexpr (H > HB) load_d(i, HB, fb);
+            cvt_p(ph, sp);
+            front_d(i, std::integral_constant<int, 0>{}, fa, dp, kb);
+            if constexpr (H > HB) front_d(i, std::integral_constant<int, HB>{}, fb, dp, kb);
+        };
+        auto back_p = [&](int i, f32x4_t (&sp)[4][H / 4], f32x4_t (&dp)[4][H / 4], const fls16x4_t (&ph)[4][H / 4], const uint32_t (&kb)[4]) {
+            f32x4_t pp[4][H / 4];
+            back_ds(i, sp, dp);
+            back_gw(i, sp, pp, ph);
+            back_dv(i, pp, kb);
+        };
+        auto step_p = [&](int i, f32x4_t (&sp)[4][H / 4], f32x4_t (&dp)[4][H / 4], const fls16x4_t (&ph)[4][H / 4], f32x4_t (&spn)[4][H / 4],
+                          f32x4_t (&dpn)[4][H / 4], fls16x4_t (&phn)[4][H / 4], Frags& fr0, Frags& fr1, const uint32_t (&kb)[4], uint32_t (&kbn)[4], bool more) {
+            f32x4_t pp[4][H / 4];
+            constexpr bool RSF = FLB_RSFUSE && H == 2 * HB && FULL == 1 && TAIL16;
+            f32x4_t rt[4], ro0, ro1;
+            load_kb(i + 1, kbn);
+            load_p(i + 1, phn);
+            if constexpr (H > HB) load_d(i + 1, HB, fr1);
+            if constexpr (RSF) d_terms(0, sp, dp, rt);
+            __builtin_amdgcn_sched_barrier(FLB_SB_NOMEM);
+            if constexpr (RSF) {
+                front_d(i + 1, std::integral_constant<int, 0>{}, fr0, dpn, kbn, &rt, &ro0);
+                d_store(i, 0, ro0);
+                back_ds(i, sp, dp, false);
+                d_terms(1, sp, dp, rt);
+            } else {
+                front_d(i + 1, std::integral_constant<int, 0>{}, fr0, dpn, kbn);
+                back_ds(i, sp, dp);
+            }
+            FLB_PHASE();
+            if (FLB_STAGGER && more && wave >= NW / 2) issue_tiles(i + 2);
+            cvt_p(phn, spn);
+            back_gw(i, sp, pp, ph);
+            FLB_PHASE();
+            if constexpr (H > HB) {
+                if constexpr (RSF) { front_d(i + 1, std::integral_constant<int, HB>{}, fr1, dpn, kbn, &rt, &ro1); d_store(i, 1, ro1); }
+                else front_d(i + 1, std::integral_constant<int, HB>{}, fr1, dpn, kbn);
+            }
+            back_dv(i, pp, kb);
+        };
         auto admit = [&](int nxt, bool late) {
             asm volatile("s_waitcnt vmcnt(0)" ::: "memory");
             __builtin_amdgcn_s_barrier();
@@ -999,10 +1083,12 @@
 
         f32x4_t spA[4][H / 4], dpA[4][H / 4], spB[4][H / 4], dpB[4][H / 4];
         uint32_t kbA[4], kbB[4];
+        fls16x4_t phA[4][H / 4], phB[4][H / 4];
         Frags frA, frB;
         issue_tiles(0);
         admit(0, false);
-        if (wvalid) front(0, spA, dpA, kbA);
+        if constexpr (SAVEDP) { if (wvalid) front_p(0, spA, dpA, phA, kbA); }
+        else if (wvalid) front(0, spA, dpA, kbA);
         for (int i = 0; i + 1 < seg; ++i) {
             FLB_STAMP(0);
             admit(i + 1, FLB_STAGGER && wvalid);
@@ -1010,13 +1096,21 @@
             if (i > 0) d_flush(i - 1);
             FLB_STAMP(2);
             if (wvalid) {
-                load_q(i + 1, 0, frA);
-                step(i, spA, dpA, spB, dpB, frA, frB, kbA, kbB, i + 2 < seg);
+                if constexpr (SAVEDP) {
+                    load_d(i + 1, 0, frA);
+                    step_p(i, spA, dpA, phA, spB, dpB, phB, frA, frB, kbA, kbB, i + 2 < seg);
+                } else {
+                    load_q(i + 1, 0, frA);
+                    step(i, spA, dpA, spB, dpB, frA, frB, kbA, kbB, i + 2 < seg);
+                }
 #pragma unroll
                 for (int r = 0; r < 4; ++r) {
                     kbA[r] = kbB[r];
 #pragma unroll
-                    for (int gh = 0; gh < H / 4; ++gh) { spA[r][gh] = spB[r][gh]; dpA[r][gh] = dpB[r][gh]; }
+                    for (int gh = 0; gh < H / 4; ++gh) {
+                        spA[r][gh] = spB[r][gh]; dpA[r][gh] = dpB[r][gh];
+                        if constexpr (SAVEDP) phA[r][gh] = phB[r][gh];
+                    }
                 }
             }
 #ifdef FLB_DBG_STAMP
@@ -1026,7 +1120,8 @@
             ++stn;
 #endif
         }
-        if (wvalid) back(seg - 1, spA, dpA, kbA);
+        if constexpr (SAVEDP) { if (wvalid) back_p(seg - 1, spA, dpA, phA, kbA); }
+        else if (wvalid) back(seg - 1, spA, dpA, kbA);
         __builtin_amdgcn_s_barrier();
         if (seg > 1) d_flush(seg - 2);
         d_flush(seg - 1);
@@ -1093,6 +1188,9 @@
 }
 constexpr int flbk_lds_bytes(int H, int DT, bool drop) {
     return (4 + FLB_NK16) * H * DT * 512 + 2048 + 2 * FLB_NW * 16 * H * 4 + 512 + FLB_NW * 3 * 4 * H * FLB_GWR + (drop ? 2048 : 0);
+}
+constexpr int flbkp_lds_bytes(int H, int DT, bool drop) {
+    return (2 + FLB_NK16) * H * DT * 512 + 2 * FLB_NW * 512 * H + 2 * FLB_NW * 16 * H * 4 + 512 + FLB_NW * 3 * 4 * H * FLB_GWR + (drop ? 2048 : 0);
 }
 
 static int dispatch_bwdq(const FlashBwdArgs& a, int H, int dh, int nwg, hipStream_t st) {
@@ -1152,8 +1250,17 @@
         constexpr int HH = decltype(h)::value, DS = decltype(ds)::value, DT = FragDims<DS, decltype(tl)::value>::DT;
         constexpr bool TL = decltype(tl)::value;
         if constexpr (flbk_lds_bytes(HH, DT, true) > FL_LDS_MAX) return -2;
-        else return fl_launch<FlashBwdKArgs, talking_bwdk_kernel<HH, DS, TL, true>, talking_bwdk_kernel<HH, DS, TL, false>>(
+        else return fl_launch<FlashBwdKArgs, talking_bwdk_kernel<HH, DS, TL, true, false>, talking_bwdk_kernel<HH, DS, TL, false, false>>(
             a, nwg, 64 * FLB_NW, flbk_lds_bytes(HH, DT, false), flbk_lds_bytes(HH, DT, true), a.p_drop > 0.f, st);
+    });
+}
+static int dispatch_bwdk_p(const FlashBwdKArgs& a, int H, int dh, int nwg, hipStream_t st) {
+    return attn_dispatch(H, dh, [&](auto h, auto ds, auto tl) {
+        constexpr int HH = decltype(h)::value, DS = decltype(ds)::value, DT = FragDims<DS, decltype(tl)::value>::DT;
+        constexpr bool TL = decltype(tl)::value;
+        if constexpr (flbk_lds_bytes(HH, DT, true) > FL_LDS_MAX || flbkp_lds_bytes(HH, DT, true) > FL_LDS_MAX) return -2;
+        else return fl_launch<FlashBwdKArgs, talking_bwdk_kernel<HH, DS, TL, true, true>, talking_bwdk_kernel<HH, DS, TL, false, true>>(
+            a, nwg, 64 * FLB_NW, flbkp_lds_bytes(HH, DT, false), flbkp_lds_bytes(HH, DT, true), a.p_drop > 0.f, st);
     });
 }
 
@@ -1164,21 +1271,24 @@
     }) == 0;
 }
 
-extern "C" int spe_talking_bwdk_pass1(const void* Qf, const void* dOf, const void* dO16, const void* Kf, const void* Vf, const float* Wl, const float* Ww,
-                                      const float* bw, const float* c0, int Np, float* ws_d, float* ws_v, float* ws_w, float* Drows, float* dv, void* dv16,
-                                      long ob, long on, long oh, const void* keepbits, int B, int H, int N, int dh, int nwg, float p_drop, hipStream_t st) {
+static_assert(flbkp_lds_bytes(8, 3, true) <= FL_LDS_MAX && flbkp_lds_bytes(4, 4, true) <= FL_LDS_MAX, "saved P: every shape of the fused path fits");
+
+static int bwdk_run(const void* Qf, const void* dOf, const void* dO16, const void* Kf, const void* Vf, const float* Wl, const float* Ww,
+                    const float* bw, const float* c0, const void* P16, int Np, float* ws_d, float* ws_v, float* ws_w, float* Drows, float* dv, void* dv16,
+                    long ob, long on, long oh, const void* keepbits, int B, int H, int N, int dh, int nwg, float p_drop, hipStream_t st) {
     const int nt = (N + 15) / 16;
     if ((long)B * nt <= 0) return 0;
     if (dh < 1 || dh > 64 || nwg <= 0 || Np < nt * 16 + 64 || (p_drop > 0.f && !keepbits)) return -2;
-    if (!Qf || !dOf || !dO16 || !Kf || !Vf || !Wl || !Ww || !bw || !c0 || !ws_d || !ws_v || !ws_w || !Drows || (!dv && !dv16)) return -2;
+    if (!P16 && (!Qf || !Kf || !Wl || !c0)) return -2;
+    if (!dOf || !dO16 || !Vf || !Ww || !bw || !ws_d || !ws_v || !ws_w || !Drows || (!dv && !dv16)) return -2;
     const FlashPlan p = fl_plan(B, nt, FLB_NW, nt, nwg);
     FlashBwdKArgs a;
     a.Qf = (const unsigned char*)Qf; a.dOf = (const unsigned char*)dOf; a.dO16 = (const unsigned char*)dO16;
     a.Kf = (const unsigned char*)Kf; a.Vf = (const unsigned char*)Vf; a.Wl = Wl; a.Ww = Ww; a.bw = bw; a.c0 = c0; a.Np = Np;
-    a.ws_d = ws_d; a.ws_v = ws_v; a.ws_w = ws_w;
+    a.ws_d = ws_d; a.ws_v = ws_v; a.ws_w = ws_w; a.P16 = (const unsigned char*)P16;
     a.keepbits = (p_drop > 0.f) ? reinterpret_cast<const unsigned*>(keepbits) : nullptr;
     a.B = B; a.N = N; a.nt = nt; a.nmaj = p.nmaj; a.spw = p.spw; a.total = p.total; a.p_drop = p_drop;
-    int rc = dispatch_bwdk(a, H, dh, p.nwg, st);
+    int rc = P16 ? dispatch_bwdk_p(a, H, dh, p.nwg, st) : dispatch_bwdk(a, H, dh, p.nwg, st);
     if (rc != 0) return rc;
     const long n = (long)B * Np * H;
     hipLaunchKernelGGL(bwdk_rows_merge_kernel, dim3((unsigned)((n + 255) / 256)), dim3(256), 0, st, ws_d, Drows, B, H, N, Np, p.nmaj);
@@ -1190,3 +1300,17 @@
     SPE_CHECK_LAUNCH();
     return 0;
 }
+
+extern "C" int spe_talking_bwdk_pass1(const void* Qf, const void* dOf, const void* dO16, const void* Kf, const void* Vf, const float* Wl, const float* Ww,
+                                      const float* bw, const float* c0, int Np, float* ws_d, float* ws_v, float* ws_w, float* Drows, float* dv, void* dv16,
+                                      long ob, long on, long oh, const void* keepbits, int B, int H, int N, int dh, int nwg, float p_drop, hipStream_t st) {
+    return bwdk_run(Qf, dOf, dO16, Kf, Vf, Wl, Ww, bw, c0, nullptr, Np, ws_d, ws_v, ws_w, Drows, dv, dv16, ob, on, oh, keepbits, B, H, N, dh, nwg, p_drop, st);
+}
+
+extern "C" int spe_talking_bwdk_pass1_p(const void* P16, const void* dOf, const void* dO16, const void* Vf, const float* Ww, const float* bw, int Np,
+                                        float* ws_d, float* ws_v, float* ws_w, float* Drows, float* dv, void* dv16, long ob, long on, long oh,
+                                        const void* keepbits, int B, int H, int N, int dh, int nwg, float p_drop, hipStream_t st) {
+    if (!P16) return -2;
+    return bwdk_run(nullptr, dOf, dO16, nullptr, Vf, nullptr, Ww, bw, nullptr, P16, Np, ws_d, ws_v, ws_w, Drows, dv, dv16, ob, on, oh, keepbits, B, H, N, dh,
+                    nwg, p_drop, st);
+}
diff --git a/spe_amd/csrc/attn_flash_common.h b/spe_amd/csrc/attn_flash_common.h
--- a/spe_amd/csrc/attn_flash_common.h
+++ b/spe_amd/csrc/attn_flash_common.h
@@ -90,35 +90,38 @@
     }
 }
 
+#pragma clang diagnostic push
+#pragma clang diagnostic ignored "-Winline-asm"
 __device__ __forceinline__ void fl_glds16(const void* gsrc, unsigned lds_dst) {
     unsigned keep;
     asm volatile("s_mov_b32 %0, m0\n\ts_mov_b32 m0, %2\n\ts_nop 0\n\tglobal_load_lds_dwordx4 %1, off\n\ts_mov_b32 m0, %0"
-                 : "=&s"(keep) : "v"(gsrc), "s"(lds_dst) : "memory");
+                 : "=&s"(keep) : "v"(gsrc), "s"(lds_dst) : "memory", "m0");
 }
 
 __device__ __forceinline__ void fl_glds16_s(const void* sbase, unsigned voff, unsigned lds_dst) {
     unsigned keep;
     asm volatile("s_mov_b32 %0, m0\n\ts_mov_b32 m0, %3\n\ts_nop 0\n\tglobal_load_lds_dwordx4 %1, %2\n\ts_mov_b32 m0, %0"
-                 : "=&s"(keep) : "v"(voff), "s"(sbase), "s"(lds_dst) : "memory");
+                 : "=&s"(keep) : "v"(voff), "s"(sbase), "s"(lds_dst) : "memory", "m0");
 }
 template <int CNT, int STRIDE>
 __device__ __forceinline__ void fl_glds16_run(const void* sbase, const unsigned* voff, unsigned lds_dst) {
     static_assert(CNT >= 1 && CNT <= 4, "pieces per wave and tile");
     if constexpr (CNT == 1)
         asm volatile("s_mov_b32 m0, %1\n\ts_nop 0\n\tglobal_load_lds_dwordx4 %2, %0"
-                     :: "s"(sbase), "s"(lds_dst), "v"(voff[0]) : "memory");
+                     :: "s"(sbase), "s"(lds_dst), "v"(voff[0]) : "memory", "m0");
     else if constexpr (CNT == 2)
         asm volatile("s_mov_b32 m0, %1\n\ts_nop 0\n\tglobal_load_lds_dwordx4 %2, %0\n\ts_add_u32 m0, m0, %4\n\ts_nop 0\n\tglobal_load_lds_dwordx4 %3, %0"
-                     :: "s"(sbase), "s"(lds_dst), "v"(voff[0]), "v"(voff[1]), "n"(STRIDE) : "memory", "scc");
+                     :: "s"(sbase), "s"(lds_dst), "v"(voff[0]), "v"(voff[1]), "n"(STRIDE) : "memory", "scc", "m0");
     else if constexpr (CNT == 3)
         asm volatile("s_mov_b32 m0, %1\n\ts_nop 0\n\tglobal_load_lds_dwordx4 %2, %0\n\ts_add_u32 m0, m0, %5\n\ts_nop 0\n\tglobal_load_lds_dwordx4 %3, %0\n\t"
                      "s_add_u32 m0, m0, %5\n\ts_nop 0\n\tglobal_load_lds_dwordx4 %4, %0"
-                     :: "s"(sbase), "s"(lds_dst), "v"(voff[0]), "v"(voff[1]), "v"(voff[2]), "n"(STRIDE) : "memory", "scc");
+                     :: "s"(sbase), "s"(lds_dst), "v"(voff[0]), "v"(voff[1]), "v"(voff[2]), "n"(STRIDE) : "memory", "scc", "m0");
     else
         asm volatile("s_mov_b32 m0, %1\n\ts_nop 0\n\tglobal_load_lds_dwordx4 %2, %0\n\ts_add_u32 m0, m0, %6\n\ts_nop 0\n\tglobal_load_lds_dwordx4 %3, %0\n\t"
                      "s_add_u32 m0, m0, %6\n\ts_nop 0\n\tglobal_load_lds_dwordx4 %4, %0\n\ts_add_u32 m0, m0, %6\n\ts_nop 0\n\tglobal_load_lds_dwordx4 %5, %0"
-                     :: "s"(sbase), "s"(lds_dst), "v"(voff[0]), "v"(voff[1]), "v"(voff[2]), "v"(voff[3]), "n"(STRIDE) : "memory", "scc");
-}
+                     :: "s"(sbase), "s"(lds_dst), "v"(voff[0]), "v"(voff[1]), "v"(voff[2]), "v"(voff[3]), "n"(STRIDE) : "memory", "scc", "m0");
+}
+#pragma clang diagnostic pop
 
 template <int DSTEPS, bool TAIL16>
 __device__ __forceinline__ flu32x4_t fl_frag_global(const flu32x4_t* __restrict__ base, long rec, int st, int lane) {
diff --git a/spe_amd/kernels.py b/spe_amd/kernels.py
--- a/spe_amd/kernels.py
+++ b/spe_amd/kernels.py
@@ -1237,7 +1237,11 @@
     return ent
 
 
-def talking_flash_fwd(Qf, Kf, V16, Wl, Ww, bw, c0, B, H, N, dh, p_drop, seed, offset, want16=False, want16lo=False, want_bits=False):
+def saved_p_blocks(B, H, N, device):
+    return score_blocks(B, H, N, device, torch.float16).view(B, (N + 15) // 16, (N + 15) // 16, 4, 64, H)
+
+
+def talking_flash_fwd(Qf, Kf, V16, Wl, Ww, bw, c0, B, H, N, dh, p_drop, seed, offset, want16=False, want16lo=False, want_bits=False, want_p=False):
     dev = Qf.device
     nmaj = flash_plan(B, N)[2]
     ws = _flash_ws(dev, B * nmaj * FLASH_SLOTS * 128 * H * 16 * ((dh + 15) // 16))
@@ -1247,11 +1251,15 @@
     O16lo = torch.empty((B * N, C), device=dev, dtype=torch.bfloat16) if (want16 and want16lo) else None
     nt = (N + 15) // 16
     bits = torch.empty((B, nt, nt, 64), device=dev, dtype=torch.int32) if (want_bits and p_drop > 0) else None
-    _call("spe_talking_flash_fwd", _p(Qf), _p(Kf), _p(V16), _p(Wl), _p(Ww), _p(bw), _p(c0), c0.shape[1], _p(ws), _p(O), _p(O16), _p(O16lo),
-          _p(bits), B, H, N, dh, FLASH_NWG, float(p_drop), seed, offset, _st())
-    if want_bits:
-        return O, O16, O16lo, bits
-    return O, O16, O16lo
+    P16 = saved_p_blocks(B, H, N, dev) if want_p else None
+    if want_p:
+        _call("spe_talking_flash_fwd_p", _p(Qf), _p(Kf), _p(V16), _p(Wl), _p(Ww), _p(bw), _p(c0), c0.shape[1], _p(ws), _p(O), _p(O16), _p(O16lo),
+              _p(bits), _p(P16), B, H, N, dh, FLASH_NWG, float(p_drop), seed, offset, _st())
+    else:
+        _call("spe_talking_flash_fwd", _p(Qf), _p(Kf), _p(V16), _p(Wl), _p(Ww), _p(bw), _p(c0), c0.shape[1], _p(ws), _p(O), _p(O16), _p(O16lo),
+              _p(bits), B, H, N, dh, FLASH_NWG, float(p_drop), seed, offset, _st())
+    res = (O, O16, O16lo) + ((bits,) if want_bits else ())
+    return res + (P16,) if want_p else res
 
 
 def bwdq_plan(B, N):
@@ -1267,16 +1275,21 @@
     return r
 
 
-def talking_bwdk_pass1(Qf, dOf, dO16, Kf, Vf, Wl, Ww, bw, c0, keepbits, dv4, dv16, B, H, N, dh, p_drop):
+def talking_bwdk_pass1(Qf, dOf, dO16, Kf, Vf, Wl, Ww, bw, c0, keepbits, dv4, dv16, B, H, N, dh, p_drop, P16=None):
     ref = dv4 if dv4 is not None else dv16
     assert ref.stride(3) == 1 and (dv4 is None or dv16 is None or dv4.stride() == dv16.stride())
-    dev = Qf.device
+    dev = dOf.device
     _, nwg, nmaj = bwdq_plan(B, N)
     Np = c0.shape[1]
     ws_d = torch.empty((B * nmaj, Np, H), device=dev, dtype=torch.float32)
     ws_v = _flash_ws(dev, B * nmaj * FLASH_SLOTS * 4 * H * 256 * ((dh + 15) // 16))
     ws_w = torch.empty((4 * nwg, 2 * (H * H + H)), device=dev, dtype=torch.float32)
     Drows = torch.empty((B, Np, H), device=dev, dtype=torch.float32)
+    if P16 is not None:
+        assert P16.dtype == torch.float16 and P16.is_contiguous() and P16.numel() == B * ((N + 15) // 16) ** 2 * 256 * H
+        _call("spe_talking_bwdk_pass1_p", _p(P16), _p(dOf), _p(dO16), _p(Vf), _p(Ww), _p(bw), Np, _p(ws_d), _p(ws_v), _p(ws_w), _p(Drows), _p(dv4),
+              _p(dv16), ref.stride(0), ref.stride(1), ref.stride(2), _p(keepbits), B, H, N, dh, max(8, FLASH_NWG - _CU_RESERVE), float(p_drop), _st())
+        return Drows, ws_w
     _call("spe_talking_bwdk_pass1", _p(Qf), _p(dOf), _p(dO16), _p(Kf), _p(Vf), _p(Wl), _p(Ww), _p(bw), _p(c0), Np, _p(ws_d), _p(ws_v), _p(ws_w),
           _p(Drows), _p(dv4), _p(dv16), ref.stride(0), ref.stride(1), ref.stride(2), _p(keepbits), B, H, N, dh, max(8, FLASH_NWG - _CU_RESERVE),
           float(p_drop), _st())
```
